# privefl/bigsnpr

Hardware: AMD Instinct MI355X
Metric: SNP-cols/sec for bed_randomSVD k=20 (m*passes/wall) (higher is better)
Workload: dtype i8 (2-bit codes x 24-bit (early block steps) / 16-bit (late block steps) fixed-point image of the fp64 basis in int8 slices, exact int32 MFMA accumulation; fp64 panel algebra and Rayleigh-Ritz)

## Files before the change

bigsnpr_amd/_lib.py:

```python
import ctypes as C
import os
import threading

import numpy as np

_HERE = os.path.dirname(os.path.abspath(__file__))
LIB_PATH = os.path.join(_HERE, "libbigsnpr_hip.so")

u8p = C.POINTER(C.c_uint8)
i32p = C.POINTER(C.c_int32)
i64p = C.POINTER(C.c_int64)
u64p = C.POINTER(C.c_uint64)
f64p = C.POINTER(C.c_double)
vp = C.c_void_p
i64 = C.c_int64

ALLREDUCE_FN = C.CFUNCTYPE(None, C.c_void_p, C.c_int64, C.c_void_p)


class SvdOptions(C.Structure):
    _fields_ = [("k", C.c_int32), ("tol", C.c_double), ("block", C.c_int32),
                ("slices", C.c_int32), ("max_basis", C.c_int32), ("seed", C.c_uint32),
                ("verbose", C.c_int32), ("m_total", C.c_int64), ("allreduce", ALLREDUCE_FN),
                ("allreduce_ctx", C.c_void_p), ("hook_rank", C.c_int32), ("hook_world", C.c_int32),
                ("comm", C.c_void_p), ("binom_scaling", C.c_int32),
                ("center_out", C.POINTER(C.c_double)), ("scale_out", C.POINTER(C.c_double)),
                ("warm_start", C.c_int32), ("warm_denominator", C.c_int32), ("max_restarts", C.c_int32),
                ("vec_floor", C.c_double), ("exchange_timing", C.c_int32), ("exchange_timeout_ms", C.c_int32)]


class SvdInfo(C.Structure):
    _fields_ = [("niter", C.c_int32), ("nops", C.c_int32), ("basis", C.c_int32),
                ("converged", C.c_int32), ("max_rel_resid", C.c_double), ("gpu_ms", C.c_double),
                ("cprod_ms", C.c_double), ("prod_ms", C.c_double), ("n_cprod", C.c_int32),
                ("n_prod", C.c_int32), ("block", C.c_int32), ("slices", C.c_int32),
                ("n_bad", C.c_int32), ("fused_stats", C.c_int32), ("cprod_stats_ms", C.c_double),
                ("n_cprod_stats", C.c_int32), ("warm_launches", C.c_int32), ("warm_fraction", C.c_double),
                ("warm_ms", C.c_double), ("tiled", C.c_int32), ("segmented_passes", C.c_int32), ("compact_gathers", C.c_int32),
                ("slices_max", C.c_int32), ("wide_steps", C.c_int32), ("wide_cprod_ms", C.c_double),
                ("wide_prod_ms", C.c_double), ("n_wide_cprod", C.c_int32), ("n_wide_prod", C.c_int32),
                ("lead_rel_resid", C.c_double), ("exchange_mode", C.c_int32), ("n_exchange", C.c_int32 * 4),
                ("exchange_ms", C.c_double * 4), ("compacted", C.c_int32), ("compact_ms", C.c_double),
                ("out_of_core", C.c_int32), ("na_free_steps", C.c_double * 2), ("na_skip", C.c_int32)]


SIGNATURES = {
    "bsn_last_error": (C.c_char_p, []),
    "bsn_version": (C.c_int, []),
    "bsn_device_count": (C.c_int, [C.POINTER(C.c_int)]),
    "bsn_set_device": (C.c_int, [C.c_int]),
    "bsn_selftest": (C.c_int, []),
    "bsn_comm_unique_id": (C.c_int, [u8p]),
    "bsn_comm_init": (C.c_int, [u8p, C.c_int, C.c_int, C.POINTER(vp)]),
    "bsn_comm_rank": (C.c_int, [vp]),
    "bsn_comm_world": (C.c_int, [vp]),
    "bsn_comm_allreduce": (C.c_int, [vp, vp, i64]),
    "bsn_comm_abort": (C.c_int, [vp]),
    "bsn_comm_destroy": (C.c_int, [vp]),
    "bsn_ld_last_stats": (C.c_int, [f64p]),
    "bsn_robust_scale_tau2": (C.c_int, [vp, i64, i64, C.c_int32, C.c_double, C.c_double, f64p, f64p]),
    "bsn_robust_pair_scales": (C.c_int, [vp, i64, i64, C.c_int32, C.c_double, C.c_double, f64p, f64p]),
    "bsn_robust_mc_count": (C.c_int, [vp, i64, vp, i64, C.c_double, C.POINTER(C.c_int64)]),
    "bsn_robust_scale_cols": (C.c_int, [vp, i64, i64, C.c_int32, f64p]),
    "bsn_robust_rotate": (C.c_int, [vp, i64, i64, C.c_int32, f64p]),
    "bsn_robust_wdist": (C.c_int, [vp, i64, i64, C.c_int32, f64p, f64p, f64p]),
    "bsn_robust_dist_ogk": (C.c_int, [vp, i64, i64, C.c_int32, C.c_int32, C.c_double, C.c_double, C.c_double, f64p, C.POINTER(C.c_int64)]),
    "bsn_robust_rollmean": (C.c_int, [f64p, i64, f64p, C.c_int32, C.POINTER(C.c_int64), C.c_int32, f64p]),
    "bsn_robust_sort": (C.c_int, [f64p, i64]),
    "bsn_order_decreasing": (C.c_int, [f64p, i64, C.POINTER(C.c_int64), C.c_int32, i32p, i32p]),
    "bsn_robust_mc_window": (C.c_int, [vp, i64, vp, i64, C.c_double, C.c_double, i64, f64p, C.POINTER(C.c_int64)]),
    "bsn_bed_open": (C.c_int, [C.c_char_p, i64, i64, C.POINTER(vp)]),
    "bsn_bed_from_host": (C.c_int, [u8p, i64, i64, i64, C.POINTER(vp)]),
    "bsn_bed_from_fbm": (C.c_int, [u8p, i64, i64, i64, C.POINTER(vp)]),
    "bsn_fbm_open": (C.c_int, [u8p, i64, i64, i64, f64p, C.POINTER(vp)]),
    "bsn_bed_bits": (C.c_int, [vp]),
    "bsn_bed_tile": (C.c_int, [vp, C.POINTER(C.c_int)]),
    "bsn_bed_sample_major": (C.c_int, [vp, C.POINTER(C.c_int)]),
    "bsn_bed_na_known": (i64, [vp]),
    "bsn_bed_synthetic": (C.c_int, [i64, i64, C.c_uint32, C.c_uint32, C.c_uint32, i64, C.POINTER(vp)]),
    "bsn_bed_close": (C.c_int, [vp]),
    "bsn_bed_release_workspace": (C.c_int, [vp]),
    "bsn_bed_nrow": (i64, [vp]),
    "bsn_bed_ncol": (i64, [vp]),
    "bsn_bed_bytes": (i64, [vp]),
    "bsn_bed_download": (C.c_int, [vp, u8p]),
    "bsn_bed_prodvec": (C.c_int, [vp, i64p, i64, i64p, i64, f64p, f64p, f64p, f64p]),
    "bsn_bed_cprodvec": (C.c_int, [vp, i64p, i64, i64p, i64, f64p, f64p, f64p, f64p]),
    "bsn_bed_prodvec_sharded": (C.c_int, [vp, i64p, i64, i64p, i64, f64p, f64p, f64p, vp, f64p]),
    "bsn_bed_col_counts": (C.c_int, [vp, i64p, i64, i64p, i64, i32p]),
    "bsn_bed_row_counts": (C.c_int, [vp, i64p, i64, i64p, i64, i32p]),
    "bsn_bed_colstats": (C.c_int, [vp, i64p, i64, i64p, i64, f64p, f64p, i32p, i32p]),
    "bsn_snp_colstats": (C.c_int, [vp, i64p, i64, i64p, i64, f64p, f64p]),
    "bsn_bed_read": (C.c_int, [vp, i64p, i64, i64p, i64, C.c_int32, i32p]),
    "bsn_bed_read_scaled": (C.c_int, [vp, i64p, i64, i64p, i64, f64p, f64p, f64p]),
    "bsn_bed_cprod_planes": (C.c_int, [vp, i64p, i64, i64p, i64, f64p, i64, f64p, f64p]),
    "bsn_bed_prod_and_rowsumssq": (C.c_int, [vp, i64p, i64, i64p, i64, f64p, f64p, f64p, i64, f64p, f64p]),
    "bsn_snp_prod_and_rowsumssq2": (C.c_int, [vp, i64p, i64, i64p, i64, f64p, f64p, f64p, i64, f64p, f64p]),
    "bsn_mult_lin_reg": (C.c_int, [vp, i64p, i64, i64p, i64, f64p, i64, f64p]),
    "bsn_univ_linreg": (C.c_int, [vp, i64p, i64, i64p, i64, f64p, f64p, i64, f64p, f64p]),
    "bsn_univ_logreg": (C.c_int, [vp, i64p, i64, i64p, i64, f64p, f64p, i64, C.c_double, C.c_int32, f64p, f64p, i32p]),
    "bsn_impute_simple": (C.c_int, [vp, C.c_int, C.c_uint64, C.POINTER(vp), u8p, i64p]),
    "bsn_impute_last_ms": (C.c_int, [f64p]),
    "bsn_bed_to_fbm": (C.c_int, [vp, i64p, i64, i64p, i64, u8p]),
    "bsn_bed_readbina": (C.c_int, [vp, u8p, u8p]),
    "bsn_bed_is_streamed": (C.c_int, [vp]),
    "bsn_bed_streaming_kernels": (C.c_int, [vp, C.c_char_p, i64]),
    "bsn_bed_subset_payload": (C.c_int, [vp, i64p, i64, i64p, i64, u8p]),
    "bsn_op_create": (C.c_int, [vp, i64p, i64, i64p, i64, f64p, f64p, C.POINTER(vp)]),
    "bsn_op_destroy": (C.c_int, [vp]),
    "bsn_op_set_slices": (C.c_int, [vp, C.c_int]),
    "bsn_op_prod": (C.c_int, [vp, vp, i64, C.c_int, vp, i64]),
    "bsn_op_cprod": (C.c_int, [vp, vp, i64, C.c_int, vp, i64]),
    "bsn_op_sync": (C.c_int, [vp]),
    "bsn_op_last_kernel": (C.c_int, [vp, C.c_char_p, i64]),
    "bsn_bed_randomsvd": (C.c_int, [vp, i64p, i64, i64p, i64, f64p, f64p, C.POINTER(SvdOptions),
                                    f64p, f64p, f64p, C.POINTER(SvdInfo)]),
    "bsn_bed_tcrossprod": (C.c_int, [vp, i64p, i64, i64p, i64, f64p, f64p, i64, f64p]),
    "bsn_cormat": (C.c_int, [vp, i64p, i64, i64p, i64, C.c_double, f64p, f64p, C.c_int, i32p,
                             C.POINTER(C.c_int64), C.POINTER(vp)]),
    "bsn_cormat_fetch": (C.c_int, [vp, i32p, f64p]),
    "bsn_cormat_has_nan": (C.c_int, [vp, C.POINTER(C.c_int)]),
    "bsn_cormat_free": (C.c_int, [vp]),
    "bsn_ld_scores": (C.c_int, [vp, i64p, i64, i64p, i64, C.c_double, f64p, f64p]),
    "bsn_clumping_chr": (C.c_int, [vp, i64p, i64, i64p, i64, C.c_int, f64p, f64p, i32p, i32p, f64p,
                                   C.c_double, C.c_double, i32p]),
    "bsn_clumping_chr_cached": (C.c_int, [vp, i64p, i64, i64p, i64, C.c_int, f64p, f64p, i32p, i32p, f64p,
                                          i64, f64p, f64p, i32p]),
    "bsn_snp_grid_prs": (C.c_int, [vp, i64p, i64, i64p, i64, f64p, i32p, C.POINTER(C.c_uint8), i64, i64,
                                   C.c_int, f64p]),
    "bsn_sfbm_from_csc": (C.c_int, [i64p, i32p, f64p, i64, C.c_int, C.POINTER(vp)]),
    "bsn_sfbm_ncol": (C.c_int, [vp, i64p, i64p, i64p]),
    "bsn_sfbm_free": (C.c_int, [vp]),
    "bsn_lassosum2": (C.c_int, [vp, f64p, i64, f64p, f64p, f64p, i64, i64p, C.c_double, C.c_int32, C.c_double,
                                f64p, i32p, f64p]),
    "bsn_ldpred2_gibbs": (C.c_int, [vp, f64p, f64p, i64, i64p, f64p, f64p, i32p, u64p, i64, C.c_int, C.c_int, C.c_uint64,
                                    f64p, f64p]),
    "bsn_ldpred2_gibbs_sampling": (C.c_int, [vp, f64p, f64p, i64, i64p, C.c_double, C.c_double, C.c_int32, C.c_uint64,
                                             C.c_int, C.c_int, C.c_uint64, f64p, f64p]),
    "bsn_ldpred2_auto": (C.c_int, [vp, f64p, f64p, f64p, i64, i64p, f64p, u64p, i64, C.c_double, C.c_int, C.c_int, C.c_int,
                                   C.c_int, C.c_double, C.c_int, C.c_double, C.c_double, C.c_double, C.c_double,
                                   C.c_double, C.c_uint64, f64p, f64p, f64p, f64p, f64p, f64p, f64p, f64p]),
    "bsn_sfbm_prodvec": (C.c_int, [vp, f64p, i64p, i64, f64p]),
    "bsn_sfbm_ld_scores": (C.c_int, [vp, i64p, i64, f64p]),
    "bsn_sfbm_solve_sym": (C.c_int, [vp, f64p, f64p, i64p, i64, C.c_double, C.c_int32, f64p, i32p, f64p]),
    "bsn_sfbm_last_ms": (C.c_int, [vp, f64p]),
    "bsn_malloc": (C.c_int, [C.POINTER(vp), i64]),
    "bsn_free": (C.c_int, [vp]),
    "bsn_host_alloc": (C.c_int, [C.POINTER(vp), i64]),
    "bsn_host_free": (C.c_int, [vp]),
    "bsn_memcpy_h2d": (C.c_int, [vp, vp, i64]),
    "bsn_memcpy_d2h": (C.c_int, [vp, vp, i64]),
    "bsn_device_sync": (C.c_int, []),
    "bsn_timer_start": (C.c_int, [vp]),
    "bsn_timer_stop": (C.c_int, [vp, f64p]),
}

_lib = None


class BsnError(RuntimeError):
    pass


def load():
    global _lib
    if _lib is None:
        LIB_PATH = os.environ.get("BSN_LIB_PATH") or globals()["LIB_PATH"]
        if not os.path.exists(LIB_PATH):
            raise ImportError(
                "%s not found: build it with `python -m bigsnpr_amd.build` "
                "(there is no CPU fallback)" % LIB_PATH)
        lib = C.CDLL(LIB_PATH)
        for name, (res, args) in SIGNATURES.items():
            fn = getattr(lib, name)
            fn.restype = res
            fn.argtypes = args
        _lib = lib
    return _lib


def check(rc):
    if rc != 0:
        raise BsnError(load().bsn_last_error().decode("utf-8", "replace"))


def ptr(a, t):
    return None if a is None else a.ctypes.data_as(t)


def as_i64(a):
    return None if a is None else np.ascontiguousarray(a, dtype=np.int64)


def as_f64(a):
    return None if a is None else np.ascontiguousarray(a, dtype=np.float64)


class DeviceArray:

    def __init__(self, rows, cols=1):
        self.rows, self.cols = int(rows), int(cols)
        p = vp()
        check(load().bsn_malloc(C.byref(p), self.rows * self.cols * 8))
        self.ptr = p

    @classmethod
    def from_numpy(cls, a):
        a = np.asarray(a, dtype=np.float64)
        if a.ndim == 1:
            a = a[:, None]
        d = cls(a.shape[0], a.shape[1])
        h = np.asfortranarray(a)
        check(load().bsn_memcpy_h2d(d.ptr, h.ctypes.data_as(vp), h.nbytes))
        return d

    def to_numpy(self):
        h = np.empty((self.rows, self.cols), dtype=np.float64, order="F")
        check(load().bsn_memcpy_d2h(h.ctypes.data_as(vp), self.ptr, h.nbytes))
        return h

    def col_ptr(self, j):
        return vp(self.ptr.value + 8 * self.rows * j)

    def free(self):
        if self.ptr is not None and self.ptr.value:
            load().bsn_free(self.ptr)
            self.ptr = None

    def __del__(self):
        try:
            self.free()
        except Exception:
            pass


class _PinnedBlock:

    def __init__(self, pool, addr, size):
        self.pool, self.addr, self.size = pool, addr, size
        self.__array_interface__ = {"data": (addr, False), "shape": (size,), "typestr": "|u1", "version": 3}

    def __del__(self):
        try:
            self.pool._give_back(self.addr, self.size)
        except Exception:
            pass


class PinnedPool:

    def __init__(self, keep=None):
        self.free = []
        self.keep = int(os.environ.get("BSN_RESULT_POOL_KEEP", 1 << 30)) if keep is None else keep
        self.keep_max = int(os.environ.get("BSN_RESULT_POOL_MAX", 8 << 30))
        self.live = 0
        self.peak_live = 0
        self.lazy = not os.environ.get("BSN_RESULT_POOL_EAGER")
        self.pending = set()
        self.wanted = []
        self.prefetched = 0
        self.lock = threading.RLock()

    def empty(self, shape, dtype=np.float64):
        n = int(np.prod(shape)) * np.dtype(dtype).itemsize
        size = max(4096, (n + 4095) // 4096 * 4096)
        addr = None
        with self.lock:
            pick = None
            for i, (_, sz) in enumerate(self.free):
                if sz >= size and (pick is None or sz < self.free[pick][1]):
                    pick = i
            if pick is not None and self.free[pick][1] <= 2 * size:
                addr, sz = self.free.pop(pick)
        if addr is None and self.lazy:
            with self.lock:
                if size not in self.pending:
                    self.pending.add(size)
                    self.wanted.append(size)
            return np.empty(shape, dtype=dtype)
        if addr is None:
            p = vp()
            if load().bsn_host_alloc(C.byref(p), size) != 0 or not p.value:
                return np.empty(shape, dtype=dtype)
            addr, sz = p.value, size
        with self.lock:
            self.live += sz
            self.peak_live = max(self.peak_live, self.live)
        blk = _PinnedBlock(self, addr, sz)
        return np.asarray(blk)[:n].view(dtype).reshape(shape)

    def kick(self):
        with self.lock:
            sizes, self.wanted = self.wanted, []
        for size in sizes:
            threading.Thread(target=self._prefetch, args=(size,), daemon=True).start()

    def _prefetch(self, size):
        p = vp()
        try:
            ok = load().bsn_host_alloc(C.byref(p), size) == 0 and p.value
        except Exception:
            ok = False
        drop = []
        with self.lock:
            self.pending.discard(size)
            if ok:
                while self.free and sum(sz for _, sz in self.free) + size > self.keep_max:
                    drop.append(self.free.pop(0))
                self.free.append((p.value, size))
                self.prefetched += 1
        for addr, _ in drop:
            load().bsn_host_free(vp(addr))

    def _give_back(self, addr, size):
        with self.lock:
            self.live -= size
            limit = max(self.keep, min(self.peak_live, self.keep_max))
            keep = sum(sz for _, sz in self.free) + size <= limit
            if keep:
                self.free.append((addr, size))
        if not keep:
            load().bsn_host_free(vp(addr))

    def drain(self):
        with self.lock:
            blocks, self.free = self.free, []
            self.peak_live = self.live
        for addr, _ in blocks:
            load().bsn_host_free(vp(addr))


result_pool = PinnedPool()
```

bigsnpr_amd/csrc/api.hip:

```cpp
#include <dlfcn.h>
#include <fcntl.h>
#include <pthread.h>
#include <sys/mman.h>
#include <sys/stat.h>
#include <unistd.h>

#include <algorithm>
#include <cerrno>
#include <cmath>
#include <condition_variable>
#include <chrono>
#include <cstring>
#include <limits>
#include <map>
#include <memory>
#include <mutex>
#include <sched.h>
#include <atomic>
#include <thread>

#include <cstdlib>

#include "bsn_internal.hpp"
#include <cxxabi.h>

namespace bsn {

namespace {
struct Roctx {
  int (*push)(const char *) = nullptr;
  int (*pop)() = nullptr;
  Roctx() {
    if (!getenv("BSN_ROCTX")) return;
    void *h = nullptr;
    for (const char *name : {"librocprofiler-sdk-roctx.so", "librocprofiler-sdk-roctx.so.1", "libroctx64.so", "libroctx64.so.4"})
      if ((h = dlopen(name, RTLD_NOW | RTLD_GLOBAL))) break;
    if (!h) return;
    push = (int (*)(const char *))dlsym(h, "roctxRangePushA");
    pop = (int (*)())dlsym(h, "roctxRangePop");
    if (!push || !pop) push = nullptr, pop = nullptr;
  }
};
Roctx &roctx() {
  static Roctx r;
  return r;
}
}
void roctx_push(const char *name) {
  if (roctx().push) roctx().push(name);
}
void roctx_pop() {
  if (roctx().pop) roctx().pop();
}

static thread_local std::string g_err;
void set_error(const char *msg) { g_err = msg ? msg : ""; }
void fail(const char *fmt, ...) {
  char buf[1024];
  va_list ap;
  va_start(ap, fmt);
  vsnprintf(buf, sizeof(buf), fmt, ap);
  va_end(ap);
  throw Error(buf);
}

void require_gpu() {
  int n = 0;
  hipError_t e = hipGetDeviceCount(&n);
  if (e != hipSuccess || n <= 0)
    fail("no HIP device available: libbigsnpr_hip has no CPU fallback (%s)",
         e == hipSuccess ? "device count is 0" : hipGetErrorString(e));
}

static std::vector<int32_t> to_i32(const int64_t *ind, int64_t len, int64_t limit, const char *what) {
  std::vector<int32_t> v((size_t)len);
  if (!ind) {
    if (len > limit)
      fail("Tested %lld < %lld. Subscript out of bounds (%s).", (long long)(len - 1), (long long)limit, what);
    for (int64_t i = 0; i < len; i++) v[(size_t)i] = (int32_t)i;
    return v;
  }
  for (int64_t i = 0; i < len; i++) {
    if (ind[i] < 0 || ind[i] >= limit)
      fail("Tested %lld < %lld. Subscript out of bounds (%s).", (long long)ind[i], (long long)limit,
           what);
    v[(size_t)i] = (int32_t)ind[i];
  }
  return v;
}

namespace {
struct DevCache {
  std::mutex mu;
  std::multimap<size_t, void *> free_blocks[16];
  size_t held[16] = {0};
};
DevCache &dev_cache() {
  static DevCache *c = new DevCache();
  return *c;
}
size_t size_class(size_t bytes) {
  size_t c = 4096;
  while (c < bytes) {
    if (c + c / 2 >= bytes) return c + c / 2;
    c *= 2;
  }
  return c;
}
}

void *dev_alloc(size_t bytes, size_t *granted, int *device) {
  if (bytes == 0) bytes = 1;
  int dev = 0;
  BSN_HIP(hipGetDevice(&dev));
  *device = dev;
  const bool cached = bytes <= kDevCacheMaxBlock && dev < 16;
  const size_t want = cached ? size_class(bytes) : bytes;
  if (cached) {
    DevCache &c = dev_cache();
    std::lock_guard<std::mutex> lk(c.mu);
    auto it = c.free_blocks[dev].find(want);
    if (it != c.free_blocks[dev].end()) {
      void *p = it->second;
      c.free_blocks[dev].erase(it);
      c.held[dev] -= want;
      *granted = want;
      return p;
    }
  }
  static const bool trace = getenv("BSN_ALLOC_TRACE") != nullptr;
  void *p = nullptr;
  const auto t0 = std::chrono::steady_clock::now();
  hipError_t e = hipMalloc(&p, want);
  if (trace)
    std::fprintf(stderr, "[bsn alloc] hipMalloc %zu bytes (asked %zu): %.2f ms\n", want, bytes,
                 std::chrono::duration<double, std::milli>(std::chrono::steady_clock::now() - t0).count());
  if (e == hipErrorOutOfMemory) {
    (void)hipGetLastError();
    dev_cache_flush();
    e = hipMalloc(&p, want);
  }
  if (e != hipSuccess) fail("HIP error %s allocating %zu bytes of device memory", hipGetErrorString(e), want);
  *granted = want;
  return p;
}

void dev_release(void *p, size_t granted, int dev) {
  if (!p) return;
  DevCache &c = dev_cache();
  if (granted <= kDevCacheMaxBlock && dev >= 0 && dev < 16 && size_class(granted) == granted) {
    int cur = dev;
    (void)hipGetDevice(&cur);
    if (cur != dev) (void)hipSetDevice(dev);
    (void)hipDeviceSynchronize();
    if (cur != dev) (void)hipSetDevice(cur);
    std::lock_guard<std::mutex> lk(c.mu);
    if (c.held[dev] + granted <= kDevCacheMaxTotal) {
      c.free_blocks[dev].emplace(granted, p);
      c.held[dev] += granted;
      return;
    }
  }
  static const bool trace = getenv("BSN_ALLOC_TRACE") != nullptr;
  if (trace) std::fprintf(stderr, "[bsn alloc] hipFree %zu bytes\n", granted);
  (void)hipFree(p);
}

size_t dev_cache_held() {
  int dev = 0;
  if (hipGetDevice(&dev) != hipSuccess || dev < 0 || dev >= 16) return 0;
  DevCache &c = dev_cache();
  std::lock_guard<std::mutex> lk(c.mu);
  return c.held[dev];
}

void dev_cache_flush() {
  DevCache &c = dev_cache();
  std::lock_guard<std::mutex> lk(c.mu);
  for (int d = 0; d < 16; d++) {
    for (auto &kv : c.free_blocks[d]) (void)hipFree(kv.second);
    c.free_blocks[d].clear();
    c.held[d] = 0;
  }
}

constexpr size_t kStagePiece = 32u << 20;

void stage_init(bsn_bed *b) {
  for (int i = 0; i < 2; i++) {
    if (!b->h_stage[i]) BSN_HIP(hipHostMalloc((void **)&b->h_stage[i], kStagePiece, hipHostMallocDefault));
    if (!b->ev_stage[i]) BSN_HIP(hipEventCreateWithFlags(&b->ev_stage[i], hipEventDisableTiming));
  }
}

namespace {
struct CopyJob {
  void *dst = nullptr;
  const void *src = nullptr;
  size_t len = 0;
};
static inline void cpu_relax() {
#if defined(__x86_64__) || defined(__i386__)
  __builtin_ia32_pause();
#elif defined(__aarch64__)
  __asm__ __volatile__("yield");
#else
  std::this_thread::yield();
#endif
}
struct CopyPool {
  static constexpr int kMaxHelpers = 6;
  int nh = 2;
  std::mutex mu;
  std::condition_variable cv_go;
  CopyJob job[kMaxHelpers];
  std::atomic<unsigned long long> seq{0};
  std::atomic<int> pending{0}, sleepers{0};
  pid_t owner = 0;
  void start() {
    owner = getpid();
    cpu_set_t set;
    int cpus = (int)std::thread::hardware_concurrency();
    if (sched_getaffinity(0, sizeof(set), &set) == 0) cpus = std::min(cpus > 0 ? cpus : 1, CPU_COUNT(&set));
    nh = std::max(1, std::min(kMaxHelpers, cpus / 2 - 1));
    if (const char *e = getenv("BSN_COPY_THREADS")) nh = std::max(1, std::min(kMaxHelpers, atoi(e) - 1));
    for (int h = 0; h < nh; h++)
      std::thread([this, h] {
        unsigned long long seen = 0;
        for (;;) {
          int spins = 0;
          while (seq.load(std::memory_order_acquire) == seen) {
            if (++spins < 4000) {
              cpu_relax();
              continue;
            }
            std::unique_lock<std::mutex> lk(mu);
            sleepers.fetch_add(1);
            cv_go.wait(lk, [&] { return seq.load() != seen; });
            sleepers.fetch_sub(1);
          }
          seen = seq.load(std::memory_order_acquire);
          const CopyJob j = job[h];
          if (j.len) std::memcpy(j.dst, j.src, j.len);
          pending.fetch_sub(1, std::memory_order_release);
        }
      }).detach();
  }
  void copy(void *dst, const void *src, size_t len) {
    const size_t part = (len / (size_t)(nh + 1) + 63) & ~(size_t)63;
    for (int h = 0; h < nh; h++) {
      const size_t lo = part * (size_t)(h + 1), hi = h + 1 == nh ? len : std::min(len, lo + part);
      job[h] = lo < hi ? CopyJob{(uint8_t *)dst + lo, (const uint8_t *)src + lo, hi - lo} : CopyJob{};
    }
    pending.store(nh, std::memory_order_relaxed);
    seq.fetch_add(1);
    if (sleepers.load() > 0) {
      { std::lock_guard<std::mutex> lk(mu); }
      cv_go.notify_all();
    }
    std::memcpy(dst, src, std::min(part, len));
    while (pending.load(std::memory_order_acquire) != 0) cpu_relax();
  }
};
CopyPool *g_pool = nullptr;
std::mutex *g_pool_mu = new std::mutex();
void pool_atfork_child() {
  g_pool_mu = new std::mutex();
  g_pool = nullptr;
}
const int g_pool_atfork = pthread_atfork(nullptr, nullptr, pool_atfork_child);
}

static void host_copy(void *dst, const void *src, size_t len) {
  static const bool pool_off = [] {
    const char *e = getenv("BSN_COPY_THREADS");
    return e && atoi(e) <= 1;
  }();
  if (len < (256u << 10) || pool_off) {
    std::memcpy(dst, src, len);
    return;
  }
  std::unique_lock<std::mutex> lk(*g_pool_mu, std::try_to_lock);
  if (!lk.owns_lock()) {
    std::memcpy(dst, src, len);
    return;
  }
  if (!g_pool || g_pool->owner != getpid()) {
    g_pool = new CopyPool();
    g_pool->start();
  }
  g_pool->copy(dst, src, len);
}

void copy_h2d(bsn_bed *b, void *d_dst, const void *src, size_t bytes, hipStream_t stream) {
  if (!stream) stream = b->stream;
  stage_init(b);
  for (size_t off = 0; off < bytes; off += kStagePiece) {
    const size_t len = std::min(kStagePiece, bytes - off);
    const int s = (int)(b->stage_next++ & 1);
    if (b->stage_busy[s]) BSN_HIP(hipEventSynchronize(b->ev_stage[s]));
    host_copy(b->h_stage[s], (const uint8_t *)src + off, len);
    BSN_HIP(hipMemcpyAsync((uint8_t *)d_dst + off, b->h_stage[s], len, hipMemcpyHostToDevice, stream));
    BSN_HIP(hipEventRecord(b->ev_stage[s], stream));
    b->stage_busy[s] = true;
  }
}

hipStream_t upload_stream(bsn_bed *b) {
  if (!b->stream_up) {
    BSN_HIP(hipStreamCreateWithFlags(&b->stream_up, hipStreamNonBlocking));
    BSN_HIP(hipEventCreateWithFlags(&b->ev_up, hipEventDisableTiming));
  }
  return b->stream_up;
}

static bool host_is_pinned(const void *p) {
  hipPointerAttribute_t at;
  if (hipPointerGetAttributes(&at, p) != hipSuccess) {
    (void)hipGetLastError();
    return false;
  }
  return at.type == hipMemoryTypeHost;
}

void copy_d2h(bsn_bed *b, void *dst, const void *d_src, size_t bytes) {
  if (bytes >= (1u << 20) && host_is_pinned(dst)) {
    BSN_HIP(hipMemcpyAsync(dst, d_src, bytes, hipMemcpyDeviceToHost, b->stream));
    BSN_HIP(hipStreamSynchronize(b->stream));
    return;
  }
  stage_init(b);
  if (b->stream_up)
    for (int i = 0; i < 2; i++)
      if (b->stage_busy[i]) BSN_HIP(hipEventSynchronize(b->ev_stage[i]));
  const size_t npiece = (bytes + kStagePiece - 1) / kStagePiece;
  for (size_t k = 0; k <= npiece; k++) {
    if (k < npiece) {
      const size_t off = k * kStagePiece, len = std::min(kStagePiece, bytes - off);
      BSN_HIP(hipMemcpyAsync(b->h_stage[k & 1], (const uint8_t *)d_src + off, len, hipMemcpyDeviceToHost, b->stream));
      BSN_HIP(hipEventRecord(b->ev_stage[k & 1], b->stream));
    }
    if (k >= 1) {
      const size_t off = (k - 1) * kStagePiece, len = std::min(kStagePiece, bytes - off);
      BSN_HIP(hipEventSynchronize(b->ev_stage[(k - 1) & 1]));
      host_copy((uint8_t *)dst + off, b->h_stage[(k - 1) & 1], len);
    }
  }
  b->stage_busy[0] = b->stage_busy[1] = false;
}

static void free_bed(bsn_bed *b) { bed_free(b); }
void bed_free(bsn_bed *b) {
  if (!b) return;
  for (int i = 0; i < 2; i++) {
    if (b->h_stage[i]) (void)hipHostFree(b->h_stage[i]);
    if (b->ev_stage[i]) (void)hipEventDestroy(b->ev_stage[i]);
  }
  if (b->smaj_job) {
    try { image_smaj_wait(b); } catch (...) {}
  }
  if (b->d_img) (void)hipFree(b->d_img);
  if (b->map_base) (void)munmap(b->map_base, b->map_len);
  if (b->fd_file >= 0) (void)close(b->fd_file);
  if (b->slab_stage) delete (bsn::FileStage *)b->slab_stage;
  if (b->slab_img) bed_free(b->slab_img);
  if (b->sub) bed_free(b->sub);
  if (b->d_tiled) (void)hipFree(b->d_tiled);
  if (b->d_smaj) (void)hipFree(b->d_smaj);
  if (b->d_lut) (void)hipFree(b->d_lut);
  if (b->h_na_blocks) (void)hipHostFree(b->h_na_blocks);
  if (b->d_na_blocks) (void)hipFree(b->d_na_blocks);
  if (b->ev0) (void)hipEventDestroy(b->ev0);
  if (b->ev1) (void)hipEventDestroy(b->ev1);
  if (b->ev_up) (void)hipEventDestroy(b->ev_up);
  if (b->stream_up) (void)hipStreamDestroy(b->stream_up);
  if (b->stream && !b->stream_borrowed) (void)hipStreamDestroy(b->stream);
  delete b;
}

__global__ void k_fill_f64(double *p, int64_t n, double v) {
  const int64_t i = (int64_t)blockIdx.x * blockDim.x + threadIdx.x;
  if (i < n) p[i] = v;
}

void fill_op(bsn_op *op, bsn_bed *bed, const int64_t *ind_row, int64_t n, const int64_t *ind_col,
             int64_t m, const double *center, const double *scale, bool defer_scale, bool allow_streamed) {
  if (n <= 0 || m <= 0) fail("'ind.row' and 'ind.col' can't be empty.");
  if (bed->n >= (int64_t)1 << 31 || bed->m >= (int64_t)1 << 31) fail("dimension too large");
  if (!allow_streamed) require_resident(bed, "this function");
  BSN_HIP(hipSetDevice(bed->device));
  op->bed = bed;
  op->n = n;
  op->m = m;
  if (!ind_row && n > bed->n)
    fail("Tested %lld < %lld. Subscript out of bounds (ind.row).", (long long)(n - 1), (long long)bed->n);
  bool ident = (n == bed->n);
  if (ind_row) {
    for (int64_t i = 0; ident && i < n; i++) ident = (ind_row[i] == i);
  }
  op->rows_identity = ident;
  if (!ident) {
    auto r = to_i32(ind_row, n, bed->n, "ind.row");
    copy_h2d(bed, op->d_rows.ensure((size_t)n), r.data(), (size_t)n * 4);
  }
  bool contig = true;
  int64_t c0 = ind_col ? ind_col[0] : 0;
  if (ind_col)
    for (int64_t j = 0; contig && j < m; j++) contig = (ind_col[j] == c0 + j);
  if (c0 < 0 || c0 >= bed->m || (contig && c0 + m > bed->m))
    fail("Tested %lld < %lld. Subscript out of bounds (ind.col).", (long long)(c0 + m - 1),
         (long long)bed->m);
  op->cols_contig = contig;
  op->col0 = contig ? c0 : 0;
  if (!contig) {
    auto c = to_i32(ind_col, m, bed->m, "ind.col");
    int64_t m_pad = bsn::round_up(m, 64);
    c.resize((size_t)m_pad, c[0]);
    copy_h2d(bed, op->d_cols.ensure((size_t)m_pad), c.data(), (size_t)m_pad * 4);
  }
  op->no_na = false;
  if ((int64_t)bed->na_cnt.size() == bed->m && !getenv("BSN_FORCE_NA_PLANE")) {
    bool all0 = true;
    for (int64_t j = 0; all0 && j < m; j++) all0 = bed->na_cnt[(size_t)(ind_col ? ind_col[j] : j)] == 0;
    op->no_na = all0;
  }
  if (defer_scale) {
    op->d_center.ensure((size_t)m);
    op->d_scale.ensure((size_t)m);
    return;
  }
  op->d_center.ensure((size_t)m);
  op->d_scale.ensure((size_t)m);
  if (center) copy_h2d(bed, op->d_center.p, center, (size_t)m * 8);
  else BSN_HIP(hipMemsetAsync(op->d_center.p, 0, (size_t)m * 8, bed->stream));
  if (scale) {
    copy_h2d(bed, op->d_scale.p, scale, (size_t)m * 8);
  } else {
    hipLaunchKernelGGL(k_fill_f64, dim3((unsigned)((m + 255) / 256)), dim3(256), 0, bed->stream, op->d_scale.p, m, 1.0);
    BSN_HIP(hipGetLastError());
  }
}

void counts_device(bsn_op *op, const int64_t *ind_row, int64_t n, int32_t *d_counts) {
  bsn_bed *bed = op->bed;
  if (op->rows_identity) {
    counts_all_rows(bed, op->cols_contig ? nullptr : op->d_cols.p, op->col0, op->m, d_counts);
  } else {
    std::vector<double> w((size_t)bed->n, 0.0);
    for (int64_t i = 0; i < n; i++) w[(size_t)(ind_row ? ind_row[i] : i)] += 1.0;
    DevBuf<double> d_w;
    copy_h2d(bed, d_w.ensure((size_t)bed->n), w.data(), (size_t)bed->n * 8);
    counts_weighted(op, d_w.p, n, d_counts);
    BSN_HIP(hipStreamSynchronize(bed->stream));
  }
}

void require_resident(const bsn_bed *b, const char *what) {
  if (b->streamed())
    fail("%s needs the genotype image resident on the device: this handle streams its file (%.1f GB do not fit the device "
         "memory that was free when it was opened); bed_prodVec, bed_cprodVec, counts / colstats / MAF / scaleBinom and the "
         "`[` accessor are served out of core",
         what, (double)b->m * (double)b->pitch / 1e9);
}

bsn_bed *slab_image(bsn_bed *b) {
  BSN_HIP(hipSetDevice(b->device));
  if (!b->slab_img) {
    std::unique_ptr<bsn_bed, void (*)(bsn_bed *)> im(new bsn_bed(), bed_free);
    image_alloc(im.get(), b->n, b->slab_cols);
    (void)hipStreamDestroy(im->stream);
    im->stream = b->stream;
    im->stream_borrowed = true;
    b->slab_img = im.release();
  }
  if (!b->slab_stage) b->slab_stage = new FileStage();
  return b->slab_img;
}
int64_t slab_count(const bsn_bed *b) { return (b->m + b->slab_cols - 1) / b->slab_cols; }
void slab_upload_range(bsn_bed *b, int64_t j0, int64_t cnt) {
  bsn_bed *img = slab_image(b);
  if (j0 < 0 || cnt <= 0 || j0 + cnt > b->m || cnt > b->slab_cols)
    fail("internal: variants %lld .. %lld into a slab image of %lld", (long long)j0, (long long)(j0 + cnt), (long long)b->slab_cols);
  img->m = cnt;
  img->na_cnt.clear();
  img->forget_counts();
  image_from_file(img, b->fd_file, 3 + j0 * b->n_byte, b->n_byte, (FileStage *)b->slab_stage);
}
int64_t slab_upload(bsn_bed *b, int64_t sl, int64_t *j0_out) {
  const int64_t j0 = sl * b->slab_cols, cnt = std::min(b->slab_cols, b->m - j0);
  if (cnt <= 0) fail("internal: slab %lld of %lld", (long long)sl, (long long)slab_count(b));
  slab_upload_range(b, j0, cnt);
  if (j0_out) *j0_out = j0;
  return cnt;
}

namespace {
struct SlabWalk {
  bsn_bed *bed;
  bsn_bed *img;
  FileStage *stage;
  SlabWalk(bsn_bed *b) : bed(b) {
    img = slab_image(b);
    stage = (FileStage *)b->slab_stage;
  }
  template <class F>
  void run(const int64_t *ind_col, int64_t m, F f) {
    const int64_t nslab = (bed->m + bed->slab_cols - 1) / bed->slab_cols;
    std::vector<std::vector<int64_t>> pos((size_t)nslab);
    for (int64_t p = 0; p < m; p++) {
      const int64_t c = ind_col ? ind_col[p] : p;
      if (c < 0 || c >= bed->m) fail("Tested %lld < %lld. Subscript out of bounds (ind.col).", (long long)c, (long long)bed->m);
      pos[(size_t)(c / bed->slab_cols)].push_back(p);
    }
    std::vector<int64_t> local;
    for (int64_t sl = 0; sl < nslab; sl++) {
      const std::vector<int64_t> &P = pos[(size_t)sl];
      if (P.empty()) continue;
      const int64_t j0 = sl * bed->slab_cols;
      slab_upload(bed, sl);
      local.resize(P.size());
      for (size_t k = 0; k < P.size(); k++) local[k] = (ind_col ? ind_col[P[k]] : P[k]) - j0;
      f(img, P, local);
    }
  }
};
}

void counts_host(bsn_bed *bed, const int64_t *ind_row, int64_t n, const int64_t *ind_col,
                 int64_t m, int32_t *res) {
  if (bed->streamed()) {
    SlabWalk W(bed);
    std::vector<int32_t> part;
    W.run(ind_col, m, [&](bsn_bed *sb, const std::vector<int64_t> &P, const std::vector<int64_t> &local) {
      part.resize(4 * P.size());
      counts_host(sb, ind_row, n, local.data(), (int64_t)local.size(), part.data());
      for (size_t k = 0; k < P.size(); k++) std::memcpy(res + 4 * P[k], part.data() + 4 * k, 16);
    });
    return;
  }
  auto &cc = bed->counts_cache;
  const bool use_cache = n > 0 && m > 0 && !getenv("BSN_NO_COUNTS_CACHE");
  bool rows_all = n == bed->n;
  for (int64_t i = 0; rows_all && ind_row && i < n; i++) rows_all = ind_row[i] == i;
  std::vector<int64_t> lead;
  const int64_t *rows = ind_row;
  if (use_cache && !rows_all && !ind_row) {
    lead.resize((size_t)n);
    for (int64_t i = 0; i < n; i++) lead[(size_t)i] = i;
    rows = lead.data();
  }
  const bool same_rows = use_cache && !rows_all && (int64_t)cc.cnt.size() == 4 * bed->m && (int64_t)cc.rows.size() == n &&
                         std::memcmp(cc.rows.data(), rows, (size_t)n * 8) == 0;
  if (same_rows) {
    bool known = true;
    for (int64_t j = 0; known && j < m; j++) {
      const int64_t c = ind_col ? ind_col[j] : j;
      known = c >= 0 && c < bed->m && cc.cnt[(size_t)4 * c] >= 0;
    }
    if (known) {
      for (int64_t j = 0; j < m; j++) std::memcpy(res + 4 * j, &cc.cnt[(size_t)4 * (ind_col ? ind_col[j] : j)], 16);
      return;
    }
  }
  bsn_op op;
  fill_op(&op, bed, ind_row, n, ind_col, m, nullptr, nullptr, true);
  DevBuf<int32_t> d_counts;
  d_counts.ensure((size_t)4 * m);
  const bool device_cache = op.rows_identity && stats_cache_enabled(bed);
  const StatsCols sel{op.cols_contig ? nullptr : ind_col, op.cols_contig ? nullptr : op.d_cols.p, op.col0, m};
  if (device_cache && use_cache && stats_cache_known(bed, sel)) {
    stats_cache_load(bed, sel, d_counts.p, bed->stream);
    copy_d2h(bed, res, d_counts.p, (size_t)4 * m * 4);
    return;
  }
  counts_device(&op, ind_row, n, d_counts.p);
  if (device_cache) stats_cache_store(bed, sel, d_counts.p, bed->stream);
  copy_d2h(bed, res, d_counts.p, (size_t)4 * m * 4);
  if (op.rows_identity) {
    if ((int64_t)bed->na_cnt.size() != bed->m) bed->na_cnt.assign((size_t)bed->m, -1);
    for (int64_t j = 0; j < m; j++) bed->na_cnt[(size_t)(ind_col ? ind_col[j] : j)] = res[4 * j + 3];
  }
  if (use_cache && !rows_all) {
    if (!same_rows) {
      cc.clear();
      cc.rows.assign(rows, rows + n);
      cc.cnt.assign((size_t)4 * bed->m, -1);
    }
    for (int64_t j = 0; j < m; j++) std::memcpy(&cc.cnt[(size_t)4 * (ind_col ? ind_col[j] : j)], res + 4 * j, 16);
  }
}

__global__ void k_stats_cache_copy(int32_t *cache, int32_t *counts, const int32_t *cols, int64_t col0, int64_t m, int to_cache) {
  const int64_t j = (int64_t)blockIdx.x * blockDim.x + threadIdx.x;
  if (j >= m) return;
  const int64_t c = cols ? (int64_t)cols[j] : col0 + j;
  if (to_cache) *(int4 *)(cache + 4 * c) = *(const int4 *)(counts + 4 * j);
  else *(int4 *)(counts + 4 * j) = *(const int4 *)(cache + 4 * c);
}

bool stats_cache_enabled(const bsn_bed *b) {
  return b->bits == 2 && !b->generic && b->d_img != nullptr && !getenv("BSN_NO_STATS_CACHE");
}

static void stats_cols_check(const bsn_bed *b, const StatsCols &c) {
  if (c.m <= 0 || (c.ind_col ? c.d_cols == nullptr : (c.col0 < 0 || c.col0 + c.m > b->m)))
    fail("internal: selection of variants for the handle's code counts");
}

bool stats_cache_known(const bsn_bed *b, const StatsCols &c) {
  const auto &sc = b->stats_cache;
  stats_cols_check(b, c);
  if ((int64_t)sc.known.size() != b->m) return false;
  if (sc.n_known == b->m) return true;
  for (int64_t j = 0; j < c.m; j++)
    if (!sc.known[(size_t)(c.ind_col ? c.ind_col[j] : c.col0 + j)]) return false;
  return true;
}

void stats_cache_store(bsn_bed *b, const StatsCols &c, const int32_t *d_counts, hipStream_t st) {
// ... 964 lines not shown
```

bigsnpr_amd/csrc/bsn_internal.hpp:

```cpp
#pragma once
#include <hip/hip_runtime.h>
#include <stdint.h>

#include <atomic>
#include <cstdarg>
#include <cstdio>
#include <functional>
#include <cstdlib>
#include <memory>
#include <stdexcept>
#include <string>
#include <vector>

#include "bigsnpr_hip.h"

namespace bsn {
inline const char *abl_getenv(const char *name) {
#ifdef BSN_ABLATION
  return getenv(name);
#else
  (void)name;
  return nullptr;
#endif
}

struct Error : std::runtime_error {
  using std::runtime_error::runtime_error;
};
void set_error(const char *msg);
[[noreturn]] void fail(const char *fmt, ...);
void require_gpu();

#define BSN_HIP(expr)                                                             \
  do {                                                                            \
    hipError_t e__ = (expr);                                                      \
    if (e__ != hipSuccess)                                                        \
      ::bsn::fail("HIP error %s at %s:%d (%s)", hipGetErrorString(e__), __FILE__, \
                  __LINE__, #expr);                                               \
  } while (0)

template <class F>
int guarded(F &&f) {
  try {
    f();
    return 0;
  } catch (const std::exception &ex) {
    set_error(ex.what());
    (void)hipGetLastError();
    return 1;
  } catch (...) {
    set_error("unknown C++ exception");
    (void)hipGetLastError();
    return 1;
  }
}

constexpr size_t kDevCacheMaxBlock = (size_t)256 << 20;
constexpr size_t kDevCacheMaxTotal = (size_t)2 << 30;
void *dev_alloc(size_t bytes, size_t *granted, int *device);
void dev_release(void *p, size_t granted, int device);
void dev_cache_flush();
size_t dev_cache_held();

template <class T>
struct DevBuf {
  T *p = nullptr;
  size_t n = 0;
  size_t granted = 0;
  int device = 0;
  DevBuf() = default;
  DevBuf(const DevBuf &) = delete;
  DevBuf &operator=(const DevBuf &) = delete;
  ~DevBuf() { release(); }
  void release() {
    if (p) dev_release(p, granted, device);
    p = nullptr;
    n = 0;
    granted = 0;
  }
  T *ensure(size_t count) {
    if (count > n) {
      release();
      p = (T *)dev_alloc(count * sizeof(T), &granted, &device);
      n = count;
    }
    return p;
  }
};

constexpr int64_t kPitchAlign = 256;

inline int64_t round_up(int64_t a, int64_t b) { return (a + b - 1) / b * b; }

__host__ __device__ inline uint32_t dev_from_plink(uint32_t w) {
  return (~w & 0xAAAAAAAAu) | ((w ^ (w >> 1)) & 0x55555555u);
}
__host__ __device__ inline uint32_t plink_from_dev(uint32_t w) {
  return (~w & 0xAAAAAAAAu) | (~(w ^ (w >> 1)) & 0x55555555u);
}

}

struct bsn_bed;
namespace bsn {
struct SvdWorkspace;
}

constexpr int kCommClasses = 4;
struct bsn_comm {
  void *comm = nullptr;
  int rank = 0, world = 1, device = 0;
  hipStream_t stream = nullptr;
  std::atomic<int> aborted{0};
  bool timing = false;
  struct Timed { hipEvent_t a, b; int cls; };
  std::vector<Timed> timed;
  std::vector<hipEvent_t> ev_pool;
  ~bsn_comm() {
    for (auto &t : timed) { (void)hipEventDestroy(t.a); (void)hipEventDestroy(t.b); }
    for (auto e : ev_pool) (void)hipEventDestroy(e);
  }
};

constexpr int kProfKinds = 6;
struct bsn_op {
  bsn_bed *bed = nullptr;
  int64_t n = 0, m = 0;
  bool rows_identity = true;
  bool cols_contig = true;
  bool no_na = false;
  bool na_skip_c = false, na_skip_p = false;
  bool stats_pending = false;
  bsn::DevBuf<int32_t> d_counts;
  bsn::DevBuf<int32_t> d_na;
  long long *h_na_total = nullptr;
  bool na_poll = false;
  int64_t col0 = 0;
  int slices = 4;
  int64_t passes = 0;
  const double *late_center = nullptr, *late_scale = nullptr;
  const double *preq_X = nullptr;
  int64_t preq_ldx = 0;
  int preq_nvec = 0, preq_S = 0;
  bool profile = false;
  int prof_kind_override = -1;
  std::vector<hipEvent_t> ev_begin, ev_end;
  std::vector<int> ev_kind;
  std::vector<char> ev_more;
  const void *prof_kernel[kProfKinds] = {};
  const void *last_kernel = nullptr;
  ~bsn_op() {
    for (auto e : ev_begin) (void)hipEventDestroy(e);
    for (auto e : ev_end) (void)hipEventDestroy(e);
    if (h_na_total) (void)hipHostFree(h_na_total);
  }
  bsn::DevBuf<int32_t> d_rows;
  bsn::DevBuf<int32_t> d_cols;
  bsn::DevBuf<double> d_center, d_scale;
  bsn::DevBuf<double> d_xfull;
  bsn::DevBuf<int8_t> d_q;
  bsn::DevBuf<int32_t> d_acc;
  bsn::DevBuf<double> d_meta;
  bsn::DevBuf<double> d_yfull;
};

struct bsn_bed {
  int64_t n = 0, m = 0, n_byte = 0, pitch = 0;
  int bits = 2;
  double v_off = 0.0, v_step = 1.0;
  bool generic = false;
  double *d_lut = nullptr;
  uint8_t *d_img = nullptr;
  uint8_t *d_tiled = nullptr;
  bool tiled_tried = false;
  size_t tiled_cap = 0;
  const uint8_t *h_map = nullptr;
  void *map_base = nullptr;
  size_t map_len = 0;
  int64_t slab_cols = 0;
  int fd_file = -1;
  bsn_bed *slab_img = nullptr;
  void *slab_stage = nullptr;
  bool streamed() const { return d_img == nullptr && h_map != nullptr; }
  uint8_t *d_smaj = nullptr;
  int64_t pitch_smaj = 0, rows_smaj = 0;
  bool smaj_tried = false;
  size_t smaj_cap = 0;
  void *smaj_job = nullptr;
  int64_t cap_m = 0;
  bsn_bed *sub = nullptr;
  uint64_t sub_key = 0;
  std::vector<int64_t> sub_cols, sub_rows;
  bool last_solve_on_sub = false;
  int device = 0;
  bool stream_borrowed = false;
  hipStream_t stream = nullptr;
  hipStream_t stream_up = nullptr;
  hipEvent_t ev_up = nullptr;
  hipEvent_t ev0 = nullptr, ev1 = nullptr;
  std::vector<int32_t> na_cnt;
  struct CountsCache {
    std::vector<int64_t> rows;
    std::vector<int32_t> cnt;
    void clear() {
      rows.clear();
      cnt.clear();
    }
  } counts_cache;
  struct StatsCache {
    bsn::DevBuf<int32_t> d_cnt;
    std::vector<uint8_t> known;
    int64_t n_known = 0;
    bsn::DevBuf<int32_t> d_cols;
    uint64_t cols_key = 0;
    void clear() {
      known.clear();
      n_known = 0;
    }
    void release() {
      clear();
      d_cnt.release();
      d_cols.release();
      cols_key = 0;
    }
  } stats_cache;
  void forget_counts() {
    counts_cache.clear();
    stats_cache.clear();
  }
  int na_blocks_state = 0;
  long long *h_na_blocks = nullptr;
  long long *d_na_blocks = nullptr;
  double na_free[2] = {0.0, 0.0};
  std::unique_ptr<bsn_op> svd_op;
  std::shared_ptr<bsn::SvdWorkspace> svd_ws;
  uint8_t *h_stage[2] = {nullptr, nullptr};
  hipEvent_t ev_stage[2] = {nullptr, nullptr};
  bool stage_busy[2] = {false, false};
  unsigned stage_next = 0;
};


namespace bsn {

void image_alloc(bsn_bed *b, int64_t n, int64_t m, int bits = 2);
void stage_init(bsn_bed *b);
void bed_free(bsn_bed *b);
bsn_bed *image_gather(bsn_bed *src, const int64_t *ind_row, int64_t n, const int64_t *ind_col, int64_t m,
                      bsn_bed *reuse = nullptr);
bool image_tile(bsn_bed *b);
bool image_smaj(bsn_bed *b);
bool image_smaj_start(bsn_bed *b);
bool image_smaj_poll(bsn_bed *b);
void image_smaj_wait(bsn_bed *b);
void image_from_host(bsn_bed *b, const uint8_t *payload, int64_t n_byte_src);
struct FileStage {
  uint8_t *pin[2] = {nullptr, nullptr};
  hipEvent_t done[2] = {nullptr, nullptr};
  size_t bytes = 0;
  ~FileStage();
  FileStage() = default;
  FileStage(const FileStage &) = delete;
  FileStage &operator=(const FileStage &) = delete;
};
void image_from_file(bsn_bed *b, int fd, int64_t offset, int64_t n_byte_src, FileStage *stage = nullptr);
void image_from_fbm(bsn_bed *b, const uint8_t *bytes, int64_t ld, const uint8_t *lut);
void stats8(bsn_bed *b, const int32_t *d_rows, int64_t n, const int32_t *d_cols, int64_t col0, int64_t m,
            long long *d_out);
void lut_colstats(bsn_bed *b, const int32_t *d_rows, int64_t n, const int32_t *d_cols, int64_t col0, int64_t m,
                  double *d_out);
void lut_cprod(bsn_bed *b, const int32_t *d_rows, int64_t n, const int32_t *d_cols, int64_t col0, int64_t m,
               const double *d_center, const double *d_scale, const double *d_x, double *d_z);
void lut_prod(bsn_bed *b, const int32_t *d_rows, int64_t n, const int32_t *d_cols, int64_t col0, int64_t m,
              const double *d_center, const double *d_scale, const double *d_x, double *d_y);
void refuse_generic(const bsn_bed *b, const char *what);
void image_generate(bsn_bed *b, uint32_t seed, uint32_t npop, uint32_t na16, int64_t j_begin);
void image_download(bsn_bed *b, uint8_t *payload_out);
void counts_all_rows(bsn_bed *b, const int32_t *d_cols, int64_t col0, int64_t m, int32_t *d_counts);
void counts_host(bsn_bed *bed, const int64_t *ind_row, int64_t n, const int64_t *ind_col, int64_t m,
                 int32_t *res);
void counts_device(bsn_op *op, const int64_t *ind_row, int64_t n, int32_t *d_counts);
struct StatsCols {
  const int64_t *ind_col;
  const int32_t *d_cols;
  int64_t col0, m;
};
bool stats_cache_enabled(const bsn_bed *b);
bool stats_cache_known(const bsn_bed *b, const StatsCols &c);
void stats_cache_store(bsn_bed *b, const StatsCols &c, const int32_t *d_counts, hipStream_t st);
void stats_cache_load(bsn_bed *b, const StatsCols &c, int32_t *d_counts, hipStream_t st);
void read_dense(bsn_bed *b, const int32_t *d_rows, int64_t n, const int32_t *d_cols, int64_t m,
                const double *d_center, const double *d_scale, int32_t na_val, int32_t *d_out_i,
                double *d_out_d);

void to_bytes(bsn_bed *b, const int32_t *d_rows, int64_t n, const int32_t *d_cols, int64_t m,
              uint8_t *d_out);
void readbina_bytes(bsn_bed *b, const uint8_t *d_tab, uint8_t *d_out);
void subset_pack(bsn_bed *b, const int32_t *d_rows, int64_t n, const int32_t *d_cols, int64_t m,
                 uint8_t *d_out);

void copy_h2d(bsn_bed *b, void *d_dst, const void *src, size_t bytes, hipStream_t stream = nullptr);
hipStream_t upload_stream(bsn_bed *b);
void copy_d2h(bsn_bed *b, void *dst, const void *d_src, size_t bytes);

void fill_op(bsn_op *op, bsn_bed *bed, const int64_t *ind_row, int64_t n, const int64_t *ind_col,
             int64_t m, const double *center, const double *scale, bool defer_scale = false,
             bool allow_streamed = false);
bsn_bed *slab_image(bsn_bed *b);
int64_t slab_count(const bsn_bed *b);
int64_t slab_upload(bsn_bed *b, int64_t sl, int64_t *j0_out = nullptr);
void slab_upload_range(bsn_bed *b, int64_t j0, int64_t cnt);

hipEvent_t comm_time_begin(bsn_comm *c, hipStream_t st);
void comm_time_end(bsn_comm *c, hipEvent_t begin, int cls, hipStream_t st);
void comm_time_collect(bsn_comm *c, double ms[kCommClasses], int count[kCommClasses]);
bool comm_abort(bsn_comm *c);
void comm_allreduce_sum(bsn_comm *c, double *d_buf, int64_t count, hipStream_t st);
void comm_reduce_scatter_sum(bsn_comm *c, const double *d_send, double *d_recv, int64_t recv_count,
                             hipStream_t st);
void comm_all_gather(bsn_comm *c, const double *d_send, double *d_recv, int64_t send_count, hipStream_t st);

void op_poll_stats(bsn_op *op);
void op_na_blocks(bsn_op *op, int digit_cols);
void op_prod(bsn_op *op, const double *d_X, int64_t ldx, int nvec, double *d_Y, int64_t ldy);
void op_prod_acc(bsn_op *op, const double *d_X, int64_t ldx, int nvec, double *d_Y, int64_t ldy, double beta);
struct ProdSegment {
  int bs = 0, off = 0;
  const int32_t *d_rows = nullptr;
  double *d_out = nullptr;
};
bool op_prod_segments(bsn_op *op, const double *d_X, int64_t ldx, int nvec, int pieces, int stride, int nseg,
                      const ProdSegment *segs, const std::function<void(int)> &after);
void op_cprod(bsn_op *op, const double *d_X, int64_t ldx, int nvec, double *d_Z, int64_t ldz);
void op_cprod_prequant(bsn_op *op, const double *d_X, int64_t ldx, int nvec);
void op_cprod_raw(bsn_op *op, const double *d_X, int64_t ldx, int nvec, double *d_P, double *d_Q,
                  int64_t ld);
void require_bits(const bsn_bed *b, int bits, const char *what);
void op_row_sums_sq(bsn_op *op, double *d_out);
void op_row_counts(bsn_op *op, double *d_out);
void counts_weighted(bsn_op *op, const double *d_w, int64_t n_sub, int32_t *d_counts);
void selftest();
void roctx_push(const char *name);
void roctx_pop();
struct RoctxRange {
  explicit RoctxRange(const char *name) { roctx_push(name); }
  ~RoctxRange() { roctx_pop(); }
  RoctxRange(const RoctxRange &) = delete;
  RoctxRange &operator=(const RoctxRange &) = delete;
};
void require_resident(const bsn_bed *b, const char *what);
void prof_begin(bsn_op *op, int kind, bool more = false);
void prof_end(bsn_op *op);
void prof_collect(bsn_op *op, double ms[kProfKinds], int count[kProfKinds]);

}
```

bigsnpr_amd/csrc/svd.hip:

```cpp
#include <chrono>
#include <unistd.h>
#include <atomic>
#include <condition_variable>
#include <mutex>
#include <thread>
#include <cmath>
#include <cstring>
#include <memory>
#include <functional>

#include "bsn_internal.hpp"
#include "orth_small.hpp"
#include "svd_driver.hpp"

namespace bsn {

constexpr int kMaxB = 16;
constexpr int kTP = 256;

__device__ __forceinline__ uint32_t hmix(uint32_t x) {
  x ^= x >> 16; x *= 0x7feb352dU; x ^= x >> 15; x *= 0x846ca68bU; x ^= x >> 16;
  return x;
}

// ... 55 lines not shown
      for (int t = 0; t < NT; t++) {
        acc[t] = __builtin_amdgcn_mfma_f64_16x16x4f64(av[u].x, bval[t] ? bv[t][u].x : 0.0, acc[t], 0, 0, 0);
        acc[t] = __builtin_amdgcn_mfma_f64_16x16x4f64(av[u].y, bval[t] ? bv[t][u].y : 0.0, acc[t], 0, 0, 0);
      }
  };
  const int64_t nfull = r1 > r0 ? (r1 - r0) / 32 : 0;
  if (nfull > 0) {
    ld(r0, av0, bv0);
    for (int64_t g = 0; g < nfull; g += 2) {
      ld(r0 + 32 * (g + 1 < nfull ? g + 1 : nfull - 1), av1, bv1);
      mm(av0, bv0);
      ld(r0 + 32 * (g + 2 < nfull ? g + 2 : nfull - 1), av0, bv0);
      if (g + 1 < nfull) mm(av1, bv1);
    }
  }
  int64_t r = r0 + 32 * nfull;
  for (; r < r1; r += 8) {
    const int64_t i0 = r + 2 * kq, i1 = i0 + 1;
    const double a0 = i0 < r1 ? Ap[i0] : 0.0, a1 = i1 < r1 ? Ap[i1] : 0.0;
#pragma unroll
    for (int t = 0; t < NT; t++) {
      const double b0 = (bval[t] && i0 < r1) ? Bp[t][i0] : 0.0, b1 = (bval[t] && i1 < r1) ? Bp[t][i1] : 0.0;
      acc[t] = __builtin_amdgcn_mfma_f64_16x16x4f64(a0, b0, acc[t], 0, 0, 0);
      acc[t] = __builtin_amdgcn_mfma_f64_16x16x4f64(a1, b1, acc[t], 0, 0, 0);
    }
  }
  __shared__ double red[4][256];
#pragma unroll
  for (int t = 0; t < NT; t++) {
    if (t > 0) __syncthreads();
#pragma unroll
    for (int g = 0; g < 4; g++) red[wave][(kq + 4 * g) * 16 + a] = acc[t][g];
    __syncthreads();
    partial[(((int64_t)rc * gridDim.x + tile) * NT + t) * 256 + tid] =
        (red[0][tid] + red[1][tid]) + (red[2][tid] + red[3][tid]);
  }
}

__global__ __launch_bounds__(1024) void k_gemm_tn_reduce(const double *__restrict__ partial, int nrc, int ntile, int p,
                                                         int cb, double *C, int ldc) {
  const int tile = blockIdx.x, bt = blockIdx.y, nt = gridDim.y, t = threadIdx.x & 255, part = threadIdx.x >> 8;
  double sum = 0;
#pragma unroll 4
  for (int c = part; c < nrc; c += 4) sum += partial[(((int64_t)c * ntile + tile) * nt + bt) * 256 + t];
  __shared__ double sp[4][256];
  sp[part][t] = sum;
  __syncthreads();
  if (part == 0) {
    sum = (sp[0][t] + sp[1][t]) + (sp[2][t] + sp[3][t]);
    const int mrow = t >> 4, ncol = bt * 16 + (t & 15);
    if (tile * 16 + mrow < p && ncol < cb) C[(tile * 16 + mrow) + (int64_t)ncol * ldc] = sum;
  }
}

__global__ __launch_bounds__(256) void k_gemm_nn(const double *__restrict__ Q, int64_t ldq, int p,
                                                 const double *__restrict__ S, int nc,
                                                 const double *In, int64_t ldi, double alpha,
                                                 double beta, double *Out, int64_t ldo, int64_t n) {
  extern __shared__ __attribute__((aligned(16))) double sS[];
  constexpr int TP = kTP;
  const int64_t i = (int64_t)blockIdx.x * blockDim.x + threadIdx.x;
  double acc[kMaxB];
#pragma unroll
  for (int j = 0; j < kMaxB; j++) acc[j] = 0;
  for (int a0 = 0; a0 < p; a0 += TP) {
    int ta = p - a0 < TP ? p - a0 : TP;
    __syncthreads();
    for (int t = threadIdx.x; t < ta * kMaxB; t += blockDim.x) {
      int a = t / kMaxB, j = t % kMaxB;
      sS[t] = j < nc ? S[(a0 + a) + (int64_t)j * p] : 0.0;
    }
    __syncthreads();
    if (i < n) {
      for (int a = 0; a < ta; a++) {
        double q = Q[i + (int64_t)(a0 + a) * ldq];
#pragma unroll
        for (int j = 0; j < kMaxB; j++) acc[j] += q * sS[a * kMaxB + j];
      }
    }
  }
  if (i < n) {
#pragma unroll
    for (int j = 0; j < kMaxB; j++)
      if (j < nc) {
        double base = alpha != 0.0 ? alpha * In[i + (int64_t)j * ldi] : 0.0;
        Out[i + (int64_t)j * ldo] = base + beta * acc[j];
      }
  }
}

__global__ void k_put_block(double *M, int ld, int r, const double *src) {
  const int t = blockIdx.x * blockDim.x + threadIdx.x;
  if (t < r * r) M[(t % r) + (int64_t)(t / r) * ld] = src[t];
}

__global__ void k_right_mult(double *W, int64_t ld, int64_t n, int cb, int r, const double *M) {
  __shared__ double sM[kMaxB * kMaxB];
  if ((int)threadIdx.x < cb * r) sM[threadIdx.x] = M[threadIdx.x];
  __syncthreads();
  int64_t i = (int64_t)blockIdx.x * blockDim.x + threadIdx.x;
  if (i >= n) return;
  double w[kMaxB], o[kMaxB];
#pragma unroll
  for (int j = 0; j < kMaxB; j++) w[j] = j < cb ? W[i + j * ld] : 0.0;
#pragma unroll
  for (int c = 0; c < kMaxB; c++) {
    double s = 0;
#pragma unroll
    for (int j = 0; j < kMaxB; j++)
      if (j < cb && c < r) s += w[j] * sM[j + c * cb];
    o[c] = s;
  }
#pragma unroll
  for (int c = 0; c < kMaxB; c++)
    if (c < r) W[i + c * ld] = o[c];
}

struct DevCtx {
  int tid, nt;
  __device__ void sync() { __syncthreads(); }
};
__global__ __launch_bounds__(512) void k_orth2(OrthSmall a, unsigned long long *mx_clear) {
  __shared__ double sCs[kOrthMaxP * kOrthMaxB];
  __shared__ double sG[kOrthMaxB * kOrthMaxB], sR[kOrthMaxB * kOrthMaxB], sRi[kOrthMaxB * kOrthMaxB],
      sRo[kOrthMaxB * kOrthMaxB], sD[kOrthMaxB * kOrthMaxB], sT[2 * kOrthMaxB + 4];
  a.Cs = sCs;
  a.Gs = sG;
  a.Rs = sR;
  a.Ris = sRi;
  a.Ro = sRo;
  a.Dv = sD;
  a.tmp = sT;
  if (mx_clear && threadIdx.x < kOrthMaxB) mx_clear[threadIdx.x] = 0ull;
  DevCtx cx{(int)threadIdx.x, (int)blockDim.x};
  orth_small(cx, a);
}

template <int CBT>
__global__ __launch_bounds__(256) void k_update(const double *__restrict__ Q, int64_t ldq, int p,
                                                const double *__restrict__ C, const double *__restrict__ Ri,
                                                int cb, double *W, int64_t ldw, int64_t n,
                                                unsigned long long *mx) {
  constexpr int TP = 128, ROWS = 4;
  __shared__ double sS[TP * CBT], sRi[CBT * CBT], smx[4][CBT];
  const int tid = threadIdx.x, lane = tid & 63, wave = tid >> 6;
  for (int t = tid; t < CBT * CBT; t += 256) {
    const int j = t % CBT, c = t / CBT;
    sRi[t] = (j < cb && c < cb) ? Ri[j + c * cb] : 0.0;
  }
  if (tid < 4 * CBT) smx[tid / CBT][tid % CBT] = 0.0;
  const bool one_tile = p <= TP;
  for (int it = 0; it < ROWS; it++) {
    const int64_t i = ((int64_t)blockIdx.x * ROWS + it) * 256 + tid;
    double acc[CBT];
#pragma unroll
    for (int j = 0; j < CBT; j++) acc[j] = 0;
    for (int a0 = 0; a0 < p; a0 += TP) {
      const int ta = p - a0 < TP ? p - a0 : TP;
      if (!(one_tile && it > 0)) {
        __syncthreads();
        for (int t = tid; t < ta * CBT; t += 256) {
          const int a = t / CBT, j = t % CBT;
          sS[t] = j < cb ? C[(a0 + a) + (int64_t)j * p] : 0.0;
        }
        __syncthreads();
      }
      if (i < n) {
#pragma unroll 8
        for (int a = 0; a < ta; a++) {
          const double q = Q[i + (int64_t)(a0 + a) * ldq];
#pragma unroll
          for (int j = 0; j < CBT; j++) acc[j] += q * sS[a * CBT + j];
        }
      }
    }
    if (p == 0 && it == 0) __syncthreads();
    double w[CBT];
#pragma unroll
    for (int j = 0; j < CBT; j++) w[j] = (i < n && j < cb) ? W[i + j * ldw] - acc[j] : 0.0;
#pragma unroll 1
    for (int c = 0; c < cb; c++) {
      double s = 0;
#pragma unroll
      for (int j = 0; j < CBT; j++) s += w[j] * sRi[j + c * CBT];
      if (i < n) W[i + c * ldw] = s;
      if (mx) {
        double m = fabs(s);
        for (int off = 32; off > 0; off >>= 1) m = fmax(m, __shfl_down(m, off));
        if (lane == 0) smx[wave][c] = fmax(smx[wave][c], m);
      }
    }
  }
  if (mx) {
    __syncthreads();
    if (tid < cb) {
      const double m = fmax(fmax(smx[0][tid], smx[1][tid]), fmax(smx[2][tid], smx[3][tid]));
      atomicMax(&mx[tid], (unsigned long long)__double_as_longlong(m));
    }
  }
}

__global__ void k_col_absmax(const double *W, int64_t ld, int64_t n, unsigned long long *mx) {
  const int v = blockIdx.y;
  double m = 0;
  for (int64_t i = (int64_t)blockIdx.x * blockDim.x + threadIdx.x; i < n; i += (int64_t)gridDim.x * blockDim.x)
    m = fmax(m, fabs(W[i + v * ld]));
  for (int off = 32; off > 0; off >>= 1) m = fmax(m, __shfl_down(m, off));
  __shared__ double sm[16];
  const int wave = threadIdx.x >> 6, nw = blockDim.x >> 6;
  if ((threadIdx.x & 63) == 0) sm[wave] = m;
  __syncthreads();
  if (threadIdx.x == 0) {
    for (int w = 1; w < nw; w++) m = fmax(m, sm[w]);
    atomicMax(&mx[v], (unsigned long long)__double_as_longlong(m));
  }
}
__global__ void k_round_cols(double *W, int64_t ld, int64_t n, const unsigned long long *mx, int slices) {
  const int v = blockIdx.y;
  const double m = __longlong_as_double((long long)mx[v]);
  if (!(m > 0)) return;
  int e;
  frexp(ldexp(0.98, 8 * slices - 1) / m, &e);
  const double qs = ldexp(1.0, e - 1), iq = ldexp(1.0, 1 - e);
  const int64_t i = (int64_t)blockIdx.x * blockDim.x + threadIdx.x;
  if (i < n) W[i + v * ld] = (double)llrint(W[i + v * ld] * qs) * iq;
}

__global__ void k_block(const double *__restrict__ full, int64_t n, int cb, int64_t nr, int world,
                        double *__restrict__ blk) {
  const int64_t t = (int64_t)blockIdx.x * blockDim.x + threadIdx.x;
  if (t >= (int64_t)world * cb * nr) return;
  const int64_t i = t % nr, j = (t / nr) % cb, r = t / (nr * cb);
  const int64_t gi = r * nr + i;
  blk[t] = gi < n ? full[gi + j * n] : 0.0;
}
__global__ void k_unblock(const double *__restrict__ blk, int64_t n, int cb, int64_t nr,
                          double *__restrict__ full) {
  const int64_t t = (int64_t)blockIdx.x * blockDim.x + threadIdx.x;
  if (t >= n * cb) return;
  const int64_t gi = t % n, j = t / n;
  full[t] = blk[((gi / nr) * cb + j) * nr + gi % nr];
}
__global__ void k_max_over_ranks(const unsigned long long *__restrict__ all, int world, int cb,
                                 unsigned long long *__restrict__ mx) {
  const int v = threadIdx.x;
  if (v >= cb) return;
  unsigned long long m = 0;
  for (int r = 0; r < world; r++) m = all[r * cb + v] > m ? all[r * cb + v] : m;
  mx[v] = m;
}
template <typename INT>
__global__ void k_pack_int(double *__restrict__ W, int64_t nr, const unsigned long long *__restrict__ mx, int slices,
                           INT *__restrict__ q) {
  const int v = blockIdx.y;
  const int64_t i = (int64_t)blockIdx.x * blockDim.x + threadIdx.x;
  if (i >= nr) return;
  const double m = __longlong_as_double((long long)mx[v]);
  if (!(m > 0)) {
    q[i + v * nr] = 0;
    return;
  }
  int e;
  frexp(ldexp(0.98, 8 * slices - 1) / m, &e);
  const double qs = ldexp(1.0, e - 1), iq = ldexp(1.0, 1 - e);
  const long long k = llrint(W[i + v * nr] * qs);
  q[i + v * nr] = (INT)k;
  W[i + v * nr] = (double)k * iq;
}
template <typename INT>
__global__ void k_unpack_int(const INT *__restrict__ q, int64_t n, int cb, int64_t nr,
                             const unsigned long long *__restrict__ mx, int slices, double *__restrict__ full) {
  const int64_t t = (int64_t)blockIdx.x * blockDim.x + threadIdx.x;
  if (t >= n * cb) return;
  const int64_t gi = t % n, v = t / n;
  const double m = __longlong_as_double((long long)mx[v]);
  double val = 0.0;
  if (m > 0) {
    int e;
    frexp(ldexp(0.98, 8 * slices - 1) / m, &e);
    val = (double)q[((gi / nr) * cb + v) * nr + gi % nr] * ldexp(1.0, 1 - e);
  }
  full[t] = val;
}

__global__ void k_place_rows(const double *__restrict__ src, int64_t rows, int cb, int64_t r0, int64_t nr,
                             double *__restrict__ W) {
  const int64_t t = (int64_t)blockIdx.x * blockDim.x + threadIdx.x;
  if (t >= rows * cb) return;
  W[r0 + t % rows + (t / rows) * nr] = src[t];
}
__global__ void k_take_rows(const double *__restrict__ full, int64_t n, int cb, int64_t nr, int64_t row0,
                            double *__restrict__ W) {
  const int64_t t = (int64_t)blockIdx.x * blockDim.x + threadIdx.x;
  if (t >= nr * cb) return;
  const int64_t i = t % nr, j = t / nr;
  W[t] = row0 + i < n ? full[row0 + i + j * n] : 0.0;
}

struct SvdWorkspace {
  DevBuf<double> Q, Z, partial, dsmall, Wsave, dorth, Wfull, Wblk, Qfull, dS, dU, dV, dUfull, dM;
  double *h_pin = nullptr;
  size_t h_pin_n = 0;
  hipEvent_t ev_small = nullptr;
  hipStream_t st_comm = nullptr;
  hipEvent_t ev_seg[8] = {nullptr, nullptr, nullptr, nullptr, nullptr, nullptr, nullptr, nullptr};
  hipEvent_t ev_arrived = nullptr;
  DevBuf<int32_t> seg_rows;
  DevBuf<double> Wrecv;
  int64_t seg_n = -1, seg_nr = -1;
  int seg_world = -1;
  double *pinned(size_t count) {
    if (count > h_pin_n) {
      if (h_pin) (void)hipHostFree(h_pin);
      h_pin = nullptr;
      BSN_HIP(hipHostMalloc((void **)&h_pin, count * sizeof(double), hipHostMallocDefault));
      h_pin_n = count;
    }
    return h_pin;
  }
  ~SvdWorkspace() {
    for (auto &e : ev_seg)
      if (e) (void)hipEventDestroy(e);
    if (ev_arrived) (void)hipEventDestroy(ev_arrived);
    if (st_comm) (void)hipStreamDestroy(st_comm);
    if (ev_small) (void)hipEventDestroy(ev_small);
    if (h_pin) (void)hipHostFree(h_pin);
  }
};

struct HipSvdBackend : SvdBackend {
  SvdWorkspace &ws;
  explicit HipSvdBackend(SvdWorkspace &w)
      : ws(w), Q(w.Q), Z(w.Z), partial(w.partial), dsmall(w.dsmall), Wsave(w.Wsave), dorth(w.dorth),
        Wfull(w.Wfull), Wblk(w.Wblk), Qfull(w.Qfull) {}
  bsn_op *op = nullptr;
  hipStream_t st = nullptr;
  bsn_allreduce_fn hook = nullptr;
  void *ctx = nullptr;
  bsn_comm *comm = nullptr;
  int rank = 0, world = 1;
  bool dist = false;
  int64_t nr = 0, row0 = 0;
  DevBuf<double> &Q, &Z, &partial, &dsmall, &Wsave, &dorth, &Wfull, &Wblk, &Qfull;
  double *Wc = nullptr;
  int wcol = 0;
  std::vector<double> horth;
  int cap = 0, b = 0;
  int kmax = 0;
  bool mx_valid = false;
  bool no_fused = false;
  bool speculate = true;
  bool spec_rounded = false;
  int n_small_ar = 0;
  int64_t m_op_full = 0, m_sub = 0;
  bool fused_stats = false;
  int warm_launches = 0, warm_den = 16;
  bool subset(bool on) override {
    if (ooc) return false;
    if (on) {
      m_op_full = op->m;
      const int64_t m_lo = m_total / (world > 0 ? world : 1);
      const int64_t ms = (m_lo / warm_den) / 256 * 256;
      if (m_total / warm_den < 16384 || ms < 256) return false;
      m_sub = ms < op->m ? ms : op->m;
      op->m = m_sub;
      op->prof_kind_override = 3;
      roctx_push("svd:warm start (leading 1/16 of the variants)");
      return true;
    }
    roctx_pop();
    op->m = m_op_full;
    op->prof_kind_override = -1;
    warm_launches += 2;
    if (fused_stats) {
      op->stats_pending = true;
      op->na_poll = false;
      op->no_na = false;
    }
    return true;
  }
  bool timing = false;
  double t_phase[8] = {0, 0, 0, 0, 0, 0, 0, 0};
  int n_sync = 0;
  struct Tick {
    HipSvdBackend *b;
    int ph;
    std::chrono::steady_clock::time_point t0;
    Tick(HipSvdBackend *b_, int ph_) : b(b_), ph(ph_), t0(std::chrono::steady_clock::now()) {
      static const char *names[8] = {"svd:alloc", "svd:crossprod pass (Z = A'Q)", "svd:product pass (W = A Z)", "svd:gram blocks",
                                     "svd:orthonormalise", "svd:round / copy block", "svd:form u, v", "svd:other"};
      roctx_push(names[ph & 7]);
    }
    ~Tick() {
      roctx_pop();
      if (b->timing)
        b->t_phase[ph] += std::chrono::duration<double, std::milli>(std::chrono::steady_clock::now() - t0).count();
    }
  };
  void sync_stream() {
    BSN_HIP(hipStreamSynchronize(st));
    n_sync++;
  }

  void setup_ranks() {
    if (comm) {
      rank = comm->rank;
      world = comm->world;
    }
    dist = comm != nullptr || hook != nullptr;
    if (!dist) world = 1, rank = 0;
    nr = dist ? (n + world - 1) / world : n;
    if (dist && comm && nr >= 4096) nr = (nr + 511) / 512 * 512;
    row0 = (int64_t)rank * nr;
  }
  void alloc(int cap_, int b_) override {
    Tick tk(this, 0);
    if (b_ > kMaxB) fail("block size must be <= %d", kMaxB);
    cap = cap_;
    b = b_;
    Q.ensure((size_t)nr * (cap + kMaxB));
    Z.ensure((size_t)m_local * cap);
    {
      const int64_t rows_max = nr > m_local ? nr : m_local;
      partial.ensure((size_t)((rows_max + kGemmRows - 1) / kGemmRows) * ((cap + kMaxB + 15) / 16) * 2 * 256);
    }
    dsmall.ensure((size_t)(cap + 4) * 64);
    Wsave.ensure((size_t)nr * kMaxB);
    dorth.ensure((size_t)16 + 3 * kMaxB * kMaxB + (size_t)7 * (cap + kMaxB + 4) * kMaxB);
    ws.dM.ensure((size_t)kOrthMaxP * kOrthMaxP);
    if (dist) {
      const int wide = kmax > kMaxB ? kmax : kMaxB;
      Wfull.ensure((size_t)n * wide);
      Wblk.ensure((size_t)world * nr * wide);
      Qfull.ensure((size_t)n * kMaxB);
    }
    Wc = Q.p;
    wcol = 0;
  }

  void ar_small(double *d, int64_t count) {
    if (!dist) return;
    n_small_ar++;
    if (comm) {
      comm_allreduce_sum(comm, d, count, st);
    } else {
      sync_stream();
      hook(d, count, ctx);
    }
  }
  void reduce_scatter_W(int cb) {
    const int64_t tot = (int64_t)world * cb * nr;
    hipLaunchKernelGGL(k_block, dim3((unsigned)((tot + 255) / 256)), dim3(256), 0, st, Wfull.p, n, cb, nr, world,
                       Wblk.p);
    BSN_HIP(hipGetLastError());
    if (comm) {
      comm_reduce_scatter_sum(comm, Wblk.p, Wc, nr * cb, st);
    } else {
      sync_stream();
      hook(Wblk.p, tot, ctx);
      BSN_HIP(hipMemcpyAsync(Wc, Wblk.p + (int64_t)rank * cb * nr, (size_t)nr * cb * 8,
                             hipMemcpyDeviceToDevice, st));
    }
  }
  void all_gather_rows(const double *src, int cb, double *dst) {
    const int64_t tot = (int64_t)world * cb * nr;
    if (comm) {
      comm_all_gather(comm, src, Wblk.p, nr * cb, st);
    } else {
      BSN_HIP(hipMemsetAsync(Wblk.p, 0, (size_t)tot * 8, st));
      BSN_HIP(hipMemcpyAsync(Wblk.p + (int64_t)rank * cb * nr, src, (size_t)nr * cb * 8, hipMemcpyDeviceToDevice, st));
      sync_stream();
      hook(Wblk.p, tot, ctx);
    }
    hipLaunchKernelGGL(k_unblock, dim3((unsigned)((n * cb + 255) / 256)), dim3(256), 0, st, Wblk.p, n, cb, nr, dst);
    BSN_HIP(hipGetLastError());
  }

  void random_W(int bb, uint32_t seed) override {
    Wc = Q.p;
    wcol = 0;
    mx_valid = false;
    spec_rounded = false;
    op->preq_X = nullptr;
    hipLaunchKernelGGL(k_random, dim3((unsigned)((nr + 255) / 256), bb), dim3(256), 0, st, Wc, nr, nr, bb, seed,
                       row0, n);
    BSN_HIP(hipGetLastError());
  }
  const double *newest_block(int p0) const { return dist ? Qfull.p : Q.p + (int64_t)p0 * nr; }
  bool ooc = false;
  const int64_t *ooc_cols = nullptr;
  std::vector<int64_t> sel_at, sel_local;
  std::unique_ptr<bsn_op> sop;
  long long ooc_na_total = 0, ooc_n_bad = 0;
  bool ooc_stats_walk = false;
  int64_t slab_selection(int64_t sl, int64_t *at) {
    if (!ooc_cols) {
      int64_t j0 = 0;
      const int64_t cnt = slab_upload(op->bed, sl, &j0);
      *at = j0;
      sel_local.clear();
      return cnt;
    }
    if (sel_at.empty()) {
      const int64_t nslab = slab_count(op->bed), sc = op->bed->slab_cols;
      sel_at.assign((size_t)nslab + 1, 0);
      for (int64_t t = 0; t < m_local; t++) sel_at[(size_t)(ooc_cols[t] / sc) + 1]++;
      for (int64_t q = 0; q < nslab; q++) sel_at[(size_t)q + 1] += sel_at[(size_t)q];
    }
    const int64_t a = sel_at[(size_t)sl], cnt = sel_at[(size_t)sl + 1] - a;
    *at = a;
    if (cnt <= 0) return 0;
    int64_t j0 = 0;
    slab_upload(op->bed, sl, &j0);
    sel_local.resize((size_t)cnt);
    for (int64_t t = 0; t < cnt; t++) sel_local[(size_t)t] = ooc_cols[a + t] - j0;
    return cnt;
  }
  void slab_operator(int64_t j0, int64_t cnt, bool with_scaling) {
    bsn_bed *img = slab_image(op->bed);
    if (!sop) sop.reset(new bsn_op());
    sop->bed = img;
    sop->n = n;
    sop->m = cnt;
    sop->rows_identity = true;
    sop->cols_contig = true;
    sop->col0 = 0;
    if (!sel_local.empty()) {
      bool contig = true;
      for (int64_t t = 1; t < cnt && contig; t++) contig = sel_local[(size_t)t] == sel_local[0] + t;
      sop->cols_contig = contig;
      sop->col0 = contig ? sel_local[0] : 0;
      if (!contig) {
        const int64_t m_pad = round_up(cnt, 64);
        std::vector<int32_t> c((size_t)m_pad, (int32_t)sel_local[0]);
        for (int64_t t = 0; t < cnt; t++) c[(size_t)t] = (int32_t)sel_local[(size_t)t];
        copy_h2d(op->bed, sop->d_cols.ensure((size_t)m_pad), c.data(), (size_t)m_pad * 4);
        BSN_HIP(hipStreamSynchronize(st));
      }
    }
    sop->no_na = false;
    sop->slices = op->slices;
    sop->profile = op->profile;
    sop->prof_kind_override = op->prof_kind_override;
    sop->preq_X = nullptr;
    sop->d_center.ensure((size_t)op->bed->slab_cols);
    sop->d_scale.ensure((size_t)op->bed->slab_cols);
    if (with_scaling) {
      BSN_HIP(hipMemcpyAsync(sop->d_center.p, op->d_center.p + j0, (size_t)cnt * 8, hipMemcpyDeviceToDevice, st));
      BSN_HIP(hipMemcpyAsync(sop->d_scale.p, op->d_scale.p + j0, (size_t)cnt * 8, hipMemcpyDeviceToDevice, st));
    }
  }
  void At_Qblock_ooc(int p0, int cb) {
    const int64_t nslab = slab_count(op->bed);
    const bool stats = op->stats_pending;
    if (stats) {
      ooc_na_total = ooc_n_bad = 0;
      op->d_na.ensure((size_t)op->m);
    }
    for (int64_t sl = 0; sl < nslab; sl++) {
      int64_t j0 = 0;
      const int64_t cnt = slab_selection(sl, &j0);
      if (cnt <= 0) continue;
      slab_operator(j0, cnt, !stats);
      sop->stats_pending = stats;
      sop->na_poll = false;
      op_cprod(sop.get(), newest_block(p0), n, cb, Z.p + (int64_t)p0 * m_local + j0, m_local);
      if (stats) {
        BSN_HIP(hipMemcpyAsync(op->d_center.p + j0, sop->d_center.p, (size_t)cnt * 8, hipMemcpyDeviceToDevice, st));
        BSN_HIP(hipMemcpyAsync(op->d_scale.p + j0, sop->d_scale.p, (size_t)cnt * 8, hipMemcpyDeviceToDevice, st));
        BSN_HIP(hipMemcpyAsync(op->d_na.p + j0, sop->d_na.p, (size_t)cnt * 4, hipMemcpyDeviceToDevice, st));
        sync_stream();
        if (sop->h_na_total && sop->h_na_total[0] >= 0) {
          ooc_na_total += sop->h_na_total[0];
          ooc_n_bad += sop->h_na_total[1];
        }
      } else {
        sync_stream();
      }
    }
    if (stats) {
      op->stats_pending = false;
      if (!op->h_na_total) BSN_HIP(hipHostMalloc((void **)&op->h_na_total, 2 * sizeof(long long), hipHostMallocDefault));
      op->h_na_total[0] = ooc_na_total;
      op->h_na_total[1] = ooc_n_bad;
    }
    op->passes++;
  }
  void A_Zblock_ooc(int p0, int cb) {
    const int64_t nslab = slab_count(op->bed);
    bool first = true;
    for (int64_t sl = 0; sl < nslab; sl++) {
      int64_t j0 = 0;
      const int64_t cnt = slab_selection(sl, &j0);
      if (cnt <= 0) continue;
      slab_operator(j0, cnt, true);
      op_prod_acc(sop.get(), Z.p + (int64_t)p0 * m_local + j0, m_local, cb, Wc, n, first ? 0.0 : 1.0);
      first = false;
      sync_stream();
    }
    op->passes++;
  }
  void At_Qblock(int p0, int cb) override {
    Tick tk(this, 1);
    if (progress) progress();
    if (ooc) return At_Qblock_ooc(p0, cb);
    op_cprod(op, newest_block(p0), n, cb, Z.p + (int64_t)p0 * m_local, m_local);
  }
  bool product_in_segments(int p0, int cb) {
    if (!comm || nr % 512 != 0 || nr < 4096 || getenv("BSN_NO_SEGMENTS")) return false;
    const int B = (int)(nr / 512), nseg = B >= 16 ? 4 : 2;
    if (ws.seg_n != n || ws.seg_nr != nr || ws.seg_world != world) {
      std::vector<int32_t> rows((size_t)world * nr);
      size_t at = 0;
      for (int sgi = 0; sgi < nseg; sgi++) {
        const int b0 = (int)((int64_t)B * sgi / nseg), b1 = (int)((int64_t)B * (sgi + 1) / nseg);
        for (int r = 0; r < world; r++)
          for (int64_t t = (int64_t)b0 * 512; t < (int64_t)b1 * 512; t++) {
            const int64_t gi = (int64_t)r * nr + t;
            rows[at++] = gi < n ? (int32_t)gi : -1;
          }
      }
      copy_h2d(op->bed, ws.seg_rows.ensure(rows.size()), rows.data(), rows.size() * 4);
      BSN_HIP(hipStreamSynchronize(st));
      ws.seg_n = n; ws.seg_nr = nr; ws.seg_world = world;
    }
    const bool overlap = !getenv("BSN_NO_OVERLAP");
    if (overlap && !ws.st_comm) BSN_HIP(hipStreamCreateWithFlags(&ws.st_comm, hipStreamNonBlocking));
    for (int i = 0; i < nseg; i++)
      if (!ws.ev_seg[i]) BSN_HIP(hipEventCreateWithFlags(&ws.ev_seg[i], hipEventDisableTiming));
    if (!ws.ev_arrived) BSN_HIP(hipEventCreateWithFlags(&ws.ev_arrived, hipEventDisableTiming));
    ws.Wrecv.ensure((size_t)nr * kMaxB);
    ProdSegment segs[4];
    for (int sgi = 0; sgi < nseg; sgi++) {
      const int b0 = (int)((int64_t)B * sgi / nseg), b1 = (int)((int64_t)B * (sgi + 1) / nseg);
      segs[sgi].bs = b1 - b0;
      segs[sgi].off = b0;
      segs[sgi].d_rows = ws.seg_rows.p + (size_t)world * 512 * b0;
      segs[sgi].d_out = Wblk.p + (size_t)world * cb * 512 * b0;
    }
    hipStream_t sc = overlap ? ws.st_comm : st;
    const std::function<void(int)> after = [&](int sgi) {
      const int64_t rows_s = (int64_t)segs[sgi].bs * 512, r0 = (int64_t)segs[sgi].off * 512;
      if (overlap) {
        BSN_HIP(hipEventRecord(ws.ev_seg[sgi], st));
        BSN_HIP(hipStreamWaitEvent(sc, ws.ev_seg[sgi], 0));
      }
      double *recv = ws.Wrecv.p + (size_t)cb * r0;
      comm_reduce_scatter_sum(comm, segs[sgi].d_out, recv, rows_s * cb, sc);
      hipLaunchKernelGGL(k_place_rows, dim3((unsigned)((rows_s * cb + 255) / 256)), dim3(256), 0, sc, recv, rows_s, cb,
                         r0, nr, Wc);
      BSN_HIP(hipGetLastError());
    };
    if (overlap) {
      BSN_HIP(hipEventRecord(ws.ev_arrived, st));
      BSN_HIP(hipStreamWaitEvent(sc, ws.ev_arrived, 0));
    }
    if (!op_prod_segments(op, Z.p + (int64_t)p0 * m_local, m_local, cb, world, B, nseg, segs, after)) return false;
    if (overlap) {
      BSN_HIP(hipEventRecord(ws.ev_arrived, sc));
      hipEvent_t t0 = comm_time_begin(comm, st);
      BSN_HIP(hipStreamWaitEvent(st, ws.ev_arrived, 0));
      comm_time_end(comm, t0, 3, st);
    }
    n_seg_passes++;
    exchange_mode = std::max(exchange_mode, overlap ? 3 : 2);
    return true;
  }
  int min_slices = 8;
  bool hold_round = false;
  void hold_rounding(bool hold) override { hold_round = hold; }
  void set_precision(int S) override {
    if (S < 1) S = 1;
    if (S > 7) S = 7;
    op->slices = S;
    if (sop) sop->slices = S;
    if (S < min_slices) min_slices = S;
  }
  std::function<void()> progress;
  int n_seg_passes = 0;
  int exchange_mode = 0;
  int n_compact_gathers = 0;
  void A_Zblock(int p0, int cb) override {
    Tick tk(this, 2);
    mx_valid = false;
    if (ooc) return A_Zblock_ooc(p0, cb);
    if (dist && product_in_segments(p0, cb)) return;
    op_prod(op, Z.p + (int64_t)p0 * m_local, m_local, cb, dist ? Wfull.p : Wc, n);
    if (dist) {
      reduce_scatter_W(cb);
      exchange_mode = std::max(exchange_mode, 1);
    }
  }
  void gemm_tn_any(const double *A, const double *B, int64_t rows, int p, int cb, double *dC, int ldc = 0) {
    if (p <= 0 || cb <= 0) return;
    dim3 grid((unsigned)((p + 15) / 16), (unsigned)((rows + kGemmRows - 1) / kGemmRows));
    const int nt = (cb + 15) / 16;
    if (nt == 1)
      hipLaunchKernelGGL((k_gemm_tn<1>), grid, dim3(256), 0, st, A, rows, p, B, rows, cb, rows, partial.p);
    else if (nt == 2)
      hipLaunchKernelGGL((k_gemm_tn<2>), grid, dim3(256), 0, st, A, rows, p, B, rows, cb, rows, partial.p);
    else
      fail("internal: panel product with %d columns", cb);
    hipLaunchKernelGGL(k_gemm_tn_reduce, dim3(grid.x, nt), dim3(1024), 0, st, partial.p, (int)grid.y, (int)grid.x, p, cb,
                       dC, ldc > 0 ? ldc : p);
  }
  void gemm_tn(const double *A, int p, int cb, double *C_host) {
    gemm_tn_any(A, Wc, nr, p, cb, dsmall.p);
    BSN_HIP(hipGetLastError());
    ar_small(dsmall.p, (int64_t)p * cb);
    double *hp = ws.pinned((size_t)(cap + kMaxB + 4) * kMaxB * 4 + 1024);
    BSN_HIP(hipMemcpyAsync(hp, dsmall.p, (size_t)p * cb * 8, hipMemcpyDeviceToHost, st));
    sync_stream();
    std::memcpy(C_host, hp, (size_t)p * cb * 8);
  }
  void round_cols(double *X, int64_t rows, int cb, bool have_mx) {
    unsigned long long *mx = (unsigned long long *)dorth.p;
    if (!have_mx) {
      BSN_HIP(hipMemsetAsync(mx, 0, (size_t)cb * 8, st));
      hipLaunchKernelGGL(k_col_absmax, dim3(256, cb), dim3(1024), 0, st, X, rows, rows, mx);
    }
    hipLaunchKernelGGL(k_round_cols, dim3((unsigned)((rows + 255) / 256), cb), dim3(256), 0, st, X, rows, rows, mx,
                       op->slices);
    BSN_HIP(hipGetLastError());
  }
  void round_W(int cb) override {
    if (cb <= 0) return;
    if (spec_rounded) {
      spec_rounded = false;
      return;
    }
    Tick tk(this, 5);
    if (!dist) {
      round_cols(Wc, n, cb, mx_valid);
      mx_valid = false;
      return;
    }
    if (comm && op->slices <= 4 && nr % 4 == 0 && !getenv("BSN_NO_COMPACT_GATHER")) {
      unsigned long long *mx = (unsigned long long *)dorth.p;
      BSN_HIP(hipMemsetAsync(mx, 0, (size_t)cb * 8, st));
      hipLaunchKernelGGL(k_col_absmax, dim3(64, cb), dim3(1024), 0, st, Wc, nr, nr, mx);
      double *gmax = ws.Wrecv.ensure(std::max((size_t)nr * kMaxB, (size_t)world * kMaxB));
      comm_all_gather(comm, (const double *)mx, gmax, cb, st);
      hipLaunchKernelGGL(k_max_over_ranks, dim3(1), dim3(64), 0, st, (const unsigned long long *)gmax, world, cb, mx);
      const dim3 gp((unsigned)((nr + 255) / 256), cb), gu((unsigned)((n * cb + 255) / 256));
      if (op->slices <= 2) {
        int16_t *q_send = (int16_t *)Wfull.p, *q_all = (int16_t *)Wblk.p;
        hipLaunchKernelGGL((k_pack_int<int16_t>), gp, dim3(256), 0, st, Wc, nr, mx, op->slices, q_send);
        BSN_HIP(hipGetLastError());
        comm_all_gather(comm, (const double *)q_send, (double *)q_all, nr * cb / 4, st);
        hipLaunchKernelGGL((k_unpack_int<int16_t>), gu, dim3(256), 0, st, q_all, n, cb, nr, mx, op->slices, Qfull.p);
      } else {
        int32_t *q_send = (int32_t *)Wfull.p, *q_all = (int32_t *)Wblk.p;
        hipLaunchKernelGGL((k_pack_int<int32_t>), gp, dim3(256), 0, st, Wc, nr, mx, op->slices, q_send);
        BSN_HIP(hipGetLastError());
        comm_all_gather(comm, (const double *)q_send, (double *)q_all, nr * cb / 2, st);
        hipLaunchKernelGGL((k_unpack_int<int32_t>), gu, dim3(256), 0, st, q_all, n, cb, nr, mx, op->slices, Qfull.p);
      }
      BSN_HIP(hipGetLastError());
      n_compact_gathers++;
      return;
    }
    all_gather_rows(Wc, cb, Qfull.p);
    round_cols(Qfull.p, n, cb, false);
    hipLaunchKernelGGL(k_take_rows, dim3((unsigned)((nr * cb + 255) / 256)), dim3(256), 0, st, Qfull.p, n, cb, nr,
                       row0, Wc);
    BSN_HIP(hipGetLastError());
  }
  void gram_to_host(const double *A, const double *B, int64_t rows, int p, int cb, double *out) {
    Tick tk(this, 3);
    gemm_tn_any(A, B, rows, p, cb, dsmall.p);
    BSN_HIP(hipGetLastError());
    ar_small(dsmall.p, (int64_t)p * cb);
    double *hp = ws.pinned((size_t)(cap + kMaxB + 4) * kMaxB * 4 + 1024);
    BSN_HIP(hipMemcpyAsync(hp, dsmall.p, (size_t)p * cb * 8, hipMemcpyDeviceToHost, st));
    sync_stream();
    std::memcpy(out, hp, (size_t)p * cb * 8);
    op_poll_stats(op);
  }
  void ZtZ(int p, int p0, int cb, double *G) override {
    gram_to_host(Z.p, Z.p + (int64_t)p0 * m_local, m_local, p, cb, G);
  }
  void QtQ(int p, int p0, int cb, double *M) override {
    gram_to_host(Q.p, Q.p + (int64_t)p0 * nr, nr, p, cb, M);
  }

  static constexpr int B2 = kMaxB * kMaxB;
  void update_W(int p, int cb, const double *C, const double *Ri, unsigned long long *mx) {
    const dim3 rows((unsigned)((nr + 1023) / 1024));
    if (cb <= 8)
      hipLaunchKernelGGL((k_update<8>), rows, dim3(256), 0, st, Q.p, nr, p, C, Ri, cb, Wc, nr, nr, mx);
    else
      hipLaunchKernelGGL((k_update<16>), rows, dim3(256), 0, st, Q.p, nr, p, C, Ri, cb, Wc, nr, nr, mx);
  }
  int fused(int p, int p0, int cb, bool with_grams, double *blkZ, double *blkQ, std::vector<double> &Rout) {
    if (cb <= 0 || cb > kMaxB || p + cb > kOrthMaxP || p + cb > cap + kMaxB || no_fused) return -1;
    if (p > 0 && Wc != Q.p + (int64_t)p * nr) return -1;
    if (p > 0 && !with_grams) return -1;
    const double *A0 = p > 0 ? Q.p : Wc;
    Tick tk(this, 4);
    hipEvent_t tev0 = nullptr, tev1 = nullptr;
    if (timing) {
      BSN_HIP(hipEventCreate(&tev0));
      BSN_HIP(hipEventCreate(&tev1));
      BSN_HIP(hipEventRecord(tev0, st));
    }
    unsigned long long *mx = (unsigned long long *)dorth.p;
    const size_t pc = (size_t)p * cb, hg = (size_t)(p + cb) * cb;
    double *flag = dorth.p + 16, *dRout = flag + 1, *dZtZ = dRout + B2, *X = dZtZ + pc, *HG1 = X + (p > 0 ? hg : 0),
           *HG2 = HG1 + hg, *C = HG2 + hg, *Ct = C + pc, *Ri = Ct + pc;
    BSN_HIP(hipMemsetAsync(flag, 0, (size_t)(1 + B2) * 8, st));
    if (p > 0) gemm_tn_any(Z.p, Z.p + (int64_t)p0 * m_local, m_local, p, cb, dZtZ);
    BSN_HIP(hipMemcpyAsync(Wsave.p, Wc, (size_t)nr * cb * 8, hipMemcpyDeviceToDevice, st));
    OrthSmall a;
    a.p = p;
    a.cb = cb;
    a.p0 = p0;
    a.QtQ = p > 0 ? X : nullptr;
    a.ldq = p + cb;
    a.M = ws.dM.p;
    a.ldm = kOrthMaxP;
    a.C = C;
    a.Ct = Ct;
    a.Ri = Ri;
    a.Rout = dRout;
    a.flag = flag;
    a.iters = std::min(min_slices, op->slices) >= 2 ? 2 : 4;
    a.Cs = a.Gs = a.Rs = a.Ris = a.Ro = a.Dv = a.tmp = nullptr;
    for (int pass = 0; pass < 2; pass++) {
      double *HG = pass == 0 ? HG1 : HG2;
      if (pass == 0 && p > 0) {
        gemm_tn_any(Q.p, Q.p + (int64_t)p0 * nr, nr, p + cb, 2 * cb, X, p + cb);
        ar_small(dZtZ, (int64_t)(pc + 2 * hg));
      } else {
        gemm_tn_any(A0, Wc, nr, p + cb, cb, HG, p + cb);
        ar_small(HG, (int64_t)hg);
      }
      a.pass = pass;
      a.HG = HG;
      unsigned long long *mxp = (pass == 1 && !dist) ? mx : nullptr;
      hipLaunchKernelGGL(k_orth2, dim3(1), dim3(512), 0, st, a, mxp);
      update_W(p, cb, C, Ri, mxp);
    }
    BSN_HIP(hipGetLastError());
    const size_t nsmall = 1 + B2 + pc + (p > 0 ? hg : 0);
    double *hp = ws.pinned((size_t)(cap + kMaxB + 4) * kMaxB * 4 + 1024);
    BSN_HIP(hipMemcpyAsync(hp, flag, nsmall * 8, hipMemcpyDeviceToHost, st));
    if (timing) BSN_HIP(hipEventRecord(tev1, st));
    if (with_grams && speculate && !hold_round) {
      if (!ws.ev_small) BSN_HIP(hipEventCreateWithFlags(&ws.ev_small, hipEventDisableTiming));
      BSN_HIP(hipEventRecord(ws.ev_small, st));
      mx_valid = !dist;
      spec_rounded = false;
      round_W(cb);
      if (!ooc) op_cprod_prequant(op, dist ? Qfull.p : Wc, n, cb);
      spec_rounded = true;
      BSN_HIP(hipEventSynchronize(ws.ev_small));
      n_sync++;
    } else {
      sync_stream();
    }
    if (timing) {
      float ms = 0;
      BSN_HIP(hipEventElapsedTime(&ms, tev0, tev1));
      t_phase[7] += ms;
      (void)hipEventDestroy(tev0);
      (void)hipEventDestroy(tev1);
    }
    op_poll_stats(op);
    if (blkZ) std::memcpy(blkZ, hp + 1 + B2, pc * 8);
    if (blkQ)
      for (int j = 0; j < cb; j++) std::memcpy(blkQ + (size_t)j * p, hp + 1 + B2 + pc + (size_t)j * (p + cb), (size_t)p * 8);
    if (hp[0] != 0.0) {
      BSN_HIP(hipMemcpyAsync(Wc, Wsave.p, (size_t)nr * cb * 8, hipMemcpyDeviceToDevice, st));
      mx_valid = false;
      spec_rounded = false;
      op->preq_X = nullptr;
      return -2;
    }
    Rout.assign((size_t)cb * cb, 0.0);
    for (int t = 0; t < cb * cb; t++) Rout[(size_t)t] = hp[1 + (size_t)t];
    mx_valid = spec_rounded ? false : !dist;
    return cb;
  }
  int step_fused(int p, int p0, int cb, double *blkZ, double *blkQ, std::vector<double> &Rout) override {
    return fused(p, p0, cb, true, blkZ, blkQ, Rout);
  }
  int orth_fused(int p, int cb, std::vector<double> &Cacc, std::vector<double> &Rout) override {
    if (p != 0) return -1;
    Cacc.clear();
    const int r = fused(0, 0, cb, false, nullptr, nullptr, Rout);
    return r < 0 ? -1 : r;
  }
  void QtW(int p, int cb, double *C) override { gemm_tn(Q.p, p, cb, C); }
  void WtW(int cb, double *G) override { gemm_tn(Wc, cb, cb, G); }
  void W_minus_QC(int p, int cb, const double *C) override {
    mx_valid = false;
    copy_h2d(op->bed, dsmall.p, C, (size_t)p * cb * 8);
    hipLaunchKernelGGL(k_gemm_nn, dim3((unsigned)((nr + 255) / 256)), dim3(256), kTP * kMaxB * 8, st,
                       Q.p, nr, p, dsmall.p, cb, Wc, nr, 1.0, -1.0, Wc, nr, nr);
    BSN_HIP(hipGetLastError());
    sync_stream();
  }
  void W_times(int cb, int r, const double *M) override {
    mx_valid = false;
    copy_h2d(op->bed, dsmall.p, M, (size_t)cb * r * 8);
    hipLaunchKernelGGL(k_right_mult, dim3((unsigned)((nr + 255) / 256)), dim3(256), 0, st, Wc, nr, nr,
                       cb, r, dsmall.p);
    BSN_HIP(hipGetLastError());
    sync_stream();
  }
  void W_to_Q(int p0, int r) override {
    double *dst = Q.p + (int64_t)p0 * nr;
    if (dst != Wc)
      BSN_HIP(hipMemcpyAsync(dst, Wc, (size_t)nr * r * 8, hipMemcpyDeviceToDevice, st));
    wcol = p0 + r;
    Wc = Q.p + (int64_t)wcol * nr;
  }
  bool restart(int pp, int keep, const double *S, int rn, const double *Mk) override {
    if (keep + rn > pp || keep <= 0) return false;
    DevBuf<double> &dS = ws.dS, &tQ = ws.dU, &tZ = ws.dV;
    dS.ensure((size_t)pp * keep + 16);
    tQ.ensure((size_t)nr * keep);
    tZ.ensure((size_t)m_local * keep);
    copy_h2d(op->bed, dS.p, S, (size_t)pp * keep * 8);
    for (int c0 = 0; c0 < keep; c0 += kMaxB) {
      const int nc = keep - c0 < kMaxB ? keep - c0 : kMaxB;
      hipLaunchKernelGGL(k_gemm_nn, dim3((unsigned)((nr + 255) / 256)), dim3(256), kTP * kMaxB * 8, st, Q.p, nr, pp,
                         dS.p + (size_t)c0 * pp, nc, (const double *)nullptr, (int64_t)0, 0.0, 1.0,
                         tQ.p + (int64_t)c0 * nr, nr, nr);
      hipLaunchKernelGGL(k_gemm_nn, dim3((unsigned)((m_local + 255) / 256)), dim3(256), kTP * kMaxB * 8, st, Z.p,
                         m_local, pp, dS.p + (size_t)c0 * pp, nc, (const double *)nullptr, (int64_t)0, 0.0, 1.0,
                         tZ.p + (int64_t)c0 * m_local, m_local, m_local);
    }
    BSN_HIP(hipGetLastError());
    BSN_HIP(hipMemcpyAsync(Q.p, tQ.p, (size_t)nr * keep * 8, hipMemcpyDeviceToDevice, st));
    BSN_HIP(hipMemcpyAsync(Z.p, tZ.p, (size_t)m_local * keep * 8, hipMemcpyDeviceToDevice, st));
    double *dst = Q.p + (int64_t)keep * nr;
    BSN_HIP(hipMemcpyAsync(dst, Wc, (size_t)nr * rn * 8, hipMemcpyDeviceToDevice, st));
    Wc = dst;
    wcol = keep;
    copy_h2d(op->bed, dS.p, Mk, (size_t)keep * keep * 8);
    hipLaunchKernelGGL(k_put_block, dim3((unsigned)((keep * keep + 255) / 256)), dim3(256), 0, st, ws.dM.p,
                       kOrthMaxP, keep, dS.p);
    BSN_HIP(hipGetLastError());
    return true;
  }
  void finalize(int pp, int k, const double *S, const double *dinv, double *u, double *v) override {
    Tick tk(this, 6);
    std::vector<double> Sv((size_t)pp * k);
    for (int t = 0; t < k; t++)
      for (int i = 0; i < pp; i++) Sv[(size_t)i + (size_t)t * pp] = S[(size_t)i + (size_t)t * pp] * dinv[t];
    DevBuf<double> &dS = ws.dS, &dU = ws.dU, &dV = ws.dV, &dUfull = ws.dUfull;
    dS.ensure((size_t)pp * k * 2 + 16);
    dU.ensure((size_t)nr * k);
    dV.ensure((size_t)m_local * k);
    copy_h2d(op->bed, dS.p, S, (size_t)pp * k * 8);
    copy_h2d(op->bed, dS.p + (size_t)pp * k, Sv.data(), (size_t)pp * k * 8);
    for (int c0 = 0; c0 < k && pp > 0; c0 += kMaxB) {
      int nc = k - c0 < kMaxB ? k - c0 : kMaxB;
      hipLaunchKernelGGL(k_gemm_nn, dim3((unsigned)((nr + 255) / 256)), dim3(256), kTP * kMaxB * 8, st,
                         Q.p, nr, pp, dS.p + (size_t)c0 * pp, nc, (const double *)nullptr, (int64_t)0,
                         0.0, 1.0, dU.p + (int64_t)c0 * nr, nr, nr);
      hipLaunchKernelGGL(k_gemm_nn, dim3((unsigned)((m_local + 255) / 256)), dim3(256),
                         kTP * kMaxB * 8, st, Z.p, m_local, pp, dS.p + (size_t)pp * k + (size_t)c0 * pp,
                         nc, (const double *)nullptr, (int64_t)0, 0.0, 1.0,
                         dV.p + (int64_t)c0 * m_local, m_local, m_local);
    }
    BSN_HIP(hipGetLastError());
    if (pp == 0) {
      BSN_HIP(hipMemsetAsync(dU.p, 0, (size_t)nr * k * 8, st));
      BSN_HIP(hipMemsetAsync(dV.p, 0, (size_t)m_local * k * 8, st));
    }
    const double *ufull = dU.p;
    if (dist) {
      dUfull.ensure((size_t)n * k);
      all_gather_rows(dU.p, k, dUfull.p);
      ufull = dUfull.p;
    }
    if (u) copy_d2h(op->bed, u, ufull, (size_t)n * k * 8);
    if (v) copy_d2h(op->bed, v, dV.p, (size_t)m_local * k * 8);
    sync_stream();
  }
};

}

using namespace bsn;

struct ExchangeWatchdog {
  bsn_comm *c;
  int ms;
  std::thread th;
  std::mutex mu;
  std::condition_variable cv;
  bool done = false;
  std::chrono::steady_clock::time_point deadline;
  std::atomic<int> fired{0};
  ExchangeWatchdog(bsn_comm *c_, int ms_) : c(c_), ms(ms_) {
    if (!c || ms <= 0) return;
    deadline = std::chrono::steady_clock::now() + std::chrono::milliseconds(ms);
    th = std::thread([this] {
      std::unique_lock<std::mutex> lk(mu);
      for (;;) {
        const auto dl = deadline;
        if (cv.wait_until(lk, dl, [this] { return done; })) return;
        if (std::chrono::steady_clock::now() >= deadline) break;
      }
      if (done) return;
      fired.store(1);
      lk.unlock();
      const bool could = comm_abort(c);
      std::fprintf(stderr, "[bsn svd] rank %d: the sharded solve made no progress for %d ms: communicator %s\n", c->rank, ms,
                   could ? "aborted" : "cannot be aborted (no ncclCommAbort)");
      lk.lock();
      if (cv.wait_for(lk, std::chrono::seconds(20), [this] { return done; })) return;
      const char *ex = getenv("BSN_WATCHDOG_EXIT");
      if (ex && atoi(ex) != 0) {
        std::fprintf(stderr, "[bsn svd] rank %d: still blocked 20 s after the abort: giving up (exit status 86, BSN_WATCHDOG_EXIT)\n", c->rank);
        std::fflush(stderr);
        _exit(86);
      }
      std::fprintf(stderr, "[bsn svd] rank %d: still blocked 20 s after the abort (BSN_WATCHDOG_EXIT=1 would end the process here)\n", c->rank);
    });
  }
  void kick() {
    if (!th.joinable()) return;
    std::lock_guard<std::mutex> lk(mu);
    deadline = std::chrono::steady_clock::now() + std::chrono::milliseconds(ms);
  }
  ~ExchangeWatchdog() {
    if (!th.joinable()) return;
    {
      std::lock_guard<std::mutex> lk(mu);
      done = true;
    }
    cv.notify_all();
    th.join();
  }
};

static void binom_scale_host(const std::vector<int32_t> &cnt, int64_t n, int64_t m, std::vector<double> &center,
                             std::vector<double> &scale, int32_t *n_bad) {
  center.resize((size_t)m);
  scale.resize((size_t)m);
  int32_t bad = 0;
  for (int64_t j = 0; j < m; j++) {
    const int32_t *c = &cnt[(size_t)4 * j];
    const double sumX = (double)(c[1] + 2 * c[2]), nona = (double)(c[0] + c[1] + c[2]);
    const double af = sumX / (2.0 * nona);
    center[(size_t)j] = 2.0 * af;
    scale[(size_t)j] = std::sqrt(2.0 * af * (1.0 - af));
    if (2 * (int64_t)(c[0] + c[1] + c[2]) < n) bad++;
  }
  *n_bad = bad;
}

#pragma clang fp contract(off)
__global__ __launch_bounds__(256) void k_scale_from_counts(const int32_t *counts, int64_t m, int64_t n, double *center,
                                                           double *scale, unsigned long long *out) {
  long long s = 0, bad = 0;
  for (int64_t j = (int64_t)blockIdx.x * 256 + threadIdx.x; j < m; j += (int64_t)gridDim.x * 256) {
    const int4 c = *(const int4 *)(counts + 4 * j);
    const double sumX = (double)(c.y + 2 * c.z);
    const double nona = (double)(c.x + c.y + c.z);
    const double af = sumX / (2.0 * nona);
    center[j] = 2.0 * af;
    scale[j] = sqrt(2.0 * af * (1.0 - af));
    s += c.w;
    if (2 * ((int64_t)c.x + c.y + c.z) < n) bad++;
  }
  for (int off = 32; off > 0; off >>= 1) {
    s += __shfl_down(s, off);
    bad += __shfl_down(bad, off);
  }
  __shared__ long long sw[4], sb[4];
  if ((threadIdx.x & 63) == 0) {
    sw[threadIdx.x >> 6] = s;
    sb[threadIdx.x >> 6] = bad;
  }
  __syncthreads();
  if (threadIdx.x == 0) {
    s = sw[0] + sw[1] + sw[2] + sw[3];
    bad = sb[0] + sb[1] + sb[2] + sb[3];
    if (s) atomicAdd(&out[0], (unsigned long long)s);
    if (bad) atomicAdd(&out[1], (unsigned long long)bad);
  }
}
#pragma clang fp contract(on)

static void stats_from_cache(bsn_op *op, bsn_bed *owner, const StatsCols &sel) {
  bsn_bed *b = op->bed;
  int32_t *cnt = op->d_counts.ensure((size_t)4 * op->m + 8);
  stats_cache_load(owner, sel, cnt, b->stream);
  if (!op->h_na_total) BSN_HIP(hipHostMalloc((void **)&op->h_na_total, 2 * sizeof(long long), hipHostMallocDefault));
  op->h_na_total[0] = -1;
  op->h_na_total[1] = -1;
  unsigned long long *d_tot = (unsigned long long *)(cnt + 4 * op->m);
  BSN_HIP(hipMemsetAsync(d_tot, 0, 16, b->stream));
  int gx = (int)((op->m + 1023) / 1024);
  if (gx > 1024) gx = 1024;
  hipLaunchKernelGGL(k_scale_from_counts, dim3(gx), dim3(256), 0, b->stream, cnt, op->m, op->n, op->d_center.p,
                     op->d_scale.p, d_tot);
  BSN_HIP(hipGetLastError());
  BSN_HIP(hipMemcpyAsync(op->h_na_total, d_tot, 16, hipMemcpyDeviceToHost, b->stream));
}

static const int32_t *owner_cols_device(bsn_bed *owner, bsn_bed *sub, const int64_t *cols, int64_t m) {
  auto &sc = owner->stats_cache;
  if (sc.cols_key == 0 || sc.cols_key != owner->sub_key || (int64_t)sc.d_cols.n < m) {
    std::vector<int32_t> c32((size_t)m);
    for (int64_t j = 0; j < m; j++) {
      if (cols[j] < 0 || cols[j] >= owner->m) fail("internal: variant %lld of %lld in a compacted solve", (long long)cols[j], (long long)owner->m);
      c32[(size_t)j] = (int32_t)cols[j];
    }
    copy_h2d(sub, sc.d_cols.ensure((size_t)m), c32.data(), (size_t)m * 4);
    sc.cols_key = owner->sub_key;
  }
  return sc.d_cols.p;
}

static bsn_bed *compacted_view(bsn_bed *bed, const int64_t *ind_row, int64_t n, const int64_t *ind_col, int64_t m) {
  if (!ind_col || m < 2 || bed->bits != 2 || bed->generic || bed->streamed() || getenv("BSN_NO_COMPACT")) return nullptr;
  bool contig = true;
  for (int64_t j = 1; j < m && contig; j++) contig = ind_col[j] == ind_col[0] + j;
  if (contig) return nullptr;
  const int64_t pitch = round_up((n + 3) / 4, 256);
  const double bytes = (double)(m + 64) * (double)pitch;
  double min_bytes = 256e6;
  if (const char *e = getenv("BSN_COMPACT_MIN_BYTES")) min_bytes = atof(e);
  if (bytes < min_bytes) return nullptr;
  uint64_t key = 1469598103934665603ull;
  auto mix = [&](const int64_t *p, size_t count) {
    for (size_t i = 0; i < count; i++) {
      key = (key ^ (uint64_t)p[i]) * 1099511628211ull;
      key ^= key >> 29;
    }
  };
  mix(&n, 1);
  mix(&m, 1);
  mix(ind_col, (size_t)m);
  bool rows_ident = n == bed->n;
  if (ind_row)
    for (int64_t i = 0; rows_ident && i < n; i++) rows_ident = ind_row[i] == i;
  if (!rows_ident && ind_row) mix(ind_row, (size_t)n);
  if (key == 0) key = 1;
  const bool keep_rows = !rows_ident && ind_row;
  if (bed->sub && bed->sub_key == key && bed->sub->n == n && bed->sub->m == m && (int64_t)bed->sub_cols.size() == m &&
      std::memcmp(bed->sub_cols.data(), ind_col, (size_t)m * 8) == 0 &&
      (keep_rows ? ((int64_t)bed->sub_rows.size() == n && std::memcmp(bed->sub_rows.data(), ind_row, (size_t)n * 8) == 0)
                 : bed->sub_rows.empty()))
    return bed->sub;
  BSN_HIP(hipSetDevice(bed->device));
  const bool in_place = bed->sub && bed->sub->n == n && bed->sub->cap_m >= m;
  if (!in_place) {
    if (bed->sub) {
      bed_free(bed->sub);
      bed->sub = nullptr;
      bed->sub_key = 0;
      bed->sub_cols.clear();
      bed->sub_rows.clear();
    }
    size_t free_b = 0, total_b = 0;
    BSN_HIP(hipMemGetInfo(&free_b, &total_b));
    if ((double)(free_b + dev_cache_held()) < 2.0 * bytes + 3000.0 * (double)(n + m) + 2e9) return nullptr;
  }
  bsn_bed *fresh = nullptr;
  try {
    fresh = image_gather(bed, rows_ident ? nullptr : ind_row, n, ind_col, m, in_place ? bed->sub : nullptr);
  } catch (const std::exception &) {
    if (in_place) {
      bed->sub_key = 0;
      bed->sub_cols.clear();
      bed->sub_rows.clear();
      throw;
    }
    (void)hipGetLastError();
    return nullptr;
  }
  bed->sub = fresh;
  bed->sub_key = key;
  bed->stats_cache.cols_key = 0;
  bed->sub_cols.assign(ind_col, ind_col + m);
  if (keep_rows) bed->sub_rows.assign(ind_row, ind_row + n);
  else bed->sub_rows.clear();
  return fresh;
}

extern "C" int bsn_bed_randomsvd(bsn_bed *bed, const int64_t *ind_row, int64_t n,
                                 const int64_t *ind_col, int64_t m, const double *center,
                                 const double *scale, const bsn_svd_options *o, double *d, double *u,
                                 double *v, bsn_svd_info *info) {
  bool unconverged = false;
  int rc = guarded([&] {
    if (!o) fail("options must not be NULL");
    if (o->k < 1) fail("'k' must be at least 1.");
    RoctxRange whole("bsn_bed_randomsvd");
    auto t_begin = std::chrono::steady_clock::now();
    auto since = [&]() {
      return std::chrono::duration<double, std::milli>(std::chrono::steady_clock::now() - t_begin).count();
    };
    const bool ooc = bed->streamed();
    if (ooc) {
      if (o->comm || o->allreduce) fail("an out-of-core handle cannot be one shard of a sharded solve: shard the file instead");
      bool all_rows = n == bed->n;
      for (int64_t i = 0; all_rows && ind_row && i < n; i++) all_rows = ind_row[i] == i;
      bool all_cols = m == bed->m, in_order = true;
      for (int64_t j = 0; ind_col && j < m; j++) {
        if (ind_col[j] != j) all_cols = false;
        if (ind_col[j] < 0 || ind_col[j] >= bed->m) fail("Tested %lld < %lld. Subscript out of bounds (ind.col).", (long long)ind_col[j], (long long)bed->m);
        if (j > 0 && ind_col[j] <= ind_col[j - 1]) in_order = false;
      }
      if (!all_rows || !in_order)
        fail("bed_randomSVD on an out-of-core handle (the file's image does not fit the device: it streams its file) "
             "covers all samples, and its variants in increasing file order; a subset small enough for the device is served "
             "by a handle of its own (snp_subset / bsn_bed_subset_payload)");
      ind_row = nullptr;
      if (all_cols) ind_col = nullptr;
    }
    bool compacted = false;
    double t_compact = 0.0;
    bed->last_solve_on_sub = false;
    bsn_bed *const owner = bed;
    const int64_t *const owner_cols = ind_col;
    bool rows_all = !ooc && n == bed->n;
    for (int64_t i = 0; rows_all && ind_row && i < n; i++) rows_all = ind_row[i] == i;
    const bool use_stats_cache = o->binom_scaling && rows_all && stats_cache_enabled(owner);
    if (bsn_bed *sub = compacted_view(bed, ind_row, n, ind_col, m)) {
      bed->last_solve_on_sub = true;
      if (ind_row == nullptr && n != bed->n) fail("internal: row count of a compacted solve");
      bed = sub;
      ind_row = nullptr;
      ind_col = nullptr;
      compacted = true;
      t_compact = since();
    }
    struct Lend {
      bsn_bed *bed;
      std::unique_ptr<bsn_op> op;
      ~Lend() { bed->svd_op = std::move(op); }
    } lend{bed, std::move(bed->svd_op)};
    if (!lend.op) lend.op.reset(new bsn_op());
    bsn_op *op = lend.op.get();
    op->passes = 0;
    op->prof_kind_override = -1;
    for (const void *&pk : op->prof_kernel) pk = nullptr;
    op->stats_pending = false;
    op->na_poll = false;
    op->no_na = false;
    if (!bed->svd_ws) bed->svd_ws = std::make_shared<SvdWorkspace>();
    int32_t n_bad = 0;
    bool fused = false, served = false;
    StatsCols sel{nullptr, nullptr, 0, m};
    if (o->binom_scaling) {
      fill_op(op, bed, ind_row, n, ind_col, m, nullptr, nullptr, true, ooc);
      if (use_stats_cache) {
        if (compacted) sel = StatsCols{owner_cols, owner_cols_device(owner, bed, owner_cols, m), 0, m};
        else if (!op->cols_contig) sel = StatsCols{ind_col, op->d_cols.p, 0, m};
        else sel.col0 = op->col0;
        served = op->rows_identity && stats_cache_known(owner, sel);
      }
      if (served) {
        fused = true;
        stats_from_cache(op, owner, sel);
        if (compacted && !getenv("BSN_FORCE_NA_PLANE")) {
          bool all0 = (int64_t)owner->na_cnt.size() == owner->m;
          for (int64_t j = 0; all0 && j < m; j++) all0 = owner->na_cnt[(size_t)owner_cols[j]] == 0;
          op->no_na = all0;
        }
      } else if (op->rows_identity) {
        op->stats_pending = true;
        op->no_na = false;
        fused = true;
      } else {
        std::vector<int32_t> cnt((size_t)4 * m);
        counts_host(bed, ind_row, n, ind_col, m, cnt.data());
        std::vector<double> ce, sc;
        binom_scale_host(cnt, n, m, ce, sc, &n_bad);
        copy_h2d(bed, op->d_center.p, ce.data(), (size_t)m * 8);
        copy_h2d(bed, op->d_scale.p, sc.data(), (size_t)m * 8);
        if (o->center_out) std::copy(ce.begin(), ce.end(), o->center_out);
        if (o->scale_out) std::copy(sc.begin(), sc.end(), o->scale_out);
      }
    } else {
      fill_op(op, bed, ind_row, n, ind_col, m, center, scale, false, ooc);
    }
    const double t_create = since();
    op->profile = true;
    if (o->slices > 7) fail("slices must be in 1..7");
    HipSvdBackend bk(*bed->svd_ws);
    bk.op = op;
    bk.ooc = ooc;
    bk.ooc_cols = ooc ? ind_col : nullptr;
    bk.st = bed->stream;
    bk.n = n;
    bk.m_local = m;
    bk.m_total = o->m_total > 0 ? o->m_total : m;
    bk.hook = o->comm ? nullptr : o->allreduce;
    bk.ctx = o->allreduce_ctx;
    bk.comm = o->comm;
    bk.rank = o->hook_rank;
    bk.world = o->hook_world > 0 ? o->hook_world : 1;
    bk.kmax = o->k;
    if (bk.comm && bk.comm->device != bed->device) fail("the communicator was created on another device");
    if (bk.hook && (bk.rank < 0 || bk.rank >= bk.world)) fail("hook_rank %d of %d", bk.rank, bk.world);
    bk.setup_ranks();
    bk.timing = getenv("BSN_TIMING") != nullptr;
    bk.speculate = getenv("BSN_NO_SPECULATION") == nullptr;
    bk.no_fused = getenv("BSN_NO_FUSED_STEP") != nullptr;
    bk.fused_stats = fused && !served;
    bk.warm_den = o->warm_denominator >= 2 ? o->warm_denominator : 16;
    int64_t dim = bk.n < bk.m_total ? bk.n : bk.m_total;
    if (o->k > dim) fail("'k' is larger than the dimensions of the matrix.");
    SvdOptions so;
    so.k = o->k;
    so.tol = o->tol > 0 ? o->tol : 1e-4;
    {
      int s_tol = 2;
      while (s_tol < 7 && 1.2 * std::ldexp(1.0, -8 * s_tol) > so.tol / 4) s_tol++;
      if (o->slices > 0) s_tol = o->slices;
      const int b1 = std::max(1, std::min(8, 16 / s_tol)), b2 = std::max(b1, std::min(kMaxB, 32 / s_tol));
      const bool warm_on = o->warm_start >= 0 && bk.m_total / bk.warm_den >= 16384;
      int bb = o->block > 0 ? (o->block > kMaxB ? kMaxB : o->block) : (4 * o->k >= 7 * b1 && warm_on ? b2 : b1);
      int ss = s_tol;
      if (o->slices <= 0) {
        const int nb = (bb * s_tol + 15) / 16;
        ss = std::max(s_tol, std::min(7, 16 * nb / bb));
      }
      so.block = bb;
      op->slices = ss;
      double vf = o->vec_floor;
      if (vf == 0.0) vf = o->slices > 0 ? -1.0 : 1e-7;
      if (const char *e = getenv("BSN_VEC_FLOOR")) vf = atof(e);
      so.slices_base = ss;
      so.slices_max = ss;
      so.vec_floor = 0.0;
      if (vf > 0) {
        int sm = ss;
        while (sm < 7 && 1.2 * std::ldexp(1.0, -8 * sm) > vf) sm++;
        so.slices_max = sm;
        so.vec_floor = vf;
      }
      so.slices_start = o->slices > 0 ? 0 : 1;
      if (const char *e = abl_getenv("BSN_START_SLICES")) so.slices_start = atoi(e);
      so.noise_gain = (fused && abl_getenv("BSN_ZQ_SPLIT")) ? std::sqrt((double)n) : 0.0;
    }
    bool have_smaj = false;
    const bool wants_smaj = so.block * so.slices_max > 16 && op->cols_contig && (op->col0 & 511) == 0 && m >= 4096;
    bool smaj_after = false;
    if (wants_smaj) {
      if (bk.dist || getenv("BSN_SMAJ_SYNC")) have_smaj = image_smaj(bed);
      else if (bed->d_smaj || bed->smaj_job) have_smaj = image_smaj_poll(bed) || bed->smaj_job != nullptr;
      else have_smaj = smaj_after = !bed->smaj_tried && bed->bits == 2 && !getenv("BSN_NO_SMAJ");
    }
    if (!have_smaj && so.block * so.slices_base <= 16 && op->cols_contig && (op->col0 & 63) == 0 && m >= 4096) image_tile(bed);
    so.resid_floor = 1.2 * std::ldexp(1.0, -8 * op->slices);
    so.warm = o->warm_start < 0 ? 0 : (o->warm_start == 0 ? 2 : o->warm_start);
    so.max_basis = o->max_basis;
    so.max_restarts = o->max_restarts == 0 ? 100 : o->max_restarts;
    so.seed = o->seed ? o->seed : 1;
    so.verbose = o->verbose;
    BSN_HIP(hipEventRecord(bed->ev0, bed->stream));
    int wd_ms = o->exchange_timeout_ms;
    if (wd_ms == 0)
      if (const char *e = getenv("BSN_EXCHANGE_TIMEOUT_MS")) wd_ms = atoi(e);
    ExchangeWatchdog watchdog(bk.comm, wd_ms);
    if (bk.comm && wd_ms > 0) bk.progress = [&watchdog] { watchdog.kick(); };
    if (bk.comm) {
      double junk_ms[kCommClasses];
      int junk_n[kCommClasses];
      bk.comm->timing = o->exchange_timing != 0;
      comm_time_collect(bk.comm, junk_ms, junk_n);
    }
    struct TimingOff {
      bsn_comm *c;
      ~TimingOff() { if (c) c->timing = false; }
    } timing_off{bk.comm};
    SvdResult r;
    try {
      r = block_lanczos_svd(bk, so, d, u, v);
    } catch (const std::exception &ex) {
      {
        double pms[kProfKinds];
        int pc[kProfKinds];
        prof_collect(op, pms, pc);
      }
      if (watchdog.fired.load())
        fail("the exchange of the sharded solve did not finish within %d ms (exchange: %s) and the communicator was aborted; "
             "what the solve saw: %s", wd_ms,
             bk.exchange_mode == 3 ? "segments, reduce-scatters on a second stream" : bk.exchange_mode == 2 ? "segments, one stream"
             : getenv("BSN_NO_SEGMENTS") ? "whole pass" : getenv("BSN_NO_OVERLAP") ? "segments, one stream" : "segments, reduce-scatters on a second stream",
             ex.what());
      throw;
    }
    if (((r.exhausted && r.exhausted_resid > 1e-9) || r.below_resolution > 0) && o->slices <= 0 && op->slices < 7) {
      if (o->verbose)
        std::fprintf(stderr, "[bsn svd] %s on %d-bit products (relative residual %.3g, %d requested triplets below their resolution): "
                             "again with 56-bit products\n", r.exhausted ? "Krylov space exhausted" : "triplets below the products' resolution",
                     8 * op->slices, r.max_rel_resid, r.below_resolution);
      op->slices = 7;
      so.slices_base = so.slices_max = 7;
      so.vec_floor = 0.0;
      so.block = std::min(so.block, 32 / 7);
      so.resid_floor = 1.2 * std::ldexp(1.0, -8 * op->slices);
      const SvdResult r1 = r;
      r = block_lanczos_svd(bk, so, d, u, v);
      r.niter += r1.niter;
      r.nops += r1.nops;
      r.restarts += r1.restarts;
    }
    const double t_solve = since() - t_create;
    if (o->verbose > 1 || bk.timing)
      std::fprintf(stderr,
                   "[bsn svd] host wall ms: op_create %.2f, solve %.2f = alloc %.2f + A'Q %.2f + AZ %.2f + grams %.2f + "
                   "orth %.2f (GPU events %.2f) + round %.2f + finalize %.2f + host algebra %.2f\n",
                   t_create, t_solve, bk.t_phase[0], bk.t_phase[1], bk.t_phase[2], bk.t_phase[3], bk.t_phase[4],
                   bk.t_phase[7], bk.t_phase[5], bk.t_phase[6],
                   t_solve - (bk.t_phase[0] + bk.t_phase[1] + bk.t_phase[2] + bk.t_phase[3] + bk.t_phase[4] +
                              bk.t_phase[5] + bk.t_phase[6]));
    BSN_HIP(hipEventRecord(bed->ev1, bed->stream));
    BSN_HIP(hipEventSynchronize(bed->ev1));
    float ms = 0;
    BSN_HIP(hipEventElapsedTime(&ms, bed->ev0, bed->ev1));
    if (fused && !served) {
      SvdWorkspace &ws = *bed->svd_ws;
      const int64_t chunk = 1 << 21;
      int32_t *hp = (int32_t *)ws.pinned((size_t)chunk / 2);
      if ((int64_t)bed->na_cnt.size() != bed->m) bed->na_cnt.assign((size_t)bed->m, -1);
      const bool feed = use_stats_cache && !op->stats_pending && op->m == m && (int64_t)op->d_counts.n >= 4 * m;
      if (feed) stats_cache_store(owner, sel, op->d_counts.p, bed->stream);
      if (feed && compacted && (int64_t)owner->na_cnt.size() != owner->m) owner->na_cnt.assign((size_t)owner->m, -1);
      for (int64_t j0 = 0; j0 < m; j0 += chunk) {
        const int64_t cnt = std::min<int64_t>(chunk, m - j0);
        BSN_HIP(hipMemcpyAsync(hp, op->d_na.p + j0, (size_t)cnt * 4, hipMemcpyDeviceToHost, bed->stream));
        BSN_HIP(hipStreamSynchronize(bed->stream));
        if (ind_col) {
          for (int64_t j = 0; j < cnt; j++) bed->na_cnt[(size_t)ind_col[j0 + j]] = hp[j];
        } else {
          std::memcpy(&bed->na_cnt[(size_t)j0], hp, (size_t)cnt * 4);
        }
        if (feed && compacted)
          for (int64_t j = 0; j < cnt; j++) owner->na_cnt[(size_t)owner_cols[j0 + j]] = hp[j];
      }
    }
    if (fused) {
      if (op->h_na_total && op->h_na_total[1] >= 0) n_bad += (int32_t)op->h_na_total[1];
      if (o->center_out) copy_d2h(bed, o->center_out, op->d_center.p, (size_t)m * 8);
      if (o->scale_out) copy_d2h(bed, o->scale_out, op->d_scale.p, (size_t)m * 8);
    }
    if (r.converged && r.below_resolution > 0) {
      unconverged = true;
      r.converged = 0;
      char buf[320];
      std::snprintf(buf, sizeof(buf),
                    "%d of the %d requested singular triplets lie below what %d-bit products resolve (sigma below %.1e sigma_1): "
                    "their values are not converged; ask for more digits (slices) or fewer triplets",
                    r.below_resolution, so.k, 8 * op->slices, std::sqrt(64.0) * so.resid_floor);
      set_error(buf);
    } else if (!r.converged) {
      unconverged = true;
      char buf[256];
      std::snprintf(buf, sizeof(buf),
                    "the Krylov basis is full (%d vectors) but only a relative residual of %.3g (tol %.3g) was "
                    "reached for the %d requested singular triplets; increase max_basis or tol",
                    r.basis, r.max_rel_resid, so.tol, so.k);
      set_error(buf);
    }
    if (info) {
      info->n_bad = n_bad;
      info->fused_stats = fused ? 1 : 0;
      info->niter = r.niter;
      info->nops = (int32_t)op->passes;
      info->basis = r.basis;
      info->converged = r.converged;
      info->max_rel_resid = r.max_rel_resid;
      info->gpu_ms = ms;
      double pms[kProfKinds];
      int pc[kProfKinds];
      prof_collect(op, pms, pc);
      if (bk.sop) {
        double p2[kProfKinds];
        int c2[kProfKinds];
        prof_collect(bk.sop.get(), p2, c2);
        for (int t = 0; t < kProfKinds; t++) {
          pms[t] += p2[t];
          pc[t] += c2[t];
          if (bk.sop->prof_kernel[t]) op->prof_kernel[t] = bk.sop->prof_kernel[t];
        }
      }
      info->wide_cprod_ms = pms[4];
      info->wide_prod_ms = pms[5];
      info->n_wide_cprod = pc[4];
      info->n_wide_prod = pc[5];
      info->slices_max = r.slices_used_max > 0 ? r.slices_used_max : so.slices_base;
      info->wide_steps = r.wide_steps;
      info->lead_rel_resid = r.lead_rel_resid;
      info->cprod_ms = pms[0];
      info->prod_ms = pms[1];
      info->n_cprod = pc[0];
      info->n_prod = pc[1];
      info->cprod_stats_ms = pms[2];
      info->n_cprod_stats = pc[2];
      info->warm_ms = pms[3];
      info->warm_launches = bk.warm_launches;
      info->warm_fraction = bk.m_sub > 0 && bk.m_op_full > 0 ? (double)bk.m_sub / (double)bk.m_op_full : 0.0;
      info->block = so.block;
      info->slices = so.slices_base;
      info->tiled = (bed->d_tiled != nullptr && op->cols_contig && (op->col0 & 63) == 0) ? 1 : 0;
      if (bed->d_smaj != nullptr && so.block * so.slices_max > 16 && so.block * so.slices_max <= 48 && op->cols_contig &&
          (op->col0 & 511) == 0)
        info->tiled = 2;
      info->segmented_passes = bk.n_seg_passes;
      info->compact_gathers = bk.n_compact_gathers;
      info->out_of_core = ooc ? 1 : 0;
      info->na_free_steps[0] = op->bed->na_free[0];
      info->na_free_steps[1] = op->bed->na_free[1];
      info->na_skip = (op->na_skip_c ? 1 : 0) | (op->na_skip_p ? 2 : 0);
      info->compacted = compacted ? 1 : 0;
      info->compact_ms = t_compact;
      info->exchange_mode = bk.exchange_mode;
      for (int c = 0; c < 4; c++) info->exchange_ms[c] = 0, info->n_exchange[c] = 0;
      if (bk.comm && o->exchange_timing) {
        double ems[kCommClasses];
        int en[kCommClasses];
        comm_time_collect(bk.comm, ems, en);
        for (int c = 0; c < 4 && c < kCommClasses; c++) info->exchange_ms[c] = ems[c], info->n_exchange[c] = en[c];
      }
    }
    if (smaj_after && !bed->d_smaj && !bed->smaj_job) (void)image_smaj_start(bed);
  });
  return rc != 0 ? rc : (unconverged ? 2 : 0);
}
```

bigsnpr_amd/csrc/svd_driver.hpp:

```cpp
#pragma once
#include <string>
#include <stdexcept>
#include <cmath>
#include <cstdint>
#include <cstdio>
#include <vector>

#include "dense_small.hpp"

namespace bsn {

struct SvdBackend {
  int64_t n = 0, m_local = 0, m_total = 0;
  virtual ~SvdBackend() {}
  virtual void alloc(int cap, int b) = 0;
  virtual void random_W(int b, uint32_t seed) = 0;
  virtual void At_Qblock(int p0, int cb) = 0;
  virtual void A_Zblock(int p0, int cb) = 0;
  virtual void QtW(int p, int cb, double *C) = 0;
  virtual void W_minus_QC(int p, int cb, const double *C) = 0;
  virtual void WtW(int cb, double *G) = 0;
  virtual void W_times(int cb, int r, const double *M) = 0;
  virtual void W_to_Q(int p0, int r) = 0;
  virtual void round_W(int cb) = 0;
  virtual void ZtZ(int p, int p0, int cb, double *G) = 0;
  virtual void QtQ(int p, int p0, int cb, double *M) = 0;
  virtual int orth_fused(int p, int cb, std::vector<double> &Cacc, std::vector<double> &Rout) {
    (void)p; (void)cb; (void)Cacc; (void)Rout;
    return -1;
  }
  virtual int step_fused(int p, int p0, int cb, double *blkZ, double *blkQ, std::vector<double> &Rout) {
    (void)p; (void)p0; (void)cb; (void)blkZ; (void)blkQ; (void)Rout;
    return -1;
  }
  virtual bool restart(int pp, int keep, const double *S, int rn, const double *Mk) {
    (void)pp; (void)keep; (void)S; (void)rn; (void)Mk;
    return false;
  }
  virtual void set_precision(int slices) { (void)slices; }
  virtual void hold_rounding(bool hold) { (void)hold; }
  virtual bool subset(bool on) {
    (void)on;
    return false;
  }
  virtual void finalize(int pp, int k, const double *S, const double *dinv, double *u,
                        double *v) = 0;
};

struct SvdOptions {
  int k = 10;
  double tol = 1e-4;
  int block = 8;
  int max_basis = 0;
  uint32_t seed = 1;
  int verbose = 0;
  int warm = 0;
  double resid_floor = 0.0;
  int max_restarts = 100;
  int slices_base = 0;
  int slices_max = 0;
  int slices_start = 0;
  double vec_floor = 0.0;
  double noise_gain = 0.0;
};

struct SvdResult {
  int niter = 0;
  int nops = 0;
  int basis = 0;
  int converged = 0;
  int warm = 0;
  int restarts = 0;
  int exhausted = 0;
  double exhausted_resid = 0;
  double max_rel_resid = 0;
  double lead_rel_resid = 0;
  int wide_steps = 0;
  int slices_used_max = 0;
  int below_resolution = 0;
};

inline SvdResult block_lanczos_svd(SvdBackend &bk, const SvdOptions &opt, double *d, double *u,
                                   double *v) {
  const int k = opt.k;
  int b = opt.block;
  {
    const int64_t small = bk.n < bk.m_total ? bk.n : bk.m_total;
    if (b > small) b = (int)small;
  }
  const int64_t dim = bk.n < bk.m_total + b ? bk.n : bk.m_total + b;
  int cap = opt.max_basis > 0 ? opt.max_basis : std::max(8 * k + 4 * b, 320);
  if (cap > dim) cap = (int)dim;
  if (cap < k) cap = k;
  bk.alloc(cap + b, b);

  std::vector<double> Gz((size_t)cap * cap, 0.0), Mq((size_t)cap * cap, 0.0);
  auto Gat = [&](int i, int j) -> double & { return Gz[(size_t)i + (size_t)j * cap]; };
  auto Mat = [&](int i, int j) -> double & { return Mq[(size_t)i + (size_t)j * cap]; };
  std::vector<double> C, C2, G, R, Ri, R2, Rt, evec, eval, M, blk, blk2;
  SvdResult res;

  const double defic = 1e-22;
  auto orth = [&](int p, int cb, std::vector<double> &Cacc, std::vector<double> &Rout, bool try_fused = true) -> int {
    if (try_fused) {
      const int rf = bk.orth_fused(p, cb, Cacc, Rout);
      if (rf >= 0) return rf;
    }
    Cacc.assign((size_t)p * cb, 0.0);
    G.assign((size_t)cb * cb, 0.0);
    bk.WtW(cb, G.data());
    double w0 = 0;
    for (int i = 0; i < cb; i++) w0 = std::max(w0, G[(size_t)i + (size_t)i * cb]);
    for (int pass = 0; pass < 8 && p > 0; pass++) {
      C.assign((size_t)p * cb, 0.0);
      bk.QtW(p, cb, C.data());
      bk.W_minus_QC(p, cb, C.data());
      for (size_t t = 0; t < C.size(); t++) Cacc[t] += C[t];
      if (pass < 1) continue;
      G.assign((size_t)cb * cb, 0.0);
      bk.WtW(cb, G.data());
      bool clean = true;
      for (int j = 0; j < cb && clean; j++) {
        const double left = G[(size_t)j + (size_t)j * cb];
        if (!(left > defic * w0)) continue;
        double c2 = 0;
        for (int a = 0; a < p; a++) c2 += C[(size_t)a + (size_t)j * p] * C[(size_t)a + (size_t)j * p];
        clean = c2 <= 1e-24 * left;
      }
      if (clean) break;
    }
    Rout.assign((size_t)cb * cb, 0.0);
    for (int i = 0; i < cb; i++) Rout[(size_t)i + (size_t)i * cb] = 1.0;
    int r = cb;
    for (int pass = 0; pass < 2; pass++) {
      G.assign((size_t)r * r, 0.0);
      bk.WtW(r, G.data());
      if (pass == 0) {
        int keep = 0;
        while (keep < r && G[(size_t)keep + (size_t)keep * r] > defic * w0 && w0 > 0) keep++;
        if (keep < r) {
          std::vector<double> G2((size_t)keep * keep);
          for (int j = 0; j < keep; j++)
            for (int i = 0; i < keep; i++) G2[(size_t)i + (size_t)j * keep] = G[(size_t)i + (size_t)j * r];
          G.swap(G2);
          r = keep;
        }
      }
      if (r == 0) return 0;
      int rk = chol_upper(r, G, R, pass == 0 ? defic : 1e-22);
      const int rc = r;
      std::vector<double> Rrows;
      if (rk < r) {
        Rrows.assign((size_t)rk * rc, 0.0);
        for (int j = 0; j < rc; j++)
          for (int i = 0; i < rk; i++) Rrows[(size_t)i + (size_t)j * rk] = R[(size_t)i + (size_t)j * rc];
        std::vector<double> G2((size_t)rk * rk);
        for (int j = 0; j < rk; j++)
          for (int i = 0; i < rk; i++) G2[(size_t)i + (size_t)j * rk] = G[(size_t)i + (size_t)j * r];
        r = rk;
        if (r == 0) return 0;
        chol_upper(r, G2, R, 0.0);
      }
      inv_upper(r, R, Ri);
      bk.W_times(r, r, Ri.data());
      std::vector<double> Rn((size_t)cb * cb, 0.0);
      for (int j = 0; j < cb; j++)
        for (int i = 0; i < r; i++) {
          double s = 0;
          if (Rrows.empty()) {
            for (int t = i; t < r; t++) s += R[(size_t)i + (size_t)t * r] * Rout[(size_t)t + (size_t)j * cb];
          } else {
            for (int t = i; t < rc; t++) s += Rrows[(size_t)i + (size_t)t * r] * Rout[(size_t)t + (size_t)j * cb];
          }
          Rn[(size_t)i + (size_t)j * cb] = s;
        }
      Rout.swap(Rn);
      if (pass == 0 && p > 0) {
        for (int again = 0; again < 6; again++) {
          C.assign((size_t)p * r, 0.0);
          bk.QtW(p, r, C.data());
          bk.W_minus_QC(p, r, C.data());
          double cmax = 0;
          for (size_t t = 0; t < C.size(); t++) cmax = std::max(cmax, std::fabs(C[t]));
          if (cmax <= 1e-12) break;
        }
      }
    }
    return r;
  };

  const bool sched = opt.slices_base > 0 && opt.slices_max > opt.slices_base && opt.vec_floor > 0;
  const int klead = (k + 1) / 2;
  double rho_lead = 1.0, z_gain = 1.0;
  auto step_slices = [&](const double gain) -> int {
    int S = opt.slices_base;
    if (sched) {
      const double rho = rho_lead < 1.0 ? rho_lead : 1.0;
      while (S < opt.slices_max && 1.2 * std::ldexp(1.0, -8 * S) * rho * gain > opt.vec_floor) S++;
    }
    return S;
  };
  if (opt.slices_base > 0) bk.set_precision(opt.slices_start > 0 ? opt.slices_start : opt.slices_base);
  bk.random_W(b, opt.seed);
  int r = orth(0, b, C2, Rt);
  for (int w = 0; w < opt.warm && r > 0; w++) {
    if (!bk.subset(true)) break;
    bk.round_W(r);
    bk.W_to_Q(0, r);
    bk.At_Qblock(0, r);
    bk.A_Zblock(0, r);
    bk.subset(false);
    res.warm++;
    r = orth(0, r, C2, Rt);
  }
  bk.round_W(r);
  bk.W_to_Q(0, r);
  int p = r;
  int cb = r;
  int pp = 0;
  std::vector<double> Rlast;
  int rr_rank = 0;
  int rl_rows = 0, rl_cols = 0;
  int exhausted_restarts = 0;

  while (cb > 0) {
    const int p0 = p - cb;
    bk.At_Qblock(p0, cb);
    int S_next = 0;
    if (opt.slices_base > 0) {
      const int Sz = step_slices(z_gain);
      S_next = step_slices(1.0);
      bk.set_precision(Sz);
      if (S_next > opt.slices_base || Sz > opt.slices_base) res.wide_steps++;
      if (std::max(Sz, S_next) > res.slices_used_max) res.slices_used_max = std::max(Sz, S_next);
      if (opt.verbose)
        std::fprintf(stderr, "[bsn svd] step %d: %d-bit product pass, next block on %d bits (leading residual %.2e, product weight %.3f)\n",
                     res.niter + 1, 8 * Sz, 8 * S_next, rho_lead, z_gain);
    }
    bk.A_Zblock(p0, cb);
    const bool hold = sched && S_next > opt.slices_base;
    if (opt.slices_base > 0) {
      bk.set_precision(S_next);
      bk.hold_rounding(hold);
    }
    res.nops += 2;
    res.niter++;
    blk.assign((size_t)p * cb, 0.0);
    blk2.assign((size_t)p * cb, 0.0);
    int rn = bk.step_fused(p, p0, cb, blk.data(), blk2.data(), Rt);
    const bool fused_failed = rn == -2;
    if (rn == -1) {
      bk.ZtZ(p, p0, cb, blk.data());
      bk.QtQ(p, p0, cb, blk2.data());
    }
    for (size_t t = 0; t < blk.size(); t++)
      if (!std::isfinite(blk[t]) || !std::isfinite(blk2[t]))
        throw std::runtime_error("the projected matrices of the partial SVD hold NaN or Inf: non-finite values in the matrix, "
                                 "its centre or scale (a scale of 0?), or entries whose squares overflow");
    if (res.niter == 1) {
      double gmax = 0;
      for (int j = 0; j < cb; j++) gmax = std::max(gmax, std::fabs(blk[(size_t)(p0 + j) + (size_t)j * p]));
      if (gmax > 1e140 || (gmax > 0 && gmax < 1e-140))
        throw std::runtime_error("the matrix of the partial SVD is of the order of 1e" +
                                 std::to_string((int)std::lround(0.5 * std::log10(gmax))) +
                                 ": outside 1e-70 .. 1e70 its Gram matrices overflow or underflow in double precision; rescale it "
                                 "(center / scale of the operator) and scale d back");
    }
    for (int j = 0; j < cb; j++)
      for (int i = 0; i < p; i++) Gat(i, p0 + j) = Gat(p0 + j, i) = blk[(size_t)i + (size_t)j * p];
    for (int j = 0; j < cb; j++)
      for (int i = 0; i < p; i++) Mat(i, p0 + j) = Mat(p0 + j, i) = blk2[(size_t)i + (size_t)j * p];
    for (int j = 0; j < cb; j++)
      for (int i = 0; i < j; i++) {
        double a = 0.5 * (Gat(p0 + i, p0 + j) + Gat(p0 + j, p0 + i));
        Gat(p0 + i, p0 + j) = Gat(p0 + j, p0 + i) = a;
        a = 0.5 * (Mat(p0 + i, p0 + j) + Mat(p0 + j, p0 + i));
        Mat(p0 + i, p0 + j) = Mat(p0 + j, p0 + i) = a;
      }
    if (rn < 0) rn = orth(p, cb, C2, Rt, !fused_failed);
    if ((int64_t)p + rn > bk.n) rn = bk.n > p ? (int)(bk.n - p) : 0;
    pp = p;
    const bool exhausted = (rn == 0) || (p >= dim);
    Rlast.assign((size_t)rn * cb, 0.0);
    for (int j = 0; j < cb; j++)
      for (int i = 0; i < rn; i++) Rlast[(size_t)i + (size_t)j * rn] = Rt[(size_t)i + (size_t)j * cb];
    rl_rows = rn;
    rl_cols = cb;
    const int rn_full = rn;
    const bool by_count = p >= dim;
    const bool want_restart = rn > cap - p && rn > 0 && pp >= k && res.restarts < opt.max_restarts &&
                              (!by_count || exhausted_restarts < 2);
    if (rn > cap - p) rn = cap - p;
    if (rn < 0) rn = 0;

    if (pp >= (sched ? std::min(k, klead) : k) || rn == 0 || exhausted || want_restart) {
      std::vector<double> Mp((size_t)pp * pp), Gp((size_t)pp * pp), Rm, Rmi, tmp((size_t)pp * pp);
      for (int j = 0; j < pp; j++)
        for (int i = 0; i < pp; i++) {
          Mp[(size_t)i + (size_t)j * pp] = Mat(i, j);
          Gp[(size_t)i + (size_t)j * pp] = Gat(i, j);
        }
      int rk = chol_upper(pp, Mp, Rm, 1e-14);
      if (opt.verbose > 1) {
        double dev = 0;
        for (int j = 0; j < pp; j++)
          for (int i = 0; i < pp; i++) dev = std::max(dev, std::fabs(Mat(i, j) - (i == j ? 1.0 : 0.0)));
        std::fprintf(stderr, "[bsn svd]   Q'Q: max |M - I| = %.3e, Cholesky rank %d of %d\n", dev, rk, pp);
      }
      rr_rank = pp;
      if (rk == pp) {
        inv_upper(pp, Rm, Rmi);
        small_mm(pp, pp, pp, Gp.data(), Rmi.data(), tmp.data());
        evec.assign((size_t)pp * pp, 0.0);
        for (int j = 0; j < pp; j++)
          for (int i = 0; i <= j; i++) {
            double a = 0;
            for (int t = 0; t <= i; t++) a += Rmi[(size_t)t + (size_t)i * pp] * tmp[(size_t)t + (size_t)j * pp];
            evec[(size_t)i + (size_t)j * pp] = a;
            evec[(size_t)j + (size_t)i * pp] = a;
          }
        eig_sym(pp, evec, eval);
        small_mm(pp, pp, pp, Rmi.data(), evec.data(), tmp.data());
        evec.swap(tmp);
      } else {
        std::vector<double> V(Mp), lam;
        eig_sym(pp, V, lam);
        const double lmax = lam[pp - 1];
        int r = 0;
        while (r < pp && lam[pp - 1 - r] > 1e-8 * lmax && lmax > 0) r++;
        std::vector<double> T((size_t)pp * std::max(r, 1), 0.0), GT((size_t)pp * std::max(r, 1)), B((size_t)r * r), bl;
        for (int c = 0; c < r; c++) {
          const double f = 1.0 / std::sqrt(lam[pp - 1 - c]);
          for (int i = 0; i < pp; i++) T[(size_t)i + (size_t)c * pp] = V[(size_t)i + (size_t)(pp - 1 - c) * pp] * f;
        }
        small_mm(pp, pp, r, Gp.data(), T.data(), GT.data());
        for (int j = 0; j < r; j++)
          for (int i = 0; i <= j; i++) {
            double a = 0;
            for (int t = 0; t < pp; t++) a += T[(size_t)t + (size_t)i * pp] * GT[(size_t)t + (size_t)j * pp];
            B[(size_t)i + (size_t)j * r] = B[(size_t)j + (size_t)i * r] = a;
          }
        eig_sym(r, B, bl);
        rr_rank = r;
        eval.assign((size_t)pp, 0.0);
        evec.assign((size_t)pp * pp, 0.0);
        for (int c = 0; c < r; c++) {
          const int col = pp - r + c;
          eval[(size_t)col] = bl[(size_t)c];
          for (int i = 0; i < pp; i++) {
            double a = 0;
            for (int t = 0; t < r; t++) a += T[(size_t)i + (size_t)t * pp] * B[(size_t)t + (size_t)c * r];
            evec[(size_t)i + (size_t)col * pp] = a;
          }
        }
        if (opt.verbose)
          std::fprintf(stderr, "[bsn svd]   dependent basis: %d of %d directions kept for the Rayleigh-Ritz step\n", r, pp);
      }
    }
    bool done = false;
    const double hard_zero = 1e-10;
    const double negligible = std::max(hard_zero, 64.0 * opt.resid_floor * opt.resid_floor);
    double worst_sig = 0;
    if (pp >= k) {
      double worst = 0, lead = 0;
      int n_soft = 0;
      for (int t = 0; t < k; t++) {
        int col = pp - 1 - t;
        double theta = eval[col];
        double rs = 0;
        for (int i = 0; i < rl_rows; i++) {
          double s = 0;
          for (int j = 0; j < rl_cols; j++)
            s += Rlast[(size_t)i + (size_t)j * rl_rows] * evec[(size_t)(pp - rl_cols + j) + (size_t)col * pp];
          rs += s * s;
        }
        double rel = std::sqrt(rs) / std::max(std::fabs(theta), 1e-300);
        worst = std::max(worst, rel);
        if (t < klead) lead = std::max(lead, rel);
        if (theta > negligible * eval[pp - 1]) worst_sig = std::max(worst_sig, rel);
        else if (theta > hard_zero * eval[pp - 1]) n_soft++;
      }
      res.below_resolution = n_soft;
      worst = worst_sig;
      res.max_rel_resid = worst;
      res.lead_rel_resid = lead;
      rho_lead = lead;
      if (opt.noise_gain > 0) {
        const double th1 = eval[pp - 1], thh = eval[pp - klead];
        z_gain = thh > 0 ? std::min(1.0, opt.noise_gain * std::sqrt(std::max(th1, 0.0)) / thh) : 1.0;
      }
      if (opt.verbose)
        std::fprintf(stderr, "[bsn svd] step %d basis %d max rel resid %.3e sigma1 %.6g\n", res.niter,
                     pp, worst, std::sqrt(std::max(eval[pp - 1], 0.0)));
      if (worst + opt.resid_floor <= opt.tol) {
        done = true;
        res.converged = 1;
      }
    }
    if (sched && pp < k && pp >= klead && !eval.empty()) {
      double lead = 0;
      for (int t = 0; t < klead; t++) {
        const int col = pp - 1 - t;
        double rs = 0;
        for (int i = 0; i < rl_rows; i++) {
          double s = 0;
          for (int j = 0; j < rl_cols; j++)
            s += Rlast[(size_t)i + (size_t)j * rl_rows] * evec[(size_t)(pp - rl_cols + j) + (size_t)col * pp];
          rs += s * s;
        }
        lead = std::max(lead, std::sqrt(rs) / std::max(std::fabs(eval[col]), 1e-300));
      }
      rho_lead = lead;
      if (opt.noise_gain > 0) {
        const double th1 = eval[pp - 1], thh = eval[pp - klead];
        z_gain = thh > 0 ? std::min(1.0, opt.noise_gain * std::sqrt(std::max(th1, 0.0)) / thh) : 1.0;
      }
      if (opt.verbose) std::fprintf(stderr, "[bsn svd] step %d basis %d leading-half rel resid %.3e\n", res.niter, pp, lead);
    }
    if (hold) {
      const int S = step_slices(1.0);
      bk.set_precision(S);
      if (S > res.slices_used_max) res.slices_used_max = S;
      if (opt.verbose) std::fprintf(stderr, "[bsn svd] step %d: next block on %d bits (leading residual %.2e)\n", res.niter, 8 * S, rho_lead);
    }
    if (!done && want_restart) {
      int keep = std::min(std::min(pp, rr_rank), k + b);
      if (keep > cap - rn_full) keep = cap - rn_full;
      if (keep >= k) {
        std::vector<double> Sk((size_t)pp * keep);
        for (int t = 0; t < keep; t++)
          for (int i = 0; i < pp; i++) Sk[(size_t)i + (size_t)t * pp] = evec[(size_t)i + (size_t)(pp - 1 - t) * pp];
        std::vector<double> Gk((size_t)keep * keep), Mk((size_t)keep * keep), tG((size_t)pp * keep), tM((size_t)pp * keep);
        {
          std::vector<double> Mp((size_t)pp * pp), Gp((size_t)pp * pp);
          for (int j = 0; j < pp; j++)
            for (int i = 0; i < pp; i++) {
              Mp[(size_t)i + (size_t)j * pp] = Mat(i, j);
              Gp[(size_t)i + (size_t)j * pp] = Gat(i, j);
            }
          small_mm(pp, pp, keep, Gp.data(), Sk.data(), tG.data());
          small_mm(pp, pp, keep, Mp.data(), Sk.data(), tM.data());
          for (int j = 0; j < keep; j++)
            for (int i = 0; i <= j; i++) {
              double g = 0, mm = 0;
              for (int t = 0; t < pp; t++) {
                g += Sk[(size_t)t + (size_t)i * pp] * tG[(size_t)t + (size_t)j * pp];
                mm += Sk[(size_t)t + (size_t)i * pp] * tM[(size_t)t + (size_t)j * pp];
              }
              Gk[(size_t)i + (size_t)j * keep] = Gk[(size_t)j + (size_t)i * keep] = g;
              Mk[(size_t)i + (size_t)j * keep] = Mk[(size_t)j + (size_t)i * keep] = mm;
            }
        }
        if (bk.restart(pp, keep, Sk.data(), rn_full, Mk.data())) {
          for (int j = 0; j < cap; j++)
            for (int i = 0; i < cap; i++) Gat(i, j) = Mat(i, j) = 0.0;
          for (int j = 0; j < keep; j++)
            for (int i = 0; i < keep; i++) {
              Gat(i, j) = Gk[(size_t)i + (size_t)j * keep];
              Mat(i, j) = Mk[(size_t)i + (size_t)j * keep];
            }
          res.restarts++;
          if (by_count) exhausted_restarts++;
          if (opt.verbose)
            std::fprintf(stderr, "[bsn svd] basis full at %d: restart with %d Ritz vectors\n", pp, keep);
          p = keep;
          pp = keep;
          rn = rn_full;
          bk.round_W(rn);
          bk.W_to_Q(p, rn);
          p += rn;
          cb = rn;
          continue;
        }
      }
    }
    if (done || rn == 0) {
      if (exhausted) {
        res.exhausted = 1;
        res.exhausted_resid = worst_sig;
      }
      if (exhausted && !done) {
        res.converged = (worst_sig + opt.resid_floor <= opt.tol) ? 1 : 0;
      }
      break;
    }
    bk.round_W(rn);
    bk.W_to_Q(p, rn);
    p += rn;
    cb = rn;
  }

  res.basis = pp;
  int kk = k < pp ? k : pp;
  std::vector<double> S((size_t)pp * k, 0.0), dinv((size_t)k, 0.0);
  for (int t = 0; t < k; t++) {
    d[t] = 0;
    if (t < kk) {
      int col = pp - 1 - t;
      double th = eval[col] > 0 ? eval[col] : 0;
      d[t] = std::sqrt(th);
      dinv[t] = d[t] > 0 ? 1.0 / d[t] : 0.0;
      for (int i = 0; i < pp; i++) S[(size_t)i + (size_t)t * pp] = evec[(size_t)i + (size_t)col * pp];
    }
  }
  bk.finalize(pp, k, S.data(), dinv.data(), u, v);
  return res;
}

}
```

bigsnpr_amd/svd.py:

```python
import ctypes as C
import warnings

import numpy as np

from . import _lib
from ._lib import check, f64p, i64p, ptr
from .bed import _args, assert_bed, bed_scaleBinom


def bed_randomSVD(obj_bed, fun_scaling=bed_scaleBinom, ind_row=None, ind_col=None, k=10,
                  tol=1e-4, verbose=False, ncores=1, block=0, slices=0, max_basis=0, seed=1,
                  comm=None, allreduce=None, rank=0, world=1, m_total=0, return_uv=True, warm_start=0, warm_denominator=0,
                  max_restarts=0, vec_floor=0.0, exchange_timing=False, exchange_timeout_ms=0):
    assert_bed(obj_bed)
    ir, ic = _args(obj_bed, ind_row, ind_col)
    opts = _lib.SvdOptions()
    if fun_scaling is bed_scaleBinom:
        center, scale = np.empty(ic.size), np.empty(ic.size)
        opts.binom_scaling = 1
        opts.center_out, opts.scale_out = ptr(center, f64p), ptr(scale, f64p)
    else:
        ms = fun_scaling(obj_bed, ind_row=ir, ind_col=ic, ncores=ncores)
        center = np.ascontiguousarray(ms["center"], dtype=np.float64)
        scale = np.ascontiguousarray(ms["scale"], dtype=np.float64)
    opts.k, opts.tol, opts.block, opts.slices = int(k), float(tol), int(block), int(slices)
    opts.warm_start, opts.warm_denominator = int(warm_start), int(warm_denominator)
    opts.max_restarts = int(max_restarts)
    opts.vec_floor = float(vec_floor)
    opts.exchange_timing, opts.exchange_timeout_ms = int(bool(exchange_timing)), int(exchange_timeout_ms)
    opts.max_basis, opts.seed, opts.verbose, opts.m_total = int(max_basis), int(seed), int(verbose), int(m_total)
    cb = None
    if comm is not None:
        opts.comm = comm.handle
    elif allreduce is not None:
        cb = _lib.ALLREDUCE_FN(lambda p, count, ctx: allreduce(p, count))
        opts.allreduce = cb
        opts.hook_rank, opts.hook_world = int(rank), int(world)
    info = _lib.SvdInfo()
    d = np.empty(k)
    big = k * (ir.size + ic.size) * 8 >= (8 << 20)
    alloc = _lib.result_pool.empty if big else np.empty
    u = alloc((k, ir.size)) if return_uv else None
    v = alloc((k, ic.size)) if return_uv else None
    L = _lib.load()
    rc = L.bsn_bed_randomsvd(obj_bed.handle, ptr(ir, i64p), ir.size, ptr(ic, i64p), ic.size,
                             ptr(center, f64p), ptr(scale, f64p), C.byref(opts), ptr(d, f64p),
                             ptr(u, f64p), ptr(v, f64p), C.byref(info))
    _lib.result_pool.kick()
    if rc == 2:
        warnings.warn("bed_randomSVD did not converge: " + L.bsn_last_error().decode(), RuntimeWarning)
    else:
        check(rc)
    if info.n_bad > 0:
        warnings.warn("%d variants have >50%% missing values." % info.n_bad)
    return dict(d=d, u=None if u is None else u.T, v=None if v is None else v.T,
                niter=info.niter, nops=info.nops, center=center, scale=scale,
                basis=info.basis, converged=bool(info.converged),
                max_rel_resid=info.max_rel_resid, gpu_ms=info.gpu_ms,
                cprod_ms=info.cprod_ms, prod_ms=info.prod_ms, n_cprod=info.n_cprod,
                n_prod=info.n_prod, block=info.block, slices=info.slices,
                fused_stats=bool(info.fused_stats), cprod_stats_ms=info.cprod_stats_ms,
                n_cprod_stats=info.n_cprod_stats, warm_launches=info.warm_launches,
                warm_fraction=info.warm_fraction, warm_ms=info.warm_ms, tiled=int(info.tiled),
                segmented_passes=int(info.segmented_passes), compact_gathers=int(info.compact_gathers),
                slices_max=int(info.slices_max), wide_steps=int(info.wide_steps),
                wide_cprod_ms=info.wide_cprod_ms, wide_prod_ms=info.wide_prod_ms,
                n_wide_cprod=int(info.n_wide_cprod), n_wide_prod=int(info.n_wide_prod),
                lead_rel_resid=info.lead_rel_resid, compacted=bool(info.compacted), compact_ms=info.compact_ms,
                out_of_core=bool(info.out_of_core),
                na_free_steps=[float(x) for x in info.na_free_steps], na_skip=int(info.na_skip),
                exchange_mode=("none", "whole pass", "segments, one stream", "segments, reduce-scatters on a second stream")[
                    max(0, min(3, int(info.exchange_mode)))],
                exchange_ms=dict(zip(("reduce_scatter", "all_gather", "small", "exposed_wait"), [float(x) for x in info.exchange_ms])),
                n_exchange=dict(zip(("reduce_scatter", "all_gather", "small", "exposed_wait"), [int(x) for x in info.n_exchange])))
```

include/bigsnpr_hip.h:

```cpp
#ifndef BIGSNPR_HIP_H
#define BIGSNPR_HIP_H

#include <stdint.h>

#ifdef __cplusplus
extern "C" {
#endif

typedef struct bsn_bed bsn_bed;
typedef struct bsn_op bsn_op;

const char *bsn_last_error(void);
int bsn_version(void);
int bsn_device_count(int *count);
int bsn_set_device(int device);
int bsn_selftest(void);

int bsn_bed_open(const char *path, int64_t n, int64_t m, bsn_bed **out);
int bsn_bed_is_streamed(const bsn_bed *bed);
int bsn_bed_from_host(const uint8_t *payload, int64_t n, int64_t m, int64_t n_byte, bsn_bed **out);
int bsn_bed_from_fbm(const uint8_t *bytes, int64_t n, int64_t m, int64_t ld, bsn_bed **out);
int bsn_fbm_open(const uint8_t *bytes, int64_t n, int64_t m, int64_t ld, const double *code256, bsn_bed **out);
int bsn_bed_bits(const bsn_bed *bed);
int64_t bsn_bed_na_known(const bsn_bed *bed);
int bsn_bed_synthetic(int64_t n, int64_t m, uint32_t seed, uint32_t npop, uint32_t na16,
                      int64_t j_begin, bsn_bed **out);
int bsn_bed_close(bsn_bed *bed);
int64_t bsn_bed_nrow(const bsn_bed *bed);
int64_t bsn_bed_ncol(const bsn_bed *bed);
int64_t bsn_bed_bytes(const bsn_bed *bed);
int bsn_bed_download(bsn_bed *bed, uint8_t *payload_out);

int bsn_bed_prodvec(bsn_bed *bed, const int64_t *ind_row, int64_t n, const int64_t *ind_col,
                    int64_t m, const double *center, const double *scale, const double *x,
                    double *y);
int bsn_bed_cprodvec(bsn_bed *bed, const int64_t *ind_row, int64_t n, const int64_t *ind_col,
                     int64_t m, const double *center, const double *scale, const double *x,
                     double *z);

struct bsn_comm;
int bsn_bed_prodvec_sharded(bsn_bed *bed, const int64_t *ind_row, int64_t n, const int64_t *ind_col,
                            int64_t m, const double *center, const double *scale, const double *x,
                            struct bsn_comm *comm, double *y);
int bsn_bed_col_counts(bsn_bed *bed, const int64_t *ind_row, int64_t n, const int64_t *ind_col,
                       int64_t m, int32_t *res);
int bsn_bed_row_counts(bsn_bed *bed, const int64_t *ind_row, int64_t n, const int64_t *ind_col, int64_t m,
                       int32_t *res);
int bsn_bed_colstats(bsn_bed *bed, const int64_t *ind_row, int64_t n, const int64_t *ind_col,
                     int64_t m, double *sumX, double *denoX, int32_t *nb_nona_col, int32_t *n_bad);
int bsn_snp_colstats(bsn_bed *bed, const int64_t *ind_row, int64_t n, const int64_t *ind_col,
                     int64_t m, double *sumX, double *denoX);
int bsn_bed_read(bsn_bed *bed, const int64_t *ind_row, int64_t n, const int64_t *ind_col,
                 int64_t m, int32_t na_val, int32_t *out);
int bsn_bed_read_scaled(bsn_bed *bed, const int64_t *ind_row, int64_t n, const int64_t *ind_col,
                        int64_t m, const double *center, const double *scale, double *out);

int bsn_bed_cprod_planes(bsn_bed *bed, const int64_t *ind_row, int64_t n, const int64_t *ind_col,
                         int64_t m, const double *X, int64_t K, double *P, double *Q);

int bsn_mult_lin_reg(bsn_bed *bed, const int64_t *ind_row, int64_t n, const int64_t *ind_col, int64_t m,
                     const double *U, int64_t K, double *res);

int bsn_univ_linreg(bsn_bed *bed, const int64_t *ind_row, int64_t n, const int64_t *ind_col, int64_t m, const double *y,
                    const double *U, int64_t K, double *estim, double *std_err);
int bsn_univ_logreg(bsn_bed *bed, const int64_t *ind_row, int64_t n, const int64_t *ind_col, int64_t m, const double *y01,
                    const double *covar, int64_t q, double tol, int32_t maxiter, double *estim, double *std_err,
                    int32_t *niter);

int bsn_impute_simple(bsn_bed *src, int method, uint64_t seed, bsn_bed **out, uint8_t *fbm_bytes_out ,
                      int64_t *n_all_missing );
int bsn_impute_last_ms(double *ms_out);

int bsn_bed_prod_and_rowsumssq(bsn_bed *bed, const int64_t *ind_row, int64_t n, const int64_t *ind_col,
                               int64_t m, const double *center, const double *scale, const double *V,
                               int64_t K, double *XV, double *rowSumsSq);

int bsn_snp_prod_and_rowsumssq2(bsn_bed *bed, const int64_t *ind_row, int64_t n, const int64_t *ind_col,
                                int64_t m, const double *center, const double *scale, const double *V,
                                int64_t K, double *XV, double *rowSumsSq);

int bsn_snp_grid_prs(bsn_bed *bed, const int64_t *ind_row, int64_t n, const int64_t *ind_col, int64_t m,
                     const double *betas, const int32_t *bin, const uint8_t *member, int64_t C, int64_t T,
                     int slices, double *out);

int bsn_bed_to_fbm(bsn_bed *bed, const int64_t *ind_row, int64_t n, const int64_t *ind_col, int64_t m,
                   uint8_t *out);
int bsn_bed_readbina(bsn_bed *bed, const uint8_t *tab, uint8_t *out);
int bsn_bed_subset_payload(bsn_bed *bed, const int64_t *ind_row, int64_t n, const int64_t *ind_col,
                           int64_t m, uint8_t *payload_out);

int bsn_op_create(bsn_bed *bed, const int64_t *ind_row, int64_t n, const int64_t *ind_col,
                  int64_t m, const double *center, const double *scale, bsn_op **out);
int bsn_op_destroy(bsn_op *op);
int bsn_op_set_slices(bsn_op *op, int slices);
int bsn_op_prod(bsn_op *op, const double *d_X, int64_t ldx, int nvec, double *d_Y, int64_t ldy);
int bsn_op_cprod(bsn_op *op, const double *d_X, int64_t ldx, int nvec, double *d_Z, int64_t ldz);
int bsn_op_sync(bsn_op *op);

typedef void (*bsn_allreduce_fn)(void *d_buf, int64_t count, void *ctx);

#define BSN_COMM_ID_BYTES 128
typedef struct bsn_comm bsn_comm;
int bsn_comm_unique_id(uint8_t *id_out );
int bsn_comm_init(const uint8_t *id, int rank, int world, bsn_comm **out);
int bsn_comm_rank(const bsn_comm *comm);
int bsn_comm_world(const bsn_comm *comm);
int bsn_comm_allreduce(bsn_comm *comm, double *d_buf, int64_t count);
int bsn_comm_abort(bsn_comm *comm);
int bsn_comm_destroy(bsn_comm *comm);
typedef struct bsn_svd_options {
  int32_t k;
  double tol;
  int32_t block;
  int32_t slices;
  int32_t max_basis;
  uint32_t seed;
  int32_t verbose;
  int64_t m_total;
  bsn_allreduce_fn allreduce;
  void *allreduce_ctx;
  int32_t hook_rank, hook_world;
  struct bsn_comm *comm;
  int32_t binom_scaling;
  double *center_out, *scale_out;
  int32_t warm_start;
  int32_t warm_denominator;
  int32_t max_restarts;
  double vec_floor;
  int32_t exchange_timing;
  int32_t exchange_timeout_ms;
} bsn_svd_options;
typedef struct bsn_svd_info {
  int32_t niter;
  int32_t nops;
  int32_t basis;
  int32_t converged;
  double max_rel_resid;
  double gpu_ms;
  double cprod_ms;
  double prod_ms;
  int32_t n_cprod, n_prod;
  int32_t block, slices;
  int32_t n_bad;
  int32_t fused_stats;
  double cprod_stats_ms;
  int32_t n_cprod_stats;
  int32_t warm_launches;
  double warm_fraction;
  double warm_ms;
  int32_t tiled;
  int32_t segmented_passes;
  int32_t compact_gathers;
  int32_t slices_max, wide_steps;
  double wide_cprod_ms, wide_prod_ms;
  int32_t n_wide_cprod, n_wide_prod;
  double lead_rel_resid;
  int32_t exchange_mode;
  int32_t n_exchange[4];
  double exchange_ms[4];
  int32_t compacted;
  double compact_ms;
  int32_t out_of_core;
  double na_free_steps[2];
  int32_t na_skip;
} bsn_svd_info;
int bsn_bed_randomsvd(bsn_bed *bed, const int64_t *ind_row, int64_t n, const int64_t *ind_col,
                      int64_t m, const double *center, const double *scale,
                      const bsn_svd_options *options, double *d, double *u, double *v,
                      bsn_svd_info *info);
int bsn_bed_streaming_kernels(bsn_bed *bed, char *buf, int64_t len);
int bsn_op_last_kernel(bsn_op *op, char *buf, int64_t len);
int bsn_bed_tile(bsn_bed *bed, int *built);
int bsn_bed_sample_major(bsn_bed *bed, int *built);

int bsn_bed_release_workspace(bsn_bed *bed);

int bsn_bed_tcrossprod(bsn_bed *bed, const int64_t *ind_row, int64_t n, const int64_t *ind_col,
                       int64_t m, const double *center, const double *scale, int64_t block_size,
                       double *K);

typedef struct bsn_cor bsn_cor;
int bsn_cormat(bsn_bed *bed, const int64_t *ind_row, int64_t n, const int64_t *ind_col, int64_t m,
               double size, const double *thr, const double *pos, int fill_diag, int32_t *p_out,
               int64_t *nnz_out, bsn_cor **out);
int bsn_cormat_fetch(bsn_cor *cor, int32_t *i_out, double *x_out);
int bsn_cormat_has_nan(const bsn_cor *cor, int *out);
int bsn_cormat_free(bsn_cor *cor);
int bsn_ld_last_stats(double *out );
int bsn_ld_scores(bsn_bed *bed, const int64_t *ind_row, int64_t n, const int64_t *ind_col, int64_t m,
                  double size, const double *pos, double *out);
int bsn_clumping_chr(bsn_bed *bed, const int64_t *ind_row, int64_t n, const int64_t *ind_col,
                     int64_t m, int mode, const double *aux1, const double *aux2,
                     const int32_t *ordInd, const int32_t *rankInd, const double *pos, double size,
                     double thr, int32_t *keep);
int bsn_clumping_chr_cached(bsn_bed *bed, const int64_t *ind_row, int64_t n, const int64_t *ind_col,
                            int64_t m, int mode, const double *aux1, const double *aux2,
                            const int32_t *ordInd, const int32_t *rankInd, const double *pos,
                            int64_t n_grid, const double *sizes, const double *thrs, int32_t *keep);

int bsn_robust_scale_tau2(const double *d_X, int64_t m, int64_t ld, int32_t ncol, double c1, double c2, double *mu_out, double *s_out);
int bsn_robust_pair_scales(const double *d_Z, int64_t m, int64_t ld, int32_t p, double c1, double c2, double *s_sum_out, double *s_diff_out);
int bsn_robust_mc_count(const double *d_up, int64_t nu, const double *d_lo, int64_t nl, double t, int64_t *count_out);
int bsn_robust_scale_cols(double *d_Z, int64_t m, int64_t ld, int32_t p, const double *div );
int bsn_robust_rotate(double *d_Z, int64_t m, int64_t ld, int32_t p, const double *E );
int bsn_robust_wdist(const double *d_Z, int64_t m, int64_t ld, int32_t p, const double *mu, const double *sig, double *out);
int bsn_robust_dist_ogk(const double *d_U, int64_t m, int64_t ld, int32_t p, int32_t niter, double cut_ratio, double c1, double c2,
                        double *dist_out, int64_t *n_kept_out);
int bsn_robust_rollmean(const double *x, int64_t m, const double *w, int32_t len, const int64_t *group_off, int32_t ngroups, double *out);
int bsn_robust_sort(double *x, int64_t m);
int bsn_robust_mc_window(const double *d_up, int64_t nu, const double *d_lo, int64_t nl, double a, double b, int64_t cap, double *out,
                         int64_t *count_out);

int bsn_order_decreasing(const double *S, int64_t m, const int64_t *group_off, int32_t ngroups, int32_t *ord, int32_t *rank);

typedef struct bsn_sfbm bsn_sfbm;
int bsn_sfbm_from_csc(const int64_t *p, const int32_t *i, const double *x, int64_t m2, int upper, bsn_sfbm **out);
int bsn_sfbm_ncol(const bsn_sfbm *s, int64_t *m2_out, int64_t *nnz_out, int64_t *bandwidth_out);
int bsn_sfbm_free(bsn_sfbm *s);
int bsn_lassosum2(const bsn_sfbm *s, const double *beta_hat, int64_t m, const double *pf, const double *lambda,
                  const double *delta, int64_t G, const int64_t *ind_sub, double dfmax, int32_t maxiter, double tol,
                  double *beta_out, int32_t *num_iter_out, double *time_out);
int bsn_ldpred2_gibbs(const bsn_sfbm *s, const double *beta_hat, const double *n_vec, int64_t m, const int64_t *ind_sub,
                      const double *h2, const double *p, const int32_t *sparse, const uint64_t *stream, int64_t G, int burn_in,
                      int num_iter, uint64_t seed, double *beta_out, double *seconds_out);
int bsn_ldpred2_gibbs_sampling(const bsn_sfbm *s, const double *beta_hat, const double *n_vec, int64_t m, const int64_t *ind_sub,
                               double h2, double p, int32_t sparse, uint64_t stream, int burn_in, int num_iter, uint64_t seed,
                               double *sample_out, double *seconds_out);
int bsn_ldpred2_auto(const bsn_sfbm *s, const double *beta_hat, const double *n_vec, const double *log_var, int64_t m,
                     const int64_t *ind_sub, const double *p_init, const uint64_t *stream, int64_t G, double h2_init,
                     int burn_in, int num_iter, int report_step, int no_jump_sign, double shrink_corr, int use_mle,
                     double p_lo, double p_hi, double alpha_lo, double alpha_hi, double mean_ld, uint64_t seed,
                     double *beta_est, double *postp_est, double *corr_est, double *sample_beta,
                     double *path_p, double *path_h2, double *path_alpha, double *seconds_out);

int bsn_sfbm_prodvec(bsn_sfbm *s, const double *x, const int64_t *ind_sub, int64_t m, double *y_out);
int bsn_sfbm_ld_scores(bsn_sfbm *s, const int64_t *ind_sub, int64_t m, double *out);
int bsn_sfbm_solve_sym(bsn_sfbm *s, const double *b, const double *add_to_diag, const int64_t *ind_sub, int64_t m, double tol,
                       int32_t maxiter, double *x_out, int32_t *iters_out, double *relres_out);
int bsn_sfbm_last_ms(const bsn_sfbm *s, double *ms_out);

int bsn_malloc(void **d_ptr, int64_t bytes);
int bsn_free(void *d_ptr);
int bsn_host_alloc(void **h_ptr, int64_t bytes);
int bsn_host_free(void *h_ptr);
int bsn_memcpy_h2d(void *d_dst, const void *src, int64_t bytes);
int bsn_memcpy_d2h(void *dst, const void *d_src, int64_t bytes);
int bsn_device_sync(void);
int bsn_timer_start(bsn_bed *bed);
int bsn_timer_stop(bsn_bed *bed, double *ms);

#ifdef __cplusplus
}
#endif
#endif
```

Before: 37.57 million.

## Compute Gram blocks early and speculatively finalize Ritz vectors during product pass

```diff
diff --git a/bigsnpr_amd/_lib.py b/bigsnpr_amd/_lib.py
--- a/bigsnpr_amd/_lib.py
+++ b/bigsnpr_amd/_lib.py
@@ -41,7 +41,8 @@
                 ("wide_prod_ms", C.c_double), ("n_wide_cprod", C.c_int32), ("n_wide_prod", C.c_int32),
                 ("lead_rel_resid", C.c_double), ("exchange_mode", C.c_int32), ("n_exchange", C.c_int32 * 4),
                 ("exchange_ms", C.c_double * 4), ("compacted", C.c_int32), ("compact_ms", C.c_double),
-                ("out_of_core", C.c_int32), ("na_free_steps", C.c_double * 2), ("na_skip", C.c_int32)]
+                ("out_of_core", C.c_int32), ("na_free_steps", C.c_double * 2), ("na_skip", C.c_int32),
+                ("early_ritz", C.c_int32 * 2)]
 
 
 SIGNATURES = {
diff --git a/bigsnpr_amd/csrc/api.hip b/bigsnpr_amd/csrc/api.hip
--- a/bigsnpr_amd/csrc/api.hip
+++ b/bigsnpr_amd/csrc/api.hip
@@ -314,7 +314,7 @@
   return b->stream_up;
 }
 
-static bool host_is_pinned(const void *p) {
+bool host_is_pinned(const void *p) {
   hipPointerAttribute_t at;
   if (hipPointerGetAttributes(&at, p) != hipSuccess) {
     (void)hipGetLastError();
diff --git a/bigsnpr_amd/csrc/bsn_internal.hpp b/bigsnpr_amd/csrc/bsn_internal.hpp
--- a/bigsnpr_amd/csrc/bsn_internal.hpp
+++ b/bigsnpr_amd/csrc/bsn_internal.hpp
@@ -302,6 +302,7 @@
 void copy_h2d(bsn_bed *b, void *d_dst, const void *src, size_t bytes, hipStream_t stream = nullptr);
 hipStream_t upload_stream(bsn_bed *b);
 void copy_d2h(bsn_bed *b, void *dst, const void *d_src, size_t bytes);
+bool host_is_pinned(const void *p);
 
 void fill_op(bsn_op *op, bsn_bed *bed, const int64_t *ind_row, int64_t n, const int64_t *ind_col,
              int64_t m, const double *center, const double *scale, bool defer_scale = false,
diff --git a/bigsnpr_amd/csrc/svd.hip b/bigsnpr_amd/csrc/svd.hip
--- a/bigsnpr_amd/csrc/svd.hip
+++ b/bigsnpr_amd/csrc/svd.hip
@@ -381,6 +381,9 @@
   double *h_pin = nullptr;
   size_t h_pin_n = 0;
   hipEvent_t ev_small = nullptr;
+  hipEvent_t ev_early = nullptr, ev_guess_up = nullptr;
+  double *h_guess = nullptr;
+  size_t h_guess_n = 0;
   hipStream_t st_comm = nullptr;
   hipEvent_t ev_seg[8] = {nullptr, nullptr, nullptr, nullptr, nullptr, nullptr, nullptr, nullptr};
   hipEvent_t ev_arrived = nullptr;
@@ -403,6 +406,9 @@
     if (ev_arrived) (void)hipEventDestroy(ev_arrived);
     if (st_comm) (void)hipStreamDestroy(st_comm);
     if (ev_small) (void)hipEventDestroy(ev_small);
+    if (ev_early) (void)hipEventDestroy(ev_early);
+    if (ev_guess_up) (void)hipEventDestroy(ev_guess_up);
+    if (h_guess) (void)hipHostFree(h_guess);
     if (h_pin) (void)hipHostFree(h_pin);
   }
 };
@@ -430,6 +436,24 @@
   bool no_fused = false;
   bool speculate = true;
   bool spec_rounded = false;
+  bool early_on = false;
+  bool grams_early = false;
+  double *eg_Z = nullptr, *eg_Q = nullptr;
+  int eg_p = 0, eg_cb = 0;
+  bool guess_live = false;
+  bool guess_inflight = false;
+  int guess_pp = 0, guess_k = 0;
+  double *guess_u = nullptr, *guess_v = nullptr;
+  std::vector<double> guess_S, guess_dinv;
+  int n_guess = 0, guess_used = 0;
+  void guess_wait() {
+    if (!guess_inflight) return;
+    BSN_HIP(hipStreamSynchronize(upload_stream(op->bed)));
+    guess_inflight = false;
+  }
+  ~HipSvdBackend() {
+    if (guess_inflight && op && op->bed && op->bed->stream_up) (void)hipStreamSynchronize(op->bed->stream_up);
+  }
   int n_small_ar = 0;
   int64_t m_op_full = 0, m_sub = 0;
   bool fused_stats = false;
@@ -560,6 +584,8 @@
     wcol = 0;
     mx_valid = false;
     spec_rounded = false;
+    guess_live = false;
+    grams_early = false;
     op->preq_X = nullptr;
     hipLaunchKernelGGL(k_random, dim3((unsigned)((nr + 255) / 256), bb), dim3(256), 0, st, Wc, nr, nr, bb, seed,
                        row0, n);
@@ -682,6 +708,7 @@
   void At_Qblock(int p0, int cb) override {
     Tick tk(this, 1);
     if (progress) progress();
+    guess_live = false;
     if (ooc) return At_Qblock_ooc(p0, cb);
     op_cprod(op, newest_block(p0), n, cb, Z.p + (int64_t)p0 * m_local, m_local);
   }
@@ -887,8 +914,10 @@
     const size_t pc = (size_t)p * cb, hg = (size_t)(p + cb) * cb;
     double *flag = dorth.p + 16, *dRout = flag + 1, *dZtZ = dRout + B2, *X = dZtZ + pc, *HG1 = X + (p > 0 ? hg : 0),
            *HG2 = HG1 + hg, *C = HG2 + hg, *Ct = C + pc, *Ri = Ct + pc;
+    const bool have_grams = grams_early && with_grams && p == eg_p && cb == eg_cb;
+    grams_early = false;
     BSN_HIP(hipMemsetAsync(flag, 0, (size_t)(1 + B2) * 8, st));
-    if (p > 0) gemm_tn_any(Z.p, Z.p + (int64_t)p0 * m_local, m_local, p, cb, dZtZ);
+    if (p > 0 && !have_grams) gemm_tn_any(Z.p, Z.p + (int64_t)p0 * m_local, m_local, p, cb, dZtZ);
     BSN_HIP(hipMemcpyAsync(Wsave.p, Wc, (size_t)nr * cb * 8, hipMemcpyDeviceToDevice, st));
     OrthSmall a;
     a.p = p;
@@ -907,7 +936,7 @@
     a.Cs = a.Gs = a.Rs = a.Ris = a.Ro = a.Dv = a.tmp = nullptr;
     for (int pass = 0; pass < 2; pass++) {
       double *HG = pass == 0 ? HG1 : HG2;
-      if (pass == 0 && p > 0) {
+      if (pass == 0 && p > 0 && !have_grams) {
         gemm_tn_any(Q.p, Q.p + (int64_t)p0 * nr, nr, p + cb, 2 * cb, X, p + cb);
         ar_small(dZtZ, (int64_t)(pc + 2 * hg));
       } else {
@@ -995,8 +1024,101 @@
     wcol = p0 + r;
     Wc = Q.p + (int64_t)wcol * nr;
   }
+  double *early_host(size_t *cnt = nullptr) {
+    const size_t half = (size_t)(cap + kMaxB + 4) * kMaxB * 2 + 512;
+    if (cnt) *cnt = half;
+    return ws.pinned(2 * half) + half;
+  }
+  bool early_grams(int p, int p0, int cb, double *blkZ, double *blkQ) override {
+    grams_early = false;
+    if (!early_on || p <= 0 || cb <= 0 || cb > kMaxB || p + cb > kOrthMaxP || p + cb > cap + kMaxB) return false;
+    if (Wc != Q.p + (int64_t)p * nr || p0 + cb != p) return false;
+    Tick tk(this, 3);
+    const size_t pc = (size_t)p * cb, hg = (size_t)(p + cb) * cb;
+    size_t room = 0;
+    double *hp = early_host(&room);
+    if (pc + hg > room) return false;
+    double *dZtZ = dorth.p + 16 + 1 + B2, *X = dZtZ + pc;
+    gemm_tn_any(Z.p, Z.p + (int64_t)p0 * m_local, m_local, p, cb, dZtZ);
+    gemm_tn_any(Q.p, Q.p + (int64_t)p0 * nr, nr, p, cb, X, p + cb);
+    BSN_HIP(hipGetLastError());
+    BSN_HIP(hipMemcpyAsync(hp, dZtZ, (pc + hg) * 8, hipMemcpyDeviceToHost, st));
+    if (!ws.ev_early) BSN_HIP(hipEventCreateWithFlags(&ws.ev_early, hipEventDisableTiming));
+    BSN_HIP(hipEventRecord(ws.ev_early, st));
+    eg_Z = blkZ;
+    eg_Q = blkQ;
+    eg_p = p;
+    eg_cb = cb;
+    grams_early = true;
+    return true;
+  }
+  bool early_grams_wait() override {
+    if (!grams_early) return false;
+    Tick tk(this, 3);
+    BSN_HIP(hipEventSynchronize(ws.ev_early));
+    n_sync++;
+    const double *hp = early_host();
+    const size_t pc = (size_t)eg_p * eg_cb;
+    std::memcpy(eg_Z, hp, pc * 8);
+    for (int j = 0; j < eg_cb; j++)
+      std::memcpy(eg_Q + (size_t)j * eg_p, hp + pc + (size_t)j * (eg_p + eg_cb), (size_t)eg_p * 8);
+    return true;
+  }
+  void prefinalize(int pp, int k, const double *S, const double *dinv, double *u, double *v) override {
+    guess_live = false;
+    if (!S || !early_on || !ws.ev_early || pp <= 0 || pp > cap + kMaxB || k <= 0 || (!u && !v)) return;
+    if ((u && !host_is_pinned(u)) || (v && !host_is_pinned(v))) return;
+    Tick tk(this, 6);
+    hipStream_t up = upload_stream(op->bed);
+    DevBuf<double> &dS = ws.dS, &dU = ws.dU, &dV = ws.dV;
+    const size_t sk = (size_t)pp * k, need_S = (size_t)(cap + kMaxB) * k * 2 + 16;
+    if (need_S > dS.n || (size_t)nr * k > dU.n || (size_t)m_local * k > dV.n) guess_wait();
+    dS.ensure(need_S);
+    dU.ensure((size_t)nr * k);
+    dV.ensure((size_t)m_local * k);
+    if (!ws.ev_guess_up) BSN_HIP(hipEventCreateWithFlags(&ws.ev_guess_up, hipEventDisableTiming));
+    else BSN_HIP(hipEventSynchronize(ws.ev_guess_up));
+    if (2 * sk > ws.h_guess_n) {
+      if (ws.h_guess) (void)hipHostFree(ws.h_guess);
+      ws.h_guess = nullptr;
+      ws.h_guess_n = 0;
+      BSN_HIP(hipHostMalloc((void **)&ws.h_guess, need_S * sizeof(double), hipHostMallocDefault));
+      ws.h_guess_n = need_S;
+    }
+    double *hs = ws.h_guess;
+    std::memcpy(hs, S, sk * 8);
+    for (int t = 0; t < k; t++)
+      for (int i = 0; i < pp; i++) hs[sk + (size_t)i + (size_t)t * pp] = S[(size_t)i + (size_t)t * pp] * dinv[t];
+    guess_inflight = true;
+    BSN_HIP(hipMemcpyAsync(dS.p, hs, 2 * sk * 8, hipMemcpyHostToDevice, up));
+    BSN_HIP(hipEventRecord(ws.ev_guess_up, up));
+    BSN_HIP(hipStreamWaitEvent(up, ws.ev_early, 0));
+    for (int c0 = 0; c0 < k; c0 += kMaxB) {
+      const int nc = k - c0 < kMaxB ? k - c0 : kMaxB;
+      hipLaunchKernelGGL(k_gemm_nn, dim3((unsigned)((nr + 255) / 256)), dim3(256), kTP * kMaxB * 8, up,
+                         Q.p, nr, pp, dS.p + (size_t)c0 * pp, nc, (const double *)nullptr, (int64_t)0,
+                         0.0, 1.0, dU.p + (int64_t)c0 * nr, nr, nr);
+      hipLaunchKernelGGL(k_gemm_nn, dim3((unsigned)((m_local + 255) / 256)), dim3(256),
+                         kTP * kMaxB * 8, up, Z.p, m_local, pp, dS.p + sk + (size_t)c0 * pp,
+                         nc, (const double *)nullptr, (int64_t)0, 0.0, 1.0,
+                         dV.p + (int64_t)c0 * m_local, m_local, m_local);
+    }
+    BSN_HIP(hipGetLastError());
+    if (u) BSN_HIP(hipMemcpyAsync(u, dU.p, (size_t)n * k * 8, hipMemcpyDeviceToHost, up));
+    if (v) BSN_HIP(hipMemcpyAsync(v, dV.p, (size_t)m_local * k * 8, hipMemcpyDeviceToHost, up));
+    guess_pp = pp;
+    guess_k = k;
+    guess_u = u;
+    guess_v = v;
+    guess_S.assign(S, S + sk);
+    guess_dinv.assign(dinv, dinv + k);
+    guess_live = true;
+    n_guess++;
+  }
   bool restart(int pp, int keep, const double *S, int rn, const double *Mk) override {
     if (keep + rn > pp || keep <= 0) return false;
+    guess_live = false;
+    guess_wait();
     DevBuf<double> &dS = ws.dS, &tQ = ws.dU, &tZ = ws.dV;
     dS.ensure((size_t)pp * keep + 16);
     tQ.ensure((size_t)nr * keep);
@@ -1026,6 +1148,17 @@
   }
   void finalize(int pp, int k, const double *S, const double *dinv, double *u, double *v) override {
     Tick tk(this, 6);
+    guess_used = 0;
+    if (guess_live && pp == guess_pp && k == guess_k && u == guess_u && v == guess_v &&
+        std::memcmp(S, guess_S.data(), (size_t)pp * k * 8) == 0 && std::memcmp(dinv, guess_dinv.data(), (size_t)k * 8) == 0) {
+      guess_live = false;
+      guess_wait();
+      guess_used = 1;
+      sync_stream();
+      return;
+    }
+    guess_live = false;
+    guess_wait();
     std::vector<double> Sv((size_t)pp * k);
     for (int t = 0; t < k; t++)
       for (int i = 0; i < pp; i++) Sv[(size_t)i + (size_t)t * pp] = S[(size_t)i + (size_t)t * pp] * dinv[t];
@@ -1386,6 +1519,7 @@
     bk.timing = getenv("BSN_TIMING") != nullptr;
     bk.speculate = getenv("BSN_NO_SPECULATION") == nullptr;
     bk.no_fused = getenv("BSN_NO_FUSED_STEP") != nullptr;
+    bk.early_on = !bk.dist && !ooc && !bk.no_fused && getenv("BSN_NO_EARLY_RITZ") == nullptr;
     bk.fused_stats = fused && !served;
     bk.warm_den = o->warm_denominator >= 2 ? o->warm_denominator : 16;
     int64_t dim = bk.n < bk.m_total ? bk.n : bk.m_total;
@@ -1597,6 +1731,8 @@
       info->compacted = compacted ? 1 : 0;
       info->compact_ms = t_compact;
       info->exchange_mode = bk.exchange_mode;
+      info->early_ritz[0] = bk.n_guess;
+      info->early_ritz[1] = bk.guess_used;
       for (int c = 0; c < 4; c++) info->exchange_ms[c] = 0, info->n_exchange[c] = 0;
       if (bk.comm && o->exchange_timing) {
         double ems[kCommClasses];
diff --git a/bigsnpr_amd/csrc/svd_driver.hpp b/bigsnpr_amd/csrc/svd_driver.hpp
--- a/bigsnpr_amd/csrc/svd_driver.hpp
+++ b/bigsnpr_amd/csrc/svd_driver.hpp
@@ -42,6 +42,14 @@
   virtual bool subset(bool on) {
     (void)on;
     return false;
+  }
+  virtual bool early_grams(int p, int p0, int cb, double *blkZ, double *blkQ) {
+    (void)p; (void)p0; (void)cb; (void)blkZ; (void)blkQ;
+    return false;
+  }
+  virtual bool early_grams_wait() { return false; }
+  virtual void prefinalize(int pp, int k, const double *S, const double *dinv, double *u, double *v) {
+    (void)pp; (void)k; (void)S; (void)dinv; (void)u; (void)v;
   }
   virtual void finalize(int pp, int k, const double *S, const double *dinv, double *u,
                         double *v) = 0;
@@ -223,36 +231,7 @@
   int rl_rows = 0, rl_cols = 0;
   int exhausted_restarts = 0;
 
-  while (cb > 0) {
-    const int p0 = p - cb;
-    bk.At_Qblock(p0, cb);
-    int S_next = 0;
-    if (opt.slices_base > 0) {
-      const int Sz = step_slices(z_gain);
-      S_next = step_slices(1.0);
-      bk.set_precision(Sz);
-      if (S_next > opt.slices_base || Sz > opt.slices_base) res.wide_steps++;
-      if (std::max(Sz, S_next) > res.slices_used_max) res.slices_used_max = std::max(Sz, S_next);
-      if (opt.verbose)
-        std::fprintf(stderr, "[bsn svd] step %d: %d-bit product pass, next block on %d bits (leading residual %.2e, product weight %.3f)\n",
-                     res.niter + 1, 8 * Sz, 8 * S_next, rho_lead, z_gain);
-    }
-    bk.A_Zblock(p0, cb);
-    const bool hold = sched && S_next > opt.slices_base;
-    if (opt.slices_base > 0) {
-      bk.set_precision(S_next);
-      bk.hold_rounding(hold);
-    }
-    res.nops += 2;
-    res.niter++;
-    blk.assign((size_t)p * cb, 0.0);
-    blk2.assign((size_t)p * cb, 0.0);
-    int rn = bk.step_fused(p, p0, cb, blk.data(), blk2.data(), Rt);
-    const bool fused_failed = rn == -2;
-    if (rn == -1) {
-      bk.ZtZ(p, p0, cb, blk.data());
-      bk.QtQ(p, p0, cb, blk2.data());
-    }
+  auto absorb_grams = [&](int p, int p0, int cb) {
     for (size_t t = 0; t < blk.size(); t++)
       if (!std::isfinite(blk[t]) || !std::isfinite(blk2[t]))
         throw std::runtime_error("the projected matrices of the partial SVD hold NaN or Inf: non-finite values in the matrix, "
@@ -277,7 +256,148 @@
         a = 0.5 * (Mat(p0 + i, p0 + j) + Mat(p0 + j, p0 + i));
         Mat(p0 + i, p0 + j) = Mat(p0 + j, p0 + i) = a;
       }
-    if (rn < 0) rn = orth(p, cb, C2, Rt, !fused_failed);
+  };
+
+  auto ritz = [&](int pp) -> int {
+    std::vector<double> Mp((size_t)pp * pp), Gp((size_t)pp * pp), Rm, Rmi, tmp((size_t)pp * pp);
+    for (int j = 0; j < pp; j++)
+      for (int i = 0; i < pp; i++) {
+        Mp[(size_t)i + (size_t)j * pp] = Mat(i, j);
+        Gp[(size_t)i + (size_t)j * pp] = Gat(i, j);
+      }
+    int rk = chol_upper(pp, Mp, Rm, 1e-14);
+    if (opt.verbose > 1) {
+      double dev = 0;
+      for (int j = 0; j < pp; j++)
+        for (int i = 0; i < pp; i++) dev = std::max(dev, std::fabs(Mat(i, j) - (i == j ? 1.0 : 0.0)));
+      std::fprintf(stderr, "[bsn svd]   Q'Q: max |M - I| = %.3e, Cholesky rank %d of %d\n", dev, rk, pp);
+    }
+    rr_rank = pp;
+    if (rk == pp) {
+      inv_upper(pp, Rm, Rmi);
+      small_mm(pp, pp, pp, Gp.data(), Rmi.data(), tmp.data());
+      evec.assign((size_t)pp * pp, 0.0);
+      for (int j = 0; j < pp; j++)
+        for (int i = 0; i <= j; i++) {
+          double a = 0;
+          for (int t = 0; t <= i; t++) a += Rmi[(size_t)t + (size_t)i * pp] * tmp[(size_t)t + (size_t)j * pp];
+          evec[(size_t)i + (size_t)j * pp] = a;
+          evec[(size_t)j + (size_t)i * pp] = a;
+        }
+      eig_sym(pp, evec, eval);
+      small_mm(pp, pp, pp, Rmi.data(), evec.data(), tmp.data());
+      evec.swap(tmp);
+    } else {
+      std::vector<double> V(Mp), lam;
+      eig_sym(pp, V, lam);
+      const double lmax = lam[pp - 1];
+      int r = 0;
+      while (r < pp && lam[pp - 1 - r] > 1e-8 * lmax && lmax > 0) r++;
+      std::vector<double> T((size_t)pp * std::max(r, 1), 0.0), GT((size_t)pp * std::max(r, 1)), B((size_t)r * r), bl;
+      for (int c = 0; c < r; c++) {
+        const double f = 1.0 / std::sqrt(lam[pp - 1 - c]);
+        for (int i = 0; i < pp; i++) T[(size_t)i + (size_t)c * pp] = V[(size_t)i + (size_t)(pp - 1 - c) * pp] * f;
+      }
+      small_mm(pp, pp, r, Gp.data(), T.data(), GT.data());
+      for (int j = 0; j < r; j++)
+        for (int i = 0; i <= j; i++) {
+          double a = 0;
+          for (int t = 0; t < pp; t++) a += T[(size_t)t + (size_t)i * pp] * GT[(size_t)t + (size_t)j * pp];
+          B[(size_t)i + (size_t)j * r] = B[(size_t)j + (size_t)i * r] = a;
+        }
+      eig_sym(r, B, bl);
+      rr_rank = r;
+      eval.assign((size_t)pp, 0.0);
+      evec.assign((size_t)pp * pp, 0.0);
+      for (int c = 0; c < r; c++) {
+        const int col = pp - r + c;
+        eval[(size_t)col] = bl[(size_t)c];
+        for (int i = 0; i < pp; i++) {
+          double a = 0;
+          for (int t = 0; t < r; t++) a += T[(size_t)i + (size_t)t * pp] * B[(size_t)t + (size_t)c * r];
+          evec[(size_t)i + (size_t)col * pp] = a;
+        }
+      }
+      if (opt.verbose)
+        std::fprintf(stderr, "[bsn svd]   dependent basis: %d of %d directions kept for the Rayleigh-Ritz step\n", r, pp);
+    }
+    return rk;
+  };
+
+  auto extract = [&](int pp, std::vector<double> &S, std::vector<double> &dinv, double *sigma) {
+    const int kk = k < pp ? k : pp;
+    S.assign((size_t)pp * k, 0.0);
+    dinv.assign((size_t)k, 0.0);
+    for (int t = 0; t < k; t++) {
+      double dt = 0;
+      if (t < kk) {
+        const int col = pp - 1 - t;
+        const double th = eval[col] > 0 ? eval[col] : 0;
+        dt = std::sqrt(th);
+        dinv[t] = dt > 0 ? 1.0 / dt : 0.0;
+        for (int i = 0; i < pp; i++) S[(size_t)i + (size_t)t * pp] = evec[(size_t)i + (size_t)col * pp];
+      }
+      if (sigma) sigma[t] = dt;
+    }
+  };
+  bool guess = false;
+  std::vector<double> S_guess, dinv_guess;
+  auto drop_guess = [&]() {
+    if (guess) bk.prefinalize(0, k, nullptr, nullptr, u, v);
+    guess = false;
+  };
+
+  while (cb > 0) {
+    const int p0 = p - cb;
+    drop_guess();
+    bk.At_Qblock(p0, cb);
+    blk.assign((size_t)p * cb, 0.0);
+    blk2.assign((size_t)p * cb, 0.0);
+    bool early = bk.early_grams(p, p0, cb, blk.data(), blk2.data());
+    int S_next = 0;
+    if (opt.slices_base > 0) {
+      const int Sz = step_slices(z_gain);
+      S_next = step_slices(1.0);
+      bk.set_precision(Sz);
+      if (S_next > opt.slices_base || Sz > opt.slices_base) res.wide_steps++;
+      if (std::max(Sz, S_next) > res.slices_used_max) res.slices_used_max = std::max(Sz, S_next);
+      if (opt.verbose)
+        std::fprintf(stderr, "[bsn svd] step %d: %d-bit product pass, next block on %d bits (leading residual %.2e, product weight %.3f)\n",
+                     res.niter + 1, 8 * Sz, 8 * S_next, rho_lead, z_gain);
+    }
+    bk.A_Zblock(p0, cb);
+    const bool hold = sched && S_next > opt.slices_base;
+    if (opt.slices_base > 0) {
+      bk.set_precision(S_next);
+      bk.hold_rounding(hold);
+    }
+    res.nops += 2;
+    res.niter++;
+    bool early_rr = false;
+    if (early) early = bk.early_grams_wait();
+    if (early) {
+      absorb_grams(p, p0, cb);
+      if (p >= (sched ? std::min(k, klead) : k)) {
+        const int rk = ritz(p);
+        early_rr = true;
+        if (p >= k && rk == p && (int64_t)p + cb <= bk.n) {
+          extract(p, S_guess, dinv_guess, nullptr);
+          bk.prefinalize(p, k, S_guess.data(), dinv_guess.data(), u, v);
+          guess = true;
+        }
+      }
+    }
+    int rn = bk.step_fused(p, p0, cb, blk.data(), blk2.data(), Rt);
+    const bool fused_failed = rn == -2;
+    if (rn == -1 && !early) {
+      bk.ZtZ(p, p0, cb, blk.data());
+      bk.QtQ(p, p0, cb, blk2.data());
+    }
+    if (!early) absorb_grams(p, p0, cb);
+    if (rn < 0) {
+      drop_guess();
+      rn = orth(p, cb, C2, Rt, !fused_failed);
+    }
     if ((int64_t)p + rn > bk.n) rn = bk.n > p ? (int)(bk.n - p) : 0;
     pp = p;
     const bool exhausted = (rn == 0) || (p >= dim);
@@ -293,70 +413,7 @@
     if (rn > cap - p) rn = cap - p;
     if (rn < 0) rn = 0;
 
-    if (pp >= (sched ? std::min(k, klead) : k) || rn == 0 || exhausted || want_restart) {
-      std::vector<double> Mp((size_t)pp * pp), Gp((size_t)pp * pp), Rm, Rmi, tmp((size_t)pp * pp);
-      for (int j = 0; j < pp; j++)
-        for (int i = 0; i < pp; i++) {
-          Mp[(size_t)i + (size_t)j * pp] = Mat(i, j);
-          Gp[(size_t)i + (size_t)j * pp] = Gat(i, j);
-        }
-      int rk = chol_upper(pp, Mp, Rm, 1e-14);
-      if (opt.verbose > 1) {
-        double dev = 0;
-        for (int j = 0; j < pp; j++)
-          for (int i = 0; i < pp; i++) dev = std::max(dev, std::fabs(Mat(i, j) - (i == j ? 1.0 : 0.0)));
-        std::fprintf(stderr, "[bsn svd]   Q'Q: max |M - I| = %.3e, Cholesky rank %d of %d\n", dev, rk, pp);
-      }
-      rr_rank = pp;
-      if (rk == pp) {
-        inv_upper(pp, Rm, Rmi);
-        small_mm(pp, pp, pp, Gp.data(), Rmi.data(), tmp.data());
-        evec.assign((size_t)pp * pp, 0.0);
-        for (int j = 0; j < pp; j++)
-          for (int i = 0; i <= j; i++) {
-            double a = 0;
-            for (int t = 0; t <= i; t++) a += Rmi[(size_t)t + (size_t)i * pp] * tmp[(size_t)t + (size_t)j * pp];
-            evec[(size_t)i + (size_t)j * pp] = a;
-            evec[(size_t)j + (size_t)i * pp] = a;
-          }
-        eig_sym(pp, evec, eval);
-        small_mm(pp, pp, pp, Rmi.data(), evec.data(), tmp.data());
-        evec.swap(tmp);
-      } else {
-        std::vector<double> V(Mp), lam;
-        eig_sym(pp, V, lam);
-        const double lmax = lam[pp - 1];
-        int r = 0;
-        while (r < pp && lam[pp - 1 - r] > 1e-8 * lmax && lmax > 0) r++;
-        std::vector<double> T((size_t)pp * std::max(r, 1), 0.0), GT((size_t)pp * std::max(r, 1)), B((size_t)r * r), bl;
-        for (int c = 0; c < r; c++) {
-          const double f = 1.0 / std::sqrt(lam[pp - 1 - c]);
-          for (int i = 0; i < pp; i++) T[(size_t)i + (size_t)c * pp] = V[(size_t)i + (size_t)(pp - 1 - c) * pp] * f;
-        }
-        small_mm(pp, pp, r, Gp.data(), T.data(), GT.data());
-        for (int j = 0; j < r; j++)
-          for (int i = 0; i <= j; i++) {
-            double a = 0;
-            for (int t = 0; t < pp; t++) a += T[(size_t)t + (size_t)i * pp] * GT[(size_t)t + (size_t)j * pp];
-            B[(size_t)i + (size_t)j * r] = B[(size_t)j + (size_t)i * r] = a;
-          }
-        eig_sym(r, B, bl);
-        rr_rank = r;
-        eval.assign((size_t)pp, 0.0);
-        evec.assign((size_t)pp * pp, 0.0);
-        for (int c = 0; c < r; c++) {
-          const int col = pp - r + c;
-          eval[(size_t)col] = bl[(size_t)c];
-          for (int i = 0; i < pp; i++) {
-            double a = 0;
-            for (int t = 0; t < r; t++) a += T[(size_t)i + (size_t)t * pp] * B[(size_t)t + (size_t)c * r];
-            evec[(size_t)i + (size_t)col * pp] = a;
-          }
-        }
-        if (opt.verbose)
-          std::fprintf(stderr, "[bsn svd]   dependent basis: %d of %d directions kept for the Rayleigh-Ritz step\n", r, pp);
-      }
-    }
+    if (!early_rr && (pp >= (sched ? std::min(k, klead) : k) || rn == 0 || exhausted || want_restart)) ritz(pp);
     bool done = false;
     const double hard_zero = 1e-10;
     const double negligible = std::max(hard_zero, 64.0 * opt.resid_floor * opt.resid_floor);
@@ -451,6 +508,7 @@
               Mk[(size_t)i + (size_t)j * keep] = Mk[(size_t)j + (size_t)i * keep] = mm;
             }
         }
+        drop_guess();
         if (bk.restart(pp, keep, Sk.data(), rn_full, Mk.data())) {
           for (int j = 0; j < cap; j++)
             for (int i = 0; i < cap; i++) Gat(i, j) = Mat(i, j) = 0.0;
@@ -491,19 +549,10 @@
   }
 
   res.basis = pp;
-  int kk = k < pp ? k : pp;
-  std::vector<double> S((size_t)pp * k, 0.0), dinv((size_t)k, 0.0);
-  for (int t = 0; t < k; t++) {
-    d[t] = 0;
-    if (t < kk) {
-      int col = pp - 1 - t;
-      double th = eval[col] > 0 ? eval[col] : 0;
-      d[t] = std::sqrt(th);
-      dinv[t] = d[t] > 0 ? 1.0 / d[t] : 0.0;
-      for (int i = 0; i < pp; i++) S[(size_t)i + (size_t)t * pp] = evec[(size_t)i + (size_t)col * pp];
-    }
-  }
-  bk.finalize(pp, k, S.data(), dinv.data(), u, v);
+  std::vector<double> S, dinv;
+  extract(pp, S, dinv, d);
+  if (guess) bk.finalize(pp, k, S_guess.data(), dinv_guess.data(), u, v);
+  else bk.finalize(pp, k, S.data(), dinv.data(), u, v);
   return res;
 }
 
diff --git a/bigsnpr_amd/svd.py b/bigsnpr_amd/svd.py
--- a/bigsnpr_amd/svd.py
+++ b/bigsnpr_amd/svd.py
@@ -69,6 +69,7 @@
                 lead_rel_resid=info.lead_rel_resid, compacted=bool(info.compacted), compact_ms=info.compact_ms,
                 out_of_core=bool(info.out_of_core),
                 na_free_steps=[float(x) for x in info.na_free_steps], na_skip=int(info.na_skip),
+                early_ritz=[int(x) for x in info.early_ritz],
                 exchange_mode=("none", "whole pass", "segments, one stream", "segments, reduce-scatters on a second stream")[
                     max(0, min(3, int(info.exchange_mode)))],
                 exchange_ms=dict(zip(("reduce_scatter", "all_gather", "small", "exposed_wait"), [float(x) for x in info.exchange_ms])),
diff --git a/include/bigsnpr_hip.h b/include/bigsnpr_hip.h
--- a/include/bigsnpr_hip.h
+++ b/include/bigsnpr_hip.h
@@ -163,6 +163,7 @@
   int32_t out_of_core;
   double na_free_steps[2];
   int32_t na_skip;
+  int32_t early_ritz[2];
 } bsn_svd_info;
 int bsn_bed_randomsvd(bsn_bed *bed, const int64_t *ind_row, int64_t n, const int64_t *ind_col,
                       int64_t m, const double *center, const double *scale,
```

Result: faster. 38.26 million, median of 6 (+1.8%).
